# cheneeheng/2s-AGCN

Measured on AMD Instinct MI355X. Metric: skeleton-clips/sec fwd+bwd, NTU (N,3,300,25,2), higher is better.
Workload: dtype f32; 1 GPU; AGCN joint-stream NTU-xview shape, full training step (fwd, CE, bwd, grad all-reduce, clip 1.0, SGD nesterov); per_gpu_batch=64, global_batch=64, input=(N,3,300,25,2), parallelism=dp1, bn=per-replica

## Files before the change

### 2s-agcn_amd/csrc/agcn_common.h

```cpp
#pragma once
#include <hip/hip_runtime.h>
#include <stdint.h>
#include <stdlib.h>
#include <string.h>

typedef float f32x16 __attribute__((ext_vector_type(16)));
typedef float f32x4 __attribute__((ext_vector_type(4)));

#define AGCN_OK 0
#define AGCN_ERR_ARG (-1)
#define AGCN_ERR_WORKSPACE (-2)
#define AGCN_ERR_UNSUPPORTED (-3)

__device__ __forceinline__ f32x16 mfma32(float a, float b, f32x16 c) {
  return __builtin_amdgcn_mfma_f32_32x32x2f32(a, b, c, 0, 0, 0);
}
__device__ __forceinline__ int mfma_row(int j, int h) { return (j & 3) + 8 * (j >> 2) + 4 * h; }

__device__ __forceinline__ float mask_load(const float* m, long idx, int bits) {
  return bits ? m[idx >> 5] : m[idx];
}
__device__ __forceinline__ bool mask_pass(float raw, long idx, int bits) {
  return bits ? ((__builtin_bit_cast(unsigned, raw) >> (idx & 31)) & 1u) != 0u : raw > 0.f;
}

__device__ __forceinline__ float half_sum(float v) {
  v += __shfl_xor(v, 16);
  v += __shfl_xor(v, 8);
  v += __shfl_xor(v, 4);
  v += __shfl_xor(v, 2);
  v += __shfl_xor(v, 1);
  return v;
}

__device__ __forceinline__ int xcd_remap(int bid, int nwg) {
  const int q = nwg >> 3, r = nwg & 7, x = bid & 7, k = bid >> 3;
  const int base = (x < r) ? x * (q + 1) : r * (q + 1) + (x - r) * q;
  return base + k;
}

extern "C" size_t agcn_colsum_scratch_bytes(int W);
extern "C" int agcn_colsum(const float* X, int nslots, int W, void* scratch, float* out, void* stream);

int agcn_adj_finalize(const float* spart, const float* A, const float* PA, const float* alpha, float* P, float* adj,
                      int N, int Ci, int T, int V, hipStream_t s, int nused = -1);

bool agcn_adj_ws_supported(int N, int C, int Ci, int T, int V);
size_t agcn_adj_ws_workspace(int C, int Ci);
int agcn_adj_ws_scores(const float* x, const float* wab, const float* bab, float* tp_out, float* spart, int slots,
                       int* nslots_used, const float* x_absmax, void* ws, size_t ws_bytes, int N, int C, int Ci, int T, int V,
                       hipStream_t s);

size_t agcn_bf16_conv_workspace(int Cin, int Cout, int T, int V, int stride);
bool agcn_bf16_conv_wide(int taps, int M);
int agcn_bf16_conv9_fwd(const float* x, const float* w, const float* bias, float* y, float* stats_part, void* ws,
                        size_t ws_bytes, int N, int Cin, int Cout, int T, int V, int stride, int npl, hipStream_t s,
                        const float* add = nullptr, int relu = 0, const float* x_absmax = nullptr);
int agcn_bf16_conv9_bwd_data(const float* dy, const float* w, float* dx, int accumulate, const float* add1,
                             const float* mask1, const float* add2, const float* mask2, void* ws, size_t ws_bytes,
                             int N, int Cin, int Cout, int T, int V, int stride, int npl, hipStream_t s,
                             const float* dy_absmax = nullptr);

bool agcn_bf16_tconv_supported(int taps, int stride);
int agcn_bf16_tconv_tile_frames(int taps, int M, int V, int T_out, int npl);
int agcn_bf16_tconv_fwd(const float* x, const float* w, const float* bias, float* y, float* stats_part, void* ws,
                        size_t ws_bytes, int N, int Cin, int Cout, int T, int V, int taps, int pad, int npl,
                        hipStream_t s, const float* x_absmax);
int agcn_bf16_tconv_bwd_data(const float* dy, const float* w, float* dx, int accumulate, const float* add1,
                             const float* mask1, const float* add2, const float* mask2, void* ws, size_t ws_bytes,
                             int N, int Cin, int Cout, int T, int V, int taps, int pad, int npl, hipStream_t s,
                             const float* dy_absmax);

struct GateArgs;
bool agcn_bf16_tconv_infer_supported(int taps, int stride, int pad);
int agcn_bf16_tconv_infer(const float* x, const float* w, const float* bias, float* y, void* ws, size_t ws_bytes, int N,
                          int Cin, int Cout, int T, int V, int taps, int stride, int pad, int npl, hipStream_t s,
                          const float* add, int relu, const float* x_absmax, const GateArgs* gate);

size_t agcn_bf16_conv1_workspace(int Cin, int Cout, int T, int V, int stride);
int agcn_bf16_conv1_fwd(const float* x, const float* w, const float* bias, float* y, float* stats_part, void* ws,
                        size_t ws_bytes, int N, int Cin, int Cout, int T, int V, int stride, int npl, hipStream_t s,
                        const float* add = nullptr, int relu = 0);
int agcn_bf16_conv1_bwd_data(const float* dy, const float* w, float* dx, int accumulate, const float* add1,
                             const float* mask1, const float* add2, const float* mask2, void* ws, size_t ws_bytes,
                             int N, int Cin, int Cout, int T, int V, int npl, hipStream_t s);

bool agcn_gcn_chain_supported(int M, int K, int V);
int agcn_chain_f16x3();
int agcn_gcn_chain_tiles(int T);
int agcn_gcn_chain_stats_slots(int N, int M, int K, int T, int V);
size_t agcn_gcn_chain_workspace(int M, int K, int K2, int T, int V);
int agcn_gcn_chain(int mode, const float* in, const float* adj, const float* wcat, const float* bias, float* out,
                   float* stats_part, int accumulate, const float* add1, const float* mask1, const float* add2,
                   const float* mask2, int mask_bits, const float* in2, const float* w2, int K2, void* ws, size_t ws_bytes,
                   int N, int C, int Cout, int T, int V, hipStream_t stream, int relu = 0, int w2_rows_are_outputs = 0,
                   const float* in_absmax = nullptr, const float* in2_absmax = nullptr);

bool agcn_gcn_dadj_chain_supported(int C, int V);
int agcn_gcn_dadj_chain_slots(int C, int T);
size_t agcn_gcn_dadj_chain_workspace(int C, int Cout);
int agcn_gcn_dadj_chain(const float* dy, const float* wcat, const float* x, float* dadj_part, void* ws, size_t ws_bytes,
                        int N, int C, int Cout, int T, int V, hipStream_t stream, const float* dy_absmax = nullptr,
                        const float* x_absmax = nullptr);

bool agcn_wgrad_chain_supported(int M, int C, int V);
size_t agcn_wgrad_chain_workspace(int agg, int N, int M, int C, int V, int T_out);
int agcn_wgrad_chain(int agg, const float* dy, const float* x, const float* adj, void* ws, size_t ws_bytes, int* nslabs,
                     int N, int M, int C, int V, int T_src, int T_out, int stride, hipStream_t s,
                     const float* dy_absmax = nullptr, const float* x_absmax = nullptr);

bool agcn_wgrad9_bf16_supported(int M, int C, int V, int stride);
size_t agcn_wgrad9_bf16_workspace(int N, int M, int C, int V, int T, int stride);
int agcn_wgrad9_bf16(const float* dy, const float* x, void* ws, size_t ws_bytes, int* nslabs, int N, int M, int C, int V,
                     int T, int stride, hipStream_t s, const float* dy_absmax = nullptr, const float* x_absmax = nullptr);

bool agcn_wgrad_tconv_f16_supported(int M, int C, int V, int taps, int stride, int pad);
size_t agcn_wgrad_tconv_f16_workspace(int N, int M, int C, int V, int T, int taps, int pad);
int agcn_wgrad_tconv_f16(const float* dy, const float* x, void* ws, size_t ws_bytes, int* nslabs, int N, int M, int C,
                         int V, int T, int taps, int pad, hipStream_t s, const float* dy_absmax, const float* x_absmax);

static inline int agcn_gemm_precision() {
  static int mode = -1;
  if (mode < 0) {
    const char* e = getenv("AGCN_GEMM");
    mode = 3;
    if (e && !strcmp(e, "f32")) mode = 0;
    else if (e && !strcmp(e, "bf16x3")) mode = 2;
    else if (e && !strcmp(e, "bf16")) mode = 1;
  }
  return mode;
}
static inline bool agcn_chained() { const int m = agcn_gemm_precision(); return m == 3 || m == 1; }
static inline int agcn_npl() { return agcn_gemm_precision() == 1 ? 1 : 3; }

#define AGCN_MAX_DEVICES 64
static inline int agcn_allow_big_lds_rt(const void* kern, unsigned char* done) {
  int dev = 0;
  if (hipGetDevice(&dev) != hipSuccess || dev < 0 || dev >= AGCN_MAX_DEVICES) dev = -1;
  if (dev >= 0 && __atomic_load_n(&done[dev], __ATOMIC_ACQUIRE)) return AGCN_OK;
  hipError_t e = hipFuncSetAttribute(kern, hipFuncAttributeMaxDynamicSharedMemorySize, 160 * 1024);
  if (e != hipSuccess) return (int)e;
  if (dev >= 0) __atomic_store_n(&done[dev], (unsigned char)1, __ATOMIC_RELEASE);
  return AGCN_OK;
}

#include <stdio.h>
inline thread_local char agcn_last_kernel_buf[192] = "";
#define AGCN_NOTE_KERNEL(...) snprintf(agcn_last_kernel_buf, sizeof(agcn_last_kernel_buf), __VA_ARGS__)

static inline int agcn_check_launch() {
  hipError_t e = hipGetLastError();
  return e == hipSuccess ? AGCN_OK : (int)e;
}
```

### 2s-agcn_amd/csrc/bn.hip

```cpp
#include "agcn_common.h"

namespace {

constexpr int RG = 64;

__global__ void __launch_bounds__(256)
colsum_stage1_kernel(const float* __restrict__ X, int nslots, int W, int per_group, double* __restrict__ partial) {
  __shared__ double red[4][64];
  const int col = blockIdx.x * 64 + (threadIdx.x & 63), sub = threadIdx.x >> 6;
  const int g = blockIdx.y;
  const int s_end = min(nslots, (g + 1) * per_group);
  double acc = 0.0;
  if (col < W)
    for (int s = g * per_group + sub; s < s_end; s += 4) acc += (double)X[(long)s * W + col];
  red[sub][threadIdx.x & 63] = acc;
  __syncthreads();
  if (sub == 0 && col < W)
    partial[(long)g * W + col] = red[0][threadIdx.x] + red[1][threadIdx.x] + red[2][threadIdx.x] + red[3][threadIdx.x];
}

__global__ void colsum_stage2_kernel(const double* __restrict__ partial, int W, float* __restrict__ out) {
  const int col = blockIdx.x * blockDim.x + threadIdx.x;
  if (col >= W) return;
  double s = 0.0;
  for (int g = 0; g < RG; ++g) s += partial[(long)g * W + col];
  out[col] = (float)s;
}

__global__ void bn_stats_finalize_kernel(const double* __restrict__ partial, int C, double count,
                                         const float* __restrict__ gamma, const float* __restrict__ beta,
                                         float* __restrict__ rmean, float* __restrict__ rvar, float momentum,
                                         float eps, float* __restrict__ mean_out, float* __restrict__ invstd_out,
                                         float* __restrict__ scale_out, float* __restrict__ shift_out) {
  const int c = blockIdx.x * blockDim.x + threadIdx.x;
  if (c >= C) return;
  double s = 0.0, ss = 0.0;
  for (int g = 0; g < RG; ++g) {
    s += partial[((long)g * 2 + 0) * C + c];
    ss += partial[((long)g * 2 + 1) * C + c];
  }
  const double mean = s / count;
  double var = ss / count - mean * mean;
  if (var < 0.0) var = 0.0;
  const float invstd = (float)(1.0 / sqrt(var + (double)eps));
  mean_out[c] = (float)mean;
  invstd_out[c] = invstd;
  const float sc = gamma[c] * invstd;
  scale_out[c] = sc;
  shift_out[c] = beta[c] - (float)mean * sc;
  if (rmean) {
    const double unb = count > 1.0 ? var * count / (count - 1.0) : var;
    rmean[c] = (1.f - momentum) * rmean[c] + momentum * (float)mean;
    rvar[c] = (1.f - momentum) * rvar[c] + momentum * (float)unb;
  }
}

__global__ void bn_eval_coeff_kernel(const float* __restrict__ gamma, const float* __restrict__ beta,
                                     const float* __restrict__ rmean, const float* __restrict__ rvar, float eps, int C,
                                     float* __restrict__ scale_out, float* __restrict__ shift_out) {
  const int c = blockIdx.x * blockDim.x + threadIdx.x;
  if (c >= C) return;
  const float sc = gamma[c] / sqrtf(rvar[c] + eps);
  scale_out[c] = sc;
  shift_out[c] = beta[c] - rmean[c] * sc;
}

template <int RES, bool RELU>
__global__ void __launch_bounds__(256)
bn_act_fwd_kernel(const float4* __restrict__ y1, const float* __restrict__ scale1, const float* __restrict__ shift1,
                  const float4* __restrict__ r, const float* __restrict__ scale2, const float* __restrict__ shift2,
                  float4* __restrict__ out, unsigned* __restrict__ bits, unsigned total4, unsigned P, unsigned C,
                  unsigned* __restrict__ amax) {
  unsigned tmax = 0;
  for (unsigned i0 = blockIdx.x * blockDim.x; i0 < total4; i0 += gridDim.x * blockDim.x) {
    const unsigned i = i0 + threadIdx.x;
    const bool valid = i < total4;
    const unsigned ic = valid ? i : 0u;
    const unsigned e0 = ic * 4u;
    const unsigned row = e0 / P;
    const unsigned rem = e0 - row * P;
    const unsigned c0 = row % C;
    const unsigned c1 = (c0 + 1 == C) ? 0u : c0 + 1;
    const float4 a = y1[ic];
    float4 b = make_float4(0.f, 0.f, 0.f, 0.f);
    if (RES != 0) b = r[ic];
    float av[4] = {a.x, a.y, a.z, a.w};
    float bv[4] = {b.x, b.y, b.z, b.w};
    float ov[4];
#pragma unroll
    for (int k = 0; k < 4; ++k) {
      const unsigned c = (rem + k < P) ? c0 : c1;
      float v = scale1[c] * av[k] + shift1[c];
      if (RES == 1) v += bv[k];
      if (RES == 2) v += scale2[c] * bv[k] + shift2[c];
      ov[k] = RELU ? fmaxf(v, 0.f) : v;
    }
    if (valid) out[i] = make_float4(ov[0], ov[1], ov[2], ov[3]);
    if (amax && valid) {
#pragma unroll
      for (int k = 0; k < 4; ++k) tmax = max(tmax, __float_as_uint(ov[k]) & 0x7fffffffu);
    }
    if (bits) {
      unsigned nib = valid ? ((ov[0] > 0.f) | ((ov[1] > 0.f) << 1) | ((ov[2] > 0.f) << 2) | ((ov[3] > 0.f) << 3)) : 0u;
      unsigned w = nib << (4u * (threadIdx.x & 7u));
      w |= __shfl_xor(w, 1);
      w |= __shfl_xor(w, 2);
      w |= __shfl_xor(w, 4);
      if ((threadIdx.x & 7u) == 0u && valid) bits[e0 >> 5] = w;
    }
  }
  if (amax) {
#pragma unroll
    for (int k = 32; k >= 1; k >>= 1) tmax = max(tmax, (unsigned)__shfl_xor((int)tmax, k));
    __shared__ unsigned wmax[4];
    if ((threadIdx.x & 63u) == 0u) wmax[threadIdx.x >> 6] = tmax;
    __syncthreads();
    if (threadIdx.x == 0) {
      const unsigned m = max(max(wmax[0], wmax[1]), max(wmax[2], wmax[3]));
      if (m) atomicMax(amax, m);
    }
  }
}

template <bool HAS2>
__global__ void __launch_bounds__(256)
bn_bwd_reduce_kernel(const float* __restrict__ dout, const float* __restrict__ mask, int mask_bits,
                     const float* __restrict__ y1, const float* __restrict__ y2, float* __restrict__ part, int P) {
  __shared__ float red[3][4];
  const long row = blockIdx.x;
  const float* d = dout + row * P;
  const float* mk = (mask && !mask_bits) ? mask + row * P : nullptr;
  const unsigned* mb = (mask && mask_bits) ? reinterpret_cast<const unsigned*>(mask) : nullptr;
  const long e_row = row * P;
  const float* a = y1 + row * P;
  const float* b = HAS2 ? y2 + row * P : nullptr;
  float s0 = 0.f, s1 = 0.f, s2 = 0.f;
  typedef float4 float4_u __attribute__((aligned(4)));
  const int P4 = P >> 2;
  for (int q4 = threadIdx.x; q4 < P4; q4 += 256) {
    const float4 d4 = reinterpret_cast<const float4_u*>(d)[q4];
    const float4 a4 = reinterpret_cast<const float4_u*>(a)[q4];
    float dv[4] = {d4.x, d4.y, d4.z, d4.w};
    const float av[4] = {a4.x, a4.y, a4.z, a4.w};
    if (mk) {
      const float4 m4 = reinterpret_cast<const float4_u*>(mk)[q4];
      const float mv[4] = {m4.x, m4.y, m4.z, m4.w};
#pragma unroll
      for (int k = 0; k < 4; ++k) dv[k] = (mv[k] > 0.f) ? dv[k] : 0.f;
    }
    if (mb) {
      const long e = e_row + 4L * q4;
      const int sh = (int)(e & 31);
      unsigned nib = mb[e >> 5] >> sh;
      if (sh > 28) nib |= mb[(e >> 5) + 1] << (32 - sh);
#pragma unroll
      for (int k = 0; k < 4; ++k) dv[k] = ((nib >> k) & 1u) ? dv[k] : 0.f;
    }
    float bv[4] = {0.f, 0.f, 0.f, 0.f};
    if (HAS2) {
      const float4 b4 = reinterpret_cast<const float4_u*>(b)[q4];
      bv[0] = b4.x; bv[1] = b4.y; bv[2] = b4.z; bv[3] = b4.w;
    }
#pragma unroll
    for (int k = 0; k < 4; ++k) {
      s0 += dv[k];
      s1 += dv[k] * av[k];
      if (HAS2) s2 += dv[k] * bv[k];
    }
  }
  for (int q = 4 * P4 + threadIdx.x; q < P; q += 256) {
    float dz = d[q];
    if (mk) dz = (mk[q] > 0.f) ? dz : 0.f;
    if (mb) {
      const long e = e_row + q;
      dz = ((mb[e >> 5] >> (e & 31)) & 1u) ? dz : 0.f;
    }
    s0 += dz;
    s1 += dz * a[q];
    if (HAS2) s2 += dz * b[q];
  }
  s0 = half_sum(s0); s1 = half_sum(s1); s2 = half_sum(s2);
  s0 += __shfl_xor(s0, 32); s1 += __shfl_xor(s1, 32); s2 += __shfl_xor(s2, 32);
  const int wave = threadIdx.x >> 6;
  if ((threadIdx.x & 63) == 0) { red[0][wave] = s0; red[1][wave] = s1; red[2][wave] = s2; }
  __syncthreads();
  if (threadIdx.x < 3) {
    const int k = threadIdx.x;
    part[row * 3 + k] = red[k][0] + red[k][1] + red[k][2] + red[k][3];
  }
}

__global__ void bn_bwd_finalize_kernel(const float* __restrict__ part, int N, int C, double count, float pscale,
                                       const float* __restrict__ gamma1, const float* __restrict__ mean1,
                                       const float* __restrict__ invstd1, const float* __restrict__ gamma2,
                                       const float* __restrict__ mean2, const float* __restrict__ invstd2,
                                       float* __restrict__ coef, float* __restrict__ dgamma1,
                                       float* __restrict__ dbeta1, float* __restrict__ dgamma2,
                                       float* __restrict__ dbeta2) {
  const int c = blockIdx.x * blockDim.x + threadIdx.x;
  if (c >= C) return;
  double s0 = 0.0, s1 = 0.0, s2 = 0.0;
#pragma unroll 8
  for (int n = 0; n < N; ++n) {
    const float* p = part + ((long)n * C + c) * 3;
    s0 += (double)p[0]; s1 += (double)p[1]; s2 += (double)p[2];
  }
  {
    const double is = invstd1[c], mu = mean1[c], g = gamma1[c];
    const double sxh = is * (s1 - mu * s0);
    const double k = g * is;
    coef[0 * C + c] = (float)k;
    coef[1 * C + c] = (float)(-k * is * sxh / count);
    coef[2 * C + c] = (float)(-k * s0 / count + k * is * mu * sxh / count);
    dgamma1[c] = (float)sxh * pscale;
    dbeta1[c] = (float)s0 * pscale;
  }
  if (gamma2) {
    const double is = invstd2[c], mu = mean2[c], g = gamma2[c];
    const double sxh = is * (s2 - mu * s0);
    const double k = g * is;
    coef[3 * C + c] = (float)k;
    coef[4 * C + c] = (float)(-k * is * sxh / count);
    coef[5 * C + c] = (float)(-k * s0 / count + k * is * mu * sxh / count);
    dgamma2[c] = (float)sxh * pscale;
    dbeta2[c] = (float)s0 * pscale;
  }
}

template <bool HAS2>
__global__ void __launch_bounds__(256)
bn_bwd_apply_kernel(const float4* __restrict__ dout, const float4* __restrict__ mask, int mask_bits,
                    const float4* __restrict__ y1,
                    const float4* __restrict__ y2, const float* __restrict__ coef, float4* __restrict__ dy1,
                    float4* __restrict__ dy2, unsigned total4, unsigned P, unsigned C, unsigned* __restrict__ amax1) {
  unsigned tmax = 0;
  for (unsigned i = blockIdx.x * blockDim.x + threadIdx.x; i < total4; i += gridDim.x * blockDim.x) {
    const unsigned e0 = i * 4u;
    const unsigned row = e0 / P;
    const unsigned rem = e0 - row * P;
    const unsigned c0 = row % C;
    const unsigned c1 = (c0 + 1 == C) ? 0u : c0 + 1;
    const float4 d4 = dout[i];
    const float4 a4 = y1[i];
    float dv[4] = {d4.x, d4.y, d4.z, d4.w};
    float av[4] = {a4.x, a4.y, a4.z, a4.w};
    if (mask && !mask_bits) {
      const float4 m4 = mask[i];
      const float mv[4] = {m4.x, m4.y, m4.z, m4.w};
#pragma unroll
      for (int k = 0; k < 4; ++k) dv[k] = (mv[k] > 0.f) ? dv[k] : 0.f;
    } else if (mask) {
      const unsigned nib = reinterpret_cast<const unsigned*>(mask)[e0 >> 5] >> (e0 & 31u);
#pragma unroll
      for (int k = 0; k < 4; ++k) dv[k] = ((nib >> k) & 1u) ? dv[k] : 0.f;
    }
    float bv[4] = {0.f, 0.f, 0.f, 0.f};
    if (HAS2) {
      const float4 b4 = y2[i];
      bv[0] = b4.x; bv[1] = b4.y; bv[2] = b4.z; bv[3] = b4.w;
    }
    float o1[4], o2[4];
#pragma unroll
    for (int k = 0; k < 4; ++k) {
      const unsigned c = (rem + k < P) ? c0 : c1;
      o1[k] = coef[0 * C + c] * dv[k] + coef[1 * C + c] * av[k] + coef[2 * C + c];
      if (HAS2) o2[k] = coef[3 * C + c] * dv[k] + coef[4 * C + c] * bv[k] + coef[5 * C + c];
    }
    dy1[i] = make_float4(o1[0], o1[1], o1[2], o1[3]);
    if (HAS2) dy2[i] = make_float4(o2[0], o2[1], o2[2], o2[3]);
    if (amax1) {
#pragma unroll
      for (int k = 0; k < 4; ++k) tmax = max(tmax, __float_as_uint(o1[k]) & 0x7fffffffu);
    }
  }
  if (amax1) {
#pragma unroll
    for (int k = 32; k >= 1; k >>= 1) tmax = max(tmax, (unsigned)__shfl_xor((int)tmax, k));
    __shared__ unsigned wmax[4];
    if ((threadIdx.x & 63u) == 0u) wmax[threadIdx.x >> 6] = tmax;
    __syncthreads();
    if (threadIdx.x == 0) {
      const unsigned m = max(max(wmax[0], wmax[1]), max(wmax[2], wmax[3]));
      if (m) atomicMax(amax1, m);
    }
  }
}

inline unsigned ew_grid(unsigned total4) {
  unsigned g = (total4 + 255u) / 256u;
  return g > 4096u ? 4096u : (g ? g : 1u);
}

}

extern "C" {

size_t agcn_colsum_scratch_bytes(int W) { return sizeof(double) * (size_t)RG * (size_t)W; }

int agcn_colsum(const float* X, int nslots, int W, void* scratch, float* out, void* stream) {
  if (!X || !scratch || !out || nslots <= 0 || W <= 0) return AGCN_ERR_ARG;
  hipStream_t s = (hipStream_t)stream;
  const int per_group = (nslots + RG - 1) / RG;
  hipLaunchKernelGGL(colsum_stage1_kernel, dim3((W + 63) / 64, RG), dim3(256), 0, s, X, nslots, W, per_group,
                     (double*)scratch);
  int rc = agcn_check_launch();
  if (rc) return rc;
  hipLaunchKernelGGL(colsum_stage2_kernel, dim3((W + 255) / 256), dim3(256), 0, s, (const double*)scratch, W, out);
  return agcn_check_launch();
}

int agcn_bn_stats_finalize(const float* part, int nslots, int C, double count, const float* gamma, const float* beta,
                           float* running_mean, float* running_var, float momentum, float eps, void* scratch,
                           float* mean, float* invstd, float* scale, float* shift, void* stream) {
  if (!part || !gamma || !beta || !scratch || !mean || !invstd || !scale || !shift || C <= 0 || nslots <= 0)
    return AGCN_ERR_ARG;
  hipStream_t s = (hipStream_t)stream;
  const int W = 2 * C;
  const int per_group = (nslots + RG - 1) / RG;
  hipLaunchKernelGGL(colsum_stage1_kernel, dim3((W + 63) / 64, RG), dim3(256), 0, s, part, nslots, W, per_group,
                     (double*)scratch);
  int rc = agcn_check_launch();
  if (rc) return rc;
  hipLaunchKernelGGL(bn_stats_finalize_kernel, dim3((C + 63) / 64), dim3(64), 0, s, (const double*)scratch, C, count,
                     gamma, beta, running_mean, running_var, momentum, eps, mean, invstd, scale, shift);
  return agcn_check_launch();
}

int agcn_bn_eval_coeff(const float* gamma, const float* beta, const float* running_mean, const float* running_var,
                       float eps, int C, float* scale, float* shift, void* stream) {
  if (!gamma || !beta || !running_mean || !running_var || !scale || !shift || C <= 0) return AGCN_ERR_ARG;
  hipLaunchKernelGGL(bn_eval_coeff_kernel, dim3((C + 63) / 64), dim3(64), 0, (hipStream_t)stream, gamma, beta,
                     running_mean, running_var, eps, C, scale, shift);
  return agcn_check_launch();
}

int agcn_bn_act_fwd_ex(const float* y1, const float* scale1, const float* shift1, const float* r, const float* scale2,
                       const float* shift2, float* out, unsigned* sign_bits, float* absmax_out, int N, int C, int P,
                       int res_mode, int relu, void* stream);
int agcn_bn_act_fwd(const float* y1, const float* scale1, const float* shift1, const float* r, const float* scale2,
                    const float* shift2, float* out, unsigned* sign_bits, int N, int C, int P, int res_mode, int relu,
                    void* stream) {
  return agcn_bn_act_fwd_ex(y1, scale1, shift1, r, scale2, shift2, out, sign_bits, nullptr, N, C, P, res_mode, relu, stream);
}

int agcn_bn_act_fwd_ex(const float* y1, const float* scale1, const float* shift1, const float* r, const float* scale2,
                       const float* shift2, float* out, unsigned* sign_bits, float* absmax_out, int N, int C, int P,
                       int res_mode, int relu, void* stream) {
  if (!y1 || !scale1 || !shift1 || !out || N <= 0 || C <= 0 || P <= 0) return AGCN_ERR_ARG;
  if (absmax_out && hipMemsetAsync(absmax_out, 0, 4, (hipStream_t)stream) != hipSuccess) return AGCN_ERR_ARG;
  const long total = (long)N * C * P;
  if (total % 4 != 0 || total > 0xffffffffL) return AGCN_ERR_UNSUPPORTED;
  if (res_mode != 0 && !r) return AGCN_ERR_ARG;
  if (res_mode == 2 && (!scale2 || !shift2)) return AGCN_ERR_ARG;
  const unsigned t4 = (unsigned)(total / 4);
  hipStream_t s = (hipStream_t)stream;
  const dim3 g(ew_grid(t4)), b(256);
#define LAUNCH_ACT(R, A)                                                                                       \
  hipLaunchKernelGGL((bn_act_fwd_kernel<R, A>), g, b, 0, s, (const float4*)y1, scale1, shift1, (const float4*)r, \
                     scale2, shift2, (float4*)out, sign_bits, t4, (unsigned)P, (unsigned)C, (unsigned*)absmax_out)
  if (relu) {
    if (res_mode == 0) LAUNCH_ACT(0, true); else if (res_mode == 1) LAUNCH_ACT(1, true); else LAUNCH_ACT(2, true);
  } else {
    if (res_mode == 0) LAUNCH_ACT(0, false); else if (res_mode == 1) LAUNCH_ACT(1, false); else LAUNCH_ACT(2, false);
  }
#undef LAUNCH_ACT
  return agcn_check_launch();
}

int agcn_bn_bwd_reduce(const float* dout, const void* mask, int mask_bits, const float* y1, const float* y2, float* part,
                       int N, int C, int P, void* stream) {
  if (!dout || !y1 || !part || N <= 0 || C <= 0 || P <= 0) return AGCN_ERR_ARG;
  hipStream_t s = (hipStream_t)stream;
  if (y2) hipLaunchKernelGGL(bn_bwd_reduce_kernel<true>, dim3(N * C), dim3(256), 0, s, dout, (const float*)mask,
                             mask_bits, y1, y2, part, P);
  else hipLaunchKernelGGL(bn_bwd_reduce_kernel<false>, dim3(N * C), dim3(256), 0, s, dout, (const float*)mask,
                          mask_bits, y1, y2, part, P);
  return agcn_check_launch();
}

int agcn_bn_bwd_apply_ex(const float* part, int nrows, double count, float param_grad_scale, const float* dout,
                         const void* mask, int mask_bits, const float* y1, const float* gamma1, const float* mean1,
                         const float* invstd1, const float* y2, const float* gamma2, const float* mean2,
                         const float* invstd2, float* coef, float* dy1, float* dgamma1, float* dbeta1, float* dy2,
                         float* dgamma2, float* dbeta2, float* absmax1_out, int N, int C, int P, void* stream);
int agcn_bn_bwd_apply(const float* part, int nrows, double count, float param_grad_scale, const float* dout,
                      const void* mask, int mask_bits, const float* y1, const float* gamma1, const float* mean1, const float* invstd1,
                      const float* y2, const float* gamma2, const float* mean2, const float* invstd2, float* coef,
                      float* dy1, float* dgamma1, float* dbeta1, float* dy2, float* dgamma2, float* dbeta2, int N, int C,
                      int P, void* stream) {
  return agcn_bn_bwd_apply_ex(part, nrows, count, param_grad_scale, dout, mask, mask_bits, y1, gamma1, mean1, invstd1, y2,
                              gamma2, mean2, invstd2, coef, dy1, dgamma1, dbeta1, dy2, dgamma2, dbeta2, nullptr, N, C, P,
                              stream);
}

int agcn_bn_bwd_apply_ex(const float* part, int nrows, double count, float param_grad_scale, const float* dout,
                         const void* mask, int mask_bits, const float* y1, const float* gamma1, const float* mean1,
                         const float* invstd1, const float* y2, const float* gamma2, const float* mean2,
                         const float* invstd2, float* coef, float* dy1, float* dgamma1, float* dbeta1, float* dy2,
                         float* dgamma2, float* dbeta2, float* absmax1_out, int N, int C, int P, void* stream) {
  if (absmax1_out && hipMemsetAsync(absmax1_out, 0, 4, (hipStream_t)stream) != hipSuccess) return AGCN_ERR_ARG;
  if (!part || !dout || !y1 || !gamma1 || !mean1 || !invstd1 || !coef || !dy1 || !dgamma1 || !dbeta1 || nrows <= 0)
    return AGCN_ERR_ARG;
  if (y2 && (!gamma2 || !mean2 || !invstd2 || !dy2 || !dgamma2 || !dbeta2)) return AGCN_ERR_ARG;
  const long total = (long)N * C * P;
  if (total % 4 != 0 || total > 0xffffffffL) return AGCN_ERR_UNSUPPORTED;
  hipStream_t s = (hipStream_t)stream;
  hipLaunchKernelGGL(bn_bwd_finalize_kernel, dim3((C + 63) / 64), dim3(64), 0, s, part, nrows, C, count,
                     param_grad_scale, gamma1, mean1, invstd1, y2 ? gamma2 : nullptr, mean2, invstd2, coef, dgamma1,
                     dbeta1, dgamma2, dbeta2);
  int rc = agcn_check_launch();
  if (rc) return rc;
  const unsigned t4 = (unsigned)(total / 4);
  const dim3 g(ew_grid(t4)), b(256);
  if (y2)
    hipLaunchKernelGGL(bn_bwd_apply_kernel<true>, g, b, 0, s, (const float4*)dout, (const float4*)mask, mask_bits,
                       (const float4*)y1, (const float4*)y2, (const float*)coef, (float4*)dy1, (float4*)dy2, t4,
                       (unsigned)P, (unsigned)C, (unsigned*)absmax1_out);
  else
    hipLaunchKernelGGL(bn_bwd_apply_kernel<false>, g, b, 0, s, (const float4*)dout, (const float4*)mask, mask_bits,
                       (const float4*)y1, (const float4*)y2, (const float*)coef, (float4*)dy1, (float4*)dy2, t4,
                       (unsigned)P, (unsigned)C, (unsigned*)absmax1_out);
  return agcn_check_launch();
}

int agcn_bn_bwd(const float* dout, const void* mask, int mask_bits, const float* y1, const float* gamma1,
                const float* mean1, const float* invstd1, const float* y2, const float* gamma2, const float* mean2,
                const float* invstd2, float* part, float* coef, float* dy1, float* dgamma1, float* dbeta1, float* dy2,
                float* dgamma2, float* dbeta2, int N, int C, int P, void* stream) {
  int rc = agcn_bn_bwd_reduce(dout, mask, mask_bits, y1, y2, part, N, C, P, stream);
  if (rc) return rc;
  return agcn_bn_bwd_apply(part, N, (double)N * (double)P, 1.0f, dout, mask, mask_bits, y1, gamma1, mean1, invstd1, y2, gamma2,
                           mean2, invstd2, coef, dy1, dgamma1, dbeta1, dy2, dgamma2, dbeta2, N, C, P, stream);
}

const char* agcn_arch(void) { return "gfx950"; }
int agcn_version(void) { return 100; }

}
```

### 2s-agcn_amd/csrc/conv_wgrad.hip

```cpp
#include "agcn_common.h"

namespace {

struct WgradArgs {
  const float* dy;
  const float* in;
  const float* adj;
  float* part;
  int N, M, C, V, T_src, T_out, stride;
  int pad;
  int tt, ntiles, FW, WLP, DAP, GP;
  long so_m, so_t, so_c;
  long wsize;
  int nsplit, pairs_per_split;
  int off_bx, off_bg, off_adj, off_qoff;
};

template <int TAPS, int AGG, int MW, int CW, int TH, bool KSPLIT, int WBX>
__global__ void __launch_bounds__(512) conv_wgrad_kernel(const WgradArgs a) {
  constexpr int NW = 8, NT = 512;
  static_assert(MW * CW * TH == NW, "8 waves");
  constexpr int BM = MW * 32, CB = CW * 32;
  constexpr int NSUB = AGG ? 3 : 1;
  constexpr bool TSPLIT = (TH == 2) && !KSPLIT;
// ... 4 lines not shown
  float* Da = smem;
  float* Bx = smem + a.off_bx;
  float* Bg = smem + a.off_bg;
  float* adjp = smem + a.off_adj;
  int* qoff = reinterpret_cast<int*>(smem + a.off_qoff);

  const int tid = threadIdx.x, lane = tid & 63;
  const int wave = __builtin_amdgcn_readfirstlane(tid >> 6);
  const int lr = lane & 31, h = lane >> 5;
  const int th = wave / (MW * CW);
  const int wmc = wave - th * (MW * CW);
  const int mw = wmc % MW, cw = wmc / MW;
  const int ncb = (a.C + CB - 1) / CB;
  const int mb = blockIdx.x / ncb, cb = blockIdx.x - mb * ncb;
  const int m0 = mb * BM, c0 = cb * CB;
  const int V = a.V, tt = a.tt, ttv = tt * V;
  const int Psrc = a.T_src * V, Pout = a.T_out * V;
  const int WL = a.FW * V, WLP = a.WLP, DAP = a.DAP, GP = a.GP;
  const int KS = (ttv + 1) >> 1;
  const int tap0 = TSPLIT ? th * NTW : 0;
  const int ntaps = TSPLIT ? (th == 0 ? NTW : TAPS - NTW) : TAPS;
  const int s_begin = KSPLIT ? (th * ((KS + 1) >> 1)) : 0;
  const int s_end = KSPLIT ? min(KS, s_begin + ((KS + 1) >> 1)) : KS;

  for (int q = tid; q < 2 * KS + 2; q += NT) {
    int o = 0;
    if (q < ttv) {
      const int tl = q / V;
      o = AGG ? q : (tl * a.stride * V + (q - tl * V));
    }
    qoff[q] = o;
  }

  f32x16 acc[NACC];
#pragma unroll
  for (int z = 0; z < NACC; ++z)
#pragma unroll
    for (int j = 0; j < 16; ++j) acc[z][j] = 0.f;

  float rda[RD][2];
  float rbx[RB][WBX];

  auto pair_geom = [&](int p, int& n, int& t0, int& nvalid, int& g0) __attribute__((always_inline)) {
    n = p / a.ntiles;
    const int tile = p - n * a.ntiles;
    t0 = tile * tt;
    nvalid = min(tt, a.T_out - t0) * V;
    g0 = (AGG ? t0 : (t0 * a.stride - a.pad)) * V;
  };
  auto issue_loads = [&](int p) __attribute__((always_inline)) {
    int n, t0, nvalid, g0;
    pair_geom(p, n, t0, nvalid, g0);
#pragma unroll
    for (int j = 0; j < RD; ++j) {
      const int m = m0 + wave + j * NW;
      const bool okr = m < a.M;
      const float* src = a.dy + ((long)n * a.M + (okr ? m : 0)) * Pout + (long)t0 * V;
#pragma unroll
      for (int u = 0; u < 2; ++u) {
        const int q = lane + 64 * u;
        rda[j][u] = src[(okr && q < nvalid) ? q : 0];
      }
    }
#pragma unroll
    for (int j = 0; j < RB; ++j) {
      const int c = c0 + wave + j * NW;
      const bool okr = c < a.C;
      const float* src = a.in + ((long)n * a.C + (okr ? c : 0)) * Psrc;
#pragma unroll
      for (int u = 0; u < WBX; ++u) {
        const int r = lane + 64 * u;
        const int gp = g0 + r;
        rbx[j][u] = src[(okr && r < WL && gp >= 0 && gp < Psrc) ? gp : 0];
      }
    }
  };
  auto commit_lds = [&](int p) __attribute__((always_inline)) {
    int n, t0, nvalid, g0;
    pair_geom(p, n, t0, nvalid, g0);
#pragma unroll
    for (int j = 0; j < RD; ++j) {
      const int ml = wave + j * NW;
      const bool okr = (m0 + ml) < a.M;
#pragma unroll
      for (int u = 0; u < 2; ++u) {
        const int q = lane + 64 * u;
        if (q < DAP) Da[ml * DAP + q] = (okr && q < nvalid) ? rda[j][u] : 0.f;
      }
    }
#pragma unroll
    for (int j = 0; j < RB; ++j) {
      const int cl = wave + j * NW;
      const bool okr = (c0 + cl) < a.C;
#pragma unroll
      for (int u = 0; u < WBX; ++u) {
        const int r = lane + 64 * u;
        const int gp = g0 + r;
        if (r < WLP) Bx[cl * WLP + r] = (okr && r < WL && gp >= 0 && gp < Psrc) ? rbx[j][u] : 0.f;
      }
    }
  };

  const int total_pairs = a.N * a.ntiles;
  const int p_begin = blockIdx.y * a.pairs_per_split;
  const int p_end = min(total_pairs, p_begin + a.pairs_per_split);
  int last_n = -1;
  if (p_begin < p_end) issue_loads(p_begin);
  for (int p = p_begin; p < p_end; ++p) {
    __syncthreads();
    commit_lds(p);
    const int n = p / a.ntiles;
    if (AGG && n != last_n) {
      const int VP = 2 * ((V + 1) / 2);
      const float* adjn = a.adj + (long)n * 3 * V * V;
      for (int e = tid; e < 3 * VP * 32; e += NT) {
        const int i = e / (VP * 32), r = e - i * (VP * 32);
        const int u = r >> 5, col = r & 31;
        const bool ok = u < V && col < V;
        const float t = adjn[ok ? ((i * V + u) * V + col) : 0];
        adjp[e] = ok ? t : 0.f;
      }
      last_n = n;
    }
    if (p + 1 < p_end) issue_loads(p + 1);
    __syncthreads();
#pragma unroll
    for (int sub = 0; sub < NSUB; ++sub) {
      if (AGG) {
        if (sub > 0) __syncthreads();
        const int nrows = CB * tt;
        const int nrt = (nrows + 31) >> 5;
        const int VS = (V + 1) >> 1, VP = 2 * VS;
        for (int rt = wave; rt < nrt; rt += NW) {
          const int row = min(rt * 32 + lr, nrows - 1);
          f32x16 d;
#pragma unroll
          for (int j = 0; j < 16; ++j) d[j] = 0.f;
          for (int s = 0; s < VS; ++s) {
            const int u = 2 * s + h;
            float av = Bx[row * V + min(u, V - 1)];
            av = (u < V) ? av : 0.f;
            d = mfma32(av, adjp[(sub * VP + u) * 32 + lr], d);
          }
#pragma unroll
          for (int j = 0; j < 16; ++j) {
            const int r2 = rt * 32 + mfma_row(j, h);
            if (r2 < nrows && lr < V) {
              const int cl = r2 / tt, tl = r2 - cl * tt;
              Bg[cl * GP + tl * V + lr] = d[j];
            }
          }
        }
        __syncthreads();
      }
      const float* Bsrc = (AGG ? Bg : Bx) + (cw * 32 + lr) * (AGG ? GP : WLP) + tap0 * V;
      const float* Asrc = Da + (mw * 32 + lr) * DAP;
      const bool lin = AGG || a.stride == 1;
      auto load_ops = [&](int s, float& av, float (&bv)[NTW]) __attribute__((always_inline)) {
        const int q = 2 * s + h;
        const int qo = lin ? q : qoff[q];
        av = Asrc[q];
#pragma unroll
        for (int t = 0; t < NTW; ++t) bv[t] = Bsrc[qo + ((TSPLIT && t >= ntaps) ? 0 : t * V)];
      };
      if (s_begin < s_end) {
        float av, bv[NTW];
        load_ops(s_begin, av, bv);
        for (int s = s_begin; s < s_end; ++s) {
          float an, bn[NTW];
          load_ops(min(s + 1, s_end - 1), an, bn);
#pragma unroll
          for (int t = 0; t < NTW; ++t)
            if (!TSPLIT || t < ntaps) acc[sub * NTW + t] = mfma32(av, bv[t], acc[sub * NTW + t]);
          av = an;
#pragma unroll
          for (int t = 0; t < NTW; ++t) bv[t] = bn[t];
        }
      }
    }
  }
  const int slab = KSPLIT ? ((int)blockIdx.y * TH + th) : (int)blockIdx.y;
  float* dst = a.part + (long)slab * a.wsize;
#pragma unroll
  for (int z = 0; z < NACC; ++z) {
    const int sub = z / NTW, t = z - sub * NTW;
    if (TSPLIT && t >= ntaps) continue;
    const int zz = AGG ? sub : (tap0 + t);
#pragma unroll
    for (int j = 0; j < 16; ++j) {
      const int m = m0 + mw * 32 + mfma_row(j, h);
      const int c = c0 + cw * 32 + lr;
      if (m < a.M && c < a.C) dst[((long)zz * a.M + m) * a.C + c] = acc[z][j];
    }
  }
}

__global__ void wgrad_reduce_kernel(const float* __restrict__ part, float* __restrict__ dw, long wsize, int nsplit,
                                    int M, int C, long so_m, long so_t, long so_c) {
  const long i = (long)blockIdx.x * blockDim.x + threadIdx.x;
  if (i >= wsize) return;
  float s = 0.f;
  for (int k = 0; k < nsplit; ++k) s += part[(long)k * wsize + i];
  const int c = (int)(i % C);
  const long r = i / C;
  const int m = (int)(r % M);
  const int z = (int)(r / M);
  dw[(long)m * so_m + (long)z * so_t + (long)c * so_c] = s;
}

__global__ void __launch_bounds__(256)
wgrad_reduce_wide_kernel(const float* __restrict__ part, float* __restrict__ dw, long wsize, int nsplit, int M, int C,
                         long so_m, long so_t, long so_c) {
  __shared__ float red[8][32];
  const int el = threadIdx.x & 31, g = threadIdx.x >> 5;
  const long i = (long)blockIdx.x * 32 + el;
  float s = 0.f;
  if (i < wsize) {
#pragma unroll 8
    for (int k = g; k < nsplit; k += 8) s += part[(long)k * wsize + i];
  }
  red[g][el] = s;
  __syncthreads();
  if (g == 0 && i < wsize) {
    float t = red[0][el];
#pragma unroll
    for (int k = 1; k < 8; ++k) t += red[k][el];
    const int c = (int)(i % C);
    const long r = i / C;
    const int m = (int)(r % M);
    const int z = (int)(r / M);
    dw[(long)m * so_m + (long)z * so_t + (long)c * so_c] = t;
  }
}

inline int launch_reduce(const float* ws, float* dw, long wsize, int nslabs, int M, int C, long so_m, long so_t, long so_c,
                         hipStream_t stream) {
  if (nslabs >= 64) {
    hipLaunchKernelGGL(wgrad_reduce_wide_kernel, dim3((unsigned)((wsize + 31) / 32)), dim3(256), 0, stream, ws, dw,
                       wsize, nslabs, M, C, so_m, so_t, so_c);
  } else {
    const int threads = 256;
    hipLaunchKernelGGL(wgrad_reduce_kernel, dim3((unsigned)((wsize + threads - 1) / threads)), dim3(threads), 0,
                       stream, ws, dw, wsize, nslabs, M, C, so_m, so_t, so_c);
  }
  return agcn_check_launch();
}

struct WGeom {
  int tt, ntiles, FW, WLP, DAP, GP, nsplit, nslabs, pairs_per_split, grid_x;
  int off_bx, off_bg, off_adj, off_qoff;
  size_t smem_bytes;
};

template <int TAPS, int AGG, int MW, int CW, int TH, bool KSPLIT>
WGeom wgeom(int N, int M, int C, int V, int T_out, int stride, int tt_cap = 0) {
  constexpr int BM = MW * 32, CB = CW * 32;
  WGeom g;
  g.tt = 128 / V;
  if (g.tt > T_out) g.tt = T_out;
  if (tt_cap > 0 && g.tt > tt_cap) g.tt = tt_cap;
  const int ttv = g.tt * V;
  g.ntiles = (T_out + g.tt - 1) / g.tt;
  g.FW = AGG ? g.tt : ((g.tt - 1) * stride + TAPS);
  const int WL = g.FW * V;
  g.WLP = AGG ? WL : (WL | 1);
  if (!AGG && g.WLP == WL) g.WLP = WL + 2;
  g.DAP = (ttv + 2) | 1;
  g.GP = ttv | 1;
  const int da = BM * g.DAP;
  g.off_bx = (da + 3) & ~3;
  const int bx = CB * g.WLP + 64;
  g.off_bg = g.off_bx + ((bx + 3) & ~3);
  const int bg = AGG ? CB * g.GP + 64 : 0;
  g.off_adj = g.off_bg + ((bg + 3) & ~3);
  const int VP = 2 * ((V + 1) / 2);
  const int adjsz = AGG ? 3 * VP * 32 : 0;
  g.off_qoff = g.off_adj + ((adjsz + 3) & ~3);
  g.smem_bytes = 4 * ((size_t)g.off_qoff + ttv + 8);
  const int nmb = (M + BM - 1) / BM, ncb = (C + CB - 1) / CB;
  g.grid_x = nmb * ncb;
  const int pairs = N * g.ntiles;
  int want = 256 / g.grid_x;
  if (want < 1) want = 1;
  if (want > pairs) want = pairs;
  g.pairs_per_split = (pairs + want - 1) / want;
  g.nsplit = (pairs + g.pairs_per_split - 1) / g.pairs_per_split;
  g.nslabs = g.nsplit * (KSPLIT ? TH : 1);
  return g;
}

template <int TAPS, int AGG, int MW, int CW, int TH, bool KSPLIT, int WBX>
int launch_wgrad(WgradArgs a, float* dw, void* ws, size_t ws_bytes, hipStream_t stream, int tt_cap = 0) {
  const WGeom g = wgeom<TAPS, AGG, MW, CW, TH, KSPLIT>(a.N, a.M, a.C, a.V, a.T_out, a.stride, tt_cap);
  if (g.smem_bytes > 160 * 1024) return AGCN_ERR_UNSUPPORTED;
  if (g.WLP > WBX * 64 || g.tt * a.V > 128) return AGCN_ERR_UNSUPPORTED;
  if ((size_t)g.nslabs * a.wsize * 4 > ws_bytes) return AGCN_ERR_WORKSPACE;
  a.part = (float*)ws;
  a.tt = g.tt; a.ntiles = g.ntiles; a.FW = g.FW; a.WLP = g.WLP; a.DAP = g.DAP; a.GP = g.GP;
  a.nsplit = g.nsplit; a.pairs_per_split = g.pairs_per_split;
  a.off_bx = g.off_bx; a.off_bg = g.off_bg; a.off_adj = g.off_adj; a.off_qoff = g.off_qoff;
  auto kern = conv_wgrad_kernel<TAPS, AGG, MW, CW, TH, KSPLIT, WBX>;
  static unsigned char lds_ok[AGCN_MAX_DEVICES] = {};
  if (int e = agcn_allow_big_lds_rt(reinterpret_cast<const void*>(kern), lds_ok)) return e;
  hipLaunchKernelGGL(kern, dim3(g.grid_x, g.nsplit), dim3(512), g.smem_bytes, stream, a);
  int rc = agcn_check_launch();
  if (rc) return rc;
  return launch_reduce((const float*)ws, dw, a.wsize, g.nslabs, a.M, a.C, a.so_m, a.so_t, a.so_c, stream);
}

template <int TAPS, int AGG, int MW, int CW, int TH, bool KSPLIT>
size_t ws_wgrad(int N, int M, int C, int V, int T_out, int stride, long wsize, int tt_cap = 0) {
  const WGeom g = wgeom<TAPS, AGG, MW, CW, TH, KSPLIT>(N, M, C, V, T_out, stride, tt_cap);
  return (size_t)g.nslabs * wsize * 4;
}

int chain_wgrad_and_reduce(int agg, const WgradArgs& a, float* dw, void* ws, size_t ws_bytes, hipStream_t stream,
                           const float* dy_absmax = nullptr, const float* x_absmax = nullptr) {
  int nslabs = 0;
  int rc = agcn_wgrad_chain(agg, a.dy, a.in, a.adj, ws, ws_bytes, &nslabs, a.N, a.M, a.C, a.V, a.T_src, a.T_out,
                            a.stride, stream, dy_absmax, x_absmax);
  if (rc) return rc;
  return launch_reduce((const float*)ws, dw, a.wsize, nslabs, a.M, a.C, a.so_m, a.so_t, a.so_c, stream);
}

inline bool wgrad9_bf16_enabled() {
  static int v = -1;
  if (v < 0) {
    const char* e = getenv("AGCN_WGRAD9_BF16");
    v = (e && atoi(e) == 0) ? 0 : 1;
  }
  return v == 1;
}

constexpr int WBXT = 8;

inline int tconv_w_tt(int V, int T_out, int taps, int stride) {
  int tt = 128 / V;
  if (tt > T_out) tt = T_out;
  while (tt > 1 && ((tt - 1) * stride + taps) * V + 2 > WBXT * 64) --tt;
  return tt < 1 ? 1 : tt;
}

template <int TAPS>
int tconv_wgrad(WgradArgs a, float* dw, void* ws, size_t ws_bytes, hipStream_t s, size_t* ws_need) {
  const int cap = tconv_w_tt(a.V, a.T_out, TAPS, a.stride);
  if (!ws_need) AGCN_NOTE_KERNEL("conv_wgrad_kernel<%d, 0>", TAPS);
  if (TAPS == 1) {
    if (a.M % 128 == 0) {
      if (ws_need) { *ws_need = ws_wgrad<1, 0, 4, 2, 1, false>(a.N, a.M, a.C, a.V, a.T_out, a.stride, a.wsize, cap); return 0; }
      return launch_wgrad<1, 0, 4, 2, 1, false, WBXT>(a, dw, ws, ws_bytes, s, cap);
    }
    if (ws_need) { *ws_need = ws_wgrad<1, 0, 2, 2, 2, true>(a.N, a.M, a.C, a.V, a.T_out, a.stride, a.wsize, cap); return 0; }
    return launch_wgrad<1, 0, 2, 2, 2, true, WBXT>(a, dw, ws, ws_bytes, s, cap);
  }
  if (a.M % 128 == 0) {
    if (ws_need) { *ws_need = ws_wgrad<TAPS, 0, 4, 1, 2, false>(a.N, a.M, a.C, a.V, a.T_out, a.stride, a.wsize, cap); return 0; }
    return launch_wgrad<TAPS, 0, 4, 1, 2, false, WBXT>(a, dw, ws, ws_bytes, s, cap);
  }
  if (ws_need) { *ws_need = ws_wgrad<TAPS, 0, 2, 2, 2, false>(a.N, a.M, a.C, a.V, a.T_out, a.stride, a.wsize, cap); return 0; }
  return launch_wgrad<TAPS, 0, 2, 2, 2, false, WBXT>(a, dw, ws, ws_bytes, s, cap);
}

int tconv_wgrad_dispatch(int taps, const WgradArgs& a, float* dw, void* ws, size_t ws_bytes, hipStream_t s,
                         size_t* ws_need) {
  switch (taps) {
    case 1: return tconv_wgrad<1>(a, dw, ws, ws_bytes, s, ws_need);
    case 2: return tconv_wgrad<2>(a, dw, ws, ws_bytes, s, ws_need);
    case 3: return tconv_wgrad<3>(a, dw, ws, ws_bytes, s, ws_need);
    case 4: return tconv_wgrad<4>(a, dw, ws, ws_bytes, s, ws_need);
    case 5: return tconv_wgrad<5>(a, dw, ws, ws_bytes, s, ws_need);
    case 6: return tconv_wgrad<6>(a, dw, ws, ws_bytes, s, ws_need);
    case 7: return tconv_wgrad<7>(a, dw, ws, ws_bytes, s, ws_need);
    case 8: return tconv_wgrad<8>(a, dw, ws, ws_bytes, s, ws_need);
    case 9: return tconv_wgrad<9>(a, dw, ws, ws_bytes, s, ws_need);
    default: return AGCN_ERR_UNSUPPORTED;
  }
}

inline bool tconv_w_domain(int T, int taps, int stride, int pad) {
  return taps >= 1 && taps <= 9 && stride >= 1 && stride <= 9 && pad >= 0 && pad <= (taps - 1) / 2 && T + 2 * pad >= taps;
}

inline bool chain_wgrad_enabled() {
  static int v = -1;
  if (v < 0) {
    const char* e = getenv("AGCN_WGRAD_BF16");
    v = (e && atoi(e) == 0) ? 0 : 1;
  }
  return v == 1 && agcn_chained();
}

}

extern "C" {

size_t agcn_conv_bwd_weight_workspace(int N, int Cin, int Cout, int T, int V, int taps, int stride) {
  const int pad = (taps - 1) / 2;
  const int T_out = (T + 2 * pad - taps) / stride + 1;
  const long wsize = (long)Cout * Cin * taps;
  if (taps == 9) {
    size_t b9 = (Cout % 128 == 0) ? ws_wgrad<9, 0, 4, 1, 2, false>(N, Cout, Cin, V, T_out, stride, wsize)
                                  : ws_wgrad<9, 0, 2, 2, 2, false>(N, Cout, Cin, V, T_out, stride, wsize);
    if (agcn_wgrad9_bf16_supported(Cout, Cin, V, stride)) {
      const size_t t = agcn_wgrad9_bf16_workspace(N, Cout, Cin, V, T, stride);
      if (t > b9) b9 = t;
    }
    return b9;
  }
  size_t b = (Cout % 128 == 0) ? ws_wgrad<1, 0, 4, 2, 1, false>(N, Cout, Cin, V, T_out, stride, wsize)
                              : ws_wgrad<1, 0, 2, 2, 2, true>(N, Cout, Cin, V, T_out, stride, wsize);
  if (agcn_wgrad_chain_supported(Cout, Cin, V)) {
    const size_t t = agcn_wgrad_chain_workspace(0, N, Cout, Cin, V, T_out);
    if (t > b) b = t;
  }
  return b;
}

int agcn_conv_bwd_weight_ex(const float* dy, const float* x, float* dw, void* workspace, size_t workspace_bytes, int N,
                            int Cin, int Cout, int T, int V, int taps, int stride, const float* dy_absmax,
                            const float* x_absmax, void* stream);
int agcn_conv_bwd_weight(const float* dy, const float* x, float* dw, void* workspace, size_t workspace_bytes, int N,
                         int Cin, int Cout, int T, int V, int taps, int stride, void* stream) {
  return agcn_conv_bwd_weight_ex(dy, x, dw, workspace, workspace_bytes, N, Cin, Cout, T, V, taps, stride, nullptr, nullptr,
                                 stream);
}
int agcn_conv_bwd_weight_ex(const float* dy, const float* x, float* dw, void* workspace, size_t workspace_bytes, int N,
                            int Cin, int Cout, int T, int V, int taps, int stride, const float* dy_absmax,
                            const float* x_absmax, void* stream) {
  if (!dy || !x || !dw || !workspace || N <= 0 || Cin <= 0 || Cout <= 0 || T <= 0 || V <= 0 || V > 32)
    return AGCN_ERR_ARG;
  if ((taps != 1 && taps != 9) || (stride != 1 && stride != 2)) return AGCN_ERR_UNSUPPORTED;
  const int pad = (taps - 1) / 2;
  WgradArgs a = {};
  a.dy = dy; a.in = x; a.N = N; a.M = Cout; a.C = Cin; a.V = V; a.T_src = T;
  a.T_out = (T + 2 * pad - taps) / stride + 1; a.stride = stride; a.pad = pad;
  a.so_m = (long)Cin * taps; a.so_t = 1; a.so_c = taps; a.wsize = (long)Cout * Cin * taps;
  hipStream_t s = (hipStream_t)stream;
  if (taps == 9) {
    if (wgrad9_bf16_enabled() && agcn_wgrad9_bf16_supported(Cout, Cin, V, stride)) {
      int nslabs = 0;
      int rc = agcn_wgrad9_bf16(dy, x, workspace, workspace_bytes, &nslabs, N, Cout, Cin, V, T, stride, s, dy_absmax, x_absmax);
      if (rc) return rc;
      return launch_reduce((const float*)workspace, dw, a.wsize, nslabs, a.M, a.C, a.so_m, a.so_t, a.so_c, s);
    }
    if (stride == 1) {
      if (Cout % 128 == 0) return launch_wgrad<9, 0, 4, 1, 2, false, 6>(a, dw, workspace, workspace_bytes, s);
      return launch_wgrad<9, 0, 2, 2, 2, false, 6>(a, dw, workspace, workspace_bytes, s);
    }
    if (Cout % 128 == 0) return launch_wgrad<9, 0, 4, 1, 2, false, 7>(a, dw, workspace, workspace_bytes, s);
    return launch_wgrad<9, 0, 2, 2, 2, false, 7>(a, dw, workspace, workspace_bytes, s);
  }
  if (chain_wgrad_enabled() && agcn_wgrad_chain_supported(Cout, Cin, V))
    return chain_wgrad_and_reduce(0, a, dw, workspace, workspace_bytes, s, dy_absmax, x_absmax);
  if (Cout % 128 == 0) return launch_wgrad<1, 0, 4, 2, 1, false, 4>(a, dw, workspace, workspace_bytes, s);
  return launch_wgrad<1, 0, 2, 2, 2, true, 4>(a, dw, workspace, workspace_bytes, s);
}

size_t agcn_gcn_project_bwd_weight_workspace(int N, int C, int Cout, int T, int V) {
  const long wsize = 3L * Cout * C;
  size_t b = (Cout % 128 == 0) ? ws_wgrad<1, 1, 4, 2, 1, false>(N, Cout, C, V, T, 1, wsize)
                              : ws_wgrad<1, 1, 2, 2, 2, true>(N, Cout, C, V, T, 1, wsize);
  if (agcn_wgrad_chain_supported(Cout, C, V)) {
    const size_t t = agcn_wgrad_chain_workspace(1, N, Cout, C, V, T);
    if (t > b) b = t;
  }
  return b;
}

int agcn_gcn_project_bwd_weight_ex(const float* dy, const float* x, const float* adj, float* dwcat, void* workspace,
                                   size_t workspace_bytes, int N, int C, int Cout, int T, int V, const float* dy_absmax,
                                   const float* x_absmax, void* stream);
int agcn_gcn_project_bwd_weight(const float* dy, const float* x, const float* adj, float* dwcat, void* workspace,
                                size_t workspace_bytes, int N, int C, int Cout, int T, int V, void* stream) {
  return agcn_gcn_project_bwd_weight_ex(dy, x, adj, dwcat, workspace, workspace_bytes, N, C, Cout, T, V, nullptr, nullptr,
                                        stream);
}
int agcn_gcn_project_bwd_weight_ex(const float* dy, const float* x, const float* adj, float* dwcat, void* workspace,
                                   size_t workspace_bytes, int N, int C, int Cout, int T, int V, const float* dy_absmax,
                                   const float* x_absmax, void* stream) {
  if (!dy || !x || !adj || !dwcat || !workspace || N <= 0 || C <= 0 || Cout <= 0 || T <= 0 || V <= 0 || V > 32)
    return AGCN_ERR_ARG;
  WgradArgs a = {};
  a.dy = dy; a.in = x; a.adj = adj; a.N = N; a.M = Cout; a.C = C; a.V = V; a.T_src = T; a.T_out = T; a.stride = 1;
  a.so_m = 3L * C; a.so_t = C; a.so_c = 1; a.wsize = 3L * Cout * C;
  hipStream_t s = (hipStream_t)stream;
  if (chain_wgrad_enabled() && agcn_wgrad_chain_supported(Cout, C, V))
    return chain_wgrad_and_reduce(1, a, dwcat, workspace, workspace_bytes, s, dy_absmax, x_absmax);
  if (Cout % 128 == 0) return launch_wgrad<1, 1, 4, 2, 1, false, 2>(a, dwcat, workspace, workspace_bytes, s);
  return launch_wgrad<1, 1, 2, 2, 2, true, 2>(a, dwcat, workspace, workspace_bytes, s);
}


size_t agcn_tconv_bwd_weight_workspace(int N, int Cin, int Cout, int T, int V, int taps, int stride, int pad) {
  if (N <= 0 || Cin <= 0 || Cout <= 0 || T <= 0 || V <= 0 || !tconv_w_domain(T, taps, stride, pad)) return 0;
  if (pad == (taps - 1) / 2 && (taps == 1 || taps == 9) && (stride == 1 || stride == 2))
    return agcn_conv_bwd_weight_workspace(N, Cin, Cout, T, V, taps, stride);
  WgradArgs a = {};
  a.N = N; a.M = Cout; a.C = Cin; a.V = V; a.T_src = T; a.T_out = (T + 2 * pad - taps) / stride + 1; a.stride = stride;
  a.pad = pad; a.wsize = (long)Cout * Cin * taps;
  size_t need = 0;
  tconv_wgrad_dispatch(taps, a, nullptr, nullptr, 0, nullptr, &need);
  if (agcn_wgrad_tconv_f16_supported(Cout, Cin, V, taps, stride, pad)) {
    const size_t t = agcn_wgrad_tconv_f16_workspace(N, Cout, Cin, V, T, taps, pad);
    if (t > need) need = t;
  }
  return need;
}

int agcn_tconv_bwd_weight(const float* dy, const float* x, float* dw, void* workspace, size_t workspace_bytes, int N,
                          int Cin, int Cout, int T, int V, int taps, int stride, int pad, const float* dy_absmax,
                          const float* x_absmax, void* stream) {
  if (!dy || !x || !dw || !workspace || N <= 0 || Cin <= 0 || Cout <= 0 || T <= 0 || V <= 0 || V > 32)
    return AGCN_ERR_ARG;
  if (!tconv_w_domain(T, taps, stride, pad)) return AGCN_ERR_UNSUPPORTED;
  if (pad == (taps - 1) / 2 && (taps == 1 || taps == 9) && (stride == 1 || stride == 2))
    return agcn_conv_bwd_weight_ex(dy, x, dw, workspace, workspace_bytes, N, Cin, Cout, T, V, taps, stride, dy_absmax,
                                   x_absmax, stream);
  WgradArgs a = {};
  a.dy = dy; a.in = x; a.N = N; a.M = Cout; a.C = Cin; a.V = V; a.T_src = T;
  a.T_out = (T + 2 * pad - taps) / stride + 1; a.stride = stride; a.pad = pad;
  a.so_m = (long)Cin * taps; a.so_t = 1; a.so_c = taps; a.wsize = (long)Cout * Cin * taps;
  hipStream_t s = (hipStream_t)stream;
  if (agcn_wgrad_tconv_f16_supported(Cout, Cin, V, taps, stride, pad)) {
    int nslabs = 0;
    const int rc = agcn_wgrad_tconv_f16(dy, x, workspace, workspace_bytes, &nslabs, N, Cout, Cin, V, T, taps, pad, s,
                                        dy_absmax, x_absmax);
    if (rc) return rc;
    return launch_reduce((const float*)workspace, dw, a.wsize, nslabs, a.M, a.C, a.so_m, a.so_t, a.so_c, s);
  }
  return tconv_wgrad_dispatch(taps, a, dw, workspace, workspace_bytes, s, nullptr);
}

}
```

### 2s-agcn_amd/csrc/wgrad_chain.hip

```cpp
#include "agcn_common.h"
#include "split_f16.h"

namespace {

typedef __bf16 bf16x8 __attribute__((ext_vector_type(8)));
typedef __bf16 bf16x2 __attribute__((ext_vector_type(2)));
typedef float f32x2 __attribute__((ext_vector_type(2)));
typedef unsigned u32x4 __attribute__((ext_vector_type(4)));
typedef f32x4 f32x4_u __attribute__((aligned(4)));

struct WcArgs {
  const float* dy;
  const float* in;
  const float* adj;
  float* part;
  int N, M, C, V, T_src, T_out, stride;
  int ntiles, pairs_per_split, ncg;
  int XP;
  long wsize;
  int npl;
  int dbg;
  int pad;
  const float* dy_absmax;
  const float* in_absmax;
// ... 314 lines not shown
            for (int e = 0; e < 4; ++e) rdy[k][4 * run + e] = q[e];
          }
        } else {
#pragma unroll
          for (int e = 0; e < 8; ++e) {
            const float* q = src + (e & 3) + 8 * (e >> 2);
            rdy[k][e] = (q < dy_end) ? *q : 0.f;
          }
        }
      }
      const int piece = ptid & (LPR - 1), rsub = (ptid & 63) / LPR;
      const float* xb = a.in + (long)n * a.C * Psrc + (long)t0 * V + 4 * piece;
#pragma unroll
      for (int u = 0; u < XV; ++u) {
        const int row = (wave - NWC) * (CG / NWP) + u * (64 / LPR) + rsub;
        const float* src = xb + (long)min(c0 + row, a.C - 1) * Psrc;
        if (src + 4 <= x_end) {
          rx[u] = *reinterpret_cast<const f32x4_u*>(src);
        } else {
#pragma unroll
          for (int e = 0; e < 4; ++e) rx[u][e] = (src + e < x_end) ? src[e] : 0.f;
        }
      }
    };
    auto commit = [&](int p, unsigned char* buf) __attribute__((always_inline)) {
      int n, t0;
      pair_geom(p, n, t0);
      int ptid = threadIdx.x - NWC * 64;
      asm volatile("" : "+v"(ptid));
      unsigned char* dyi = buf;
      float* xs = reinterpret_cast<float*>(buf + DY_BYTES);
#pragma unroll
      for (int k = 0; k < DI; ++k) {
        const int item = ptid + k * NTP;
        const int o = item / (FT * 4), r = item - o * (FT * 4);
        u32x4 ph, pm, pl;
#pragma unroll
        for (int e2 = 0; e2 < 4; ++e2) {
          unsigned q0, q1, q2 = 0;
          if constexpr (F16) split_pair_f16(rdy[k][2 * e2] * s_dy, rdy[k][2 * e2 + 1] * s_dy, q0, q1);
          else wc_split_pair(rdy[k][2 * e2], rdy[k][2 * e2 + 1], q0, q1, q2);
          ph[e2] = q0; pm[e2] = q1; pl[e2] = q2;
        }
        const int slot = r * BMP + o;
        *reinterpret_cast<u32x4*>(dyi + ((0 * FT * 4) * BMP + slot) * 16) = ph;
        *reinterpret_cast<u32x4*>(dyi + ((1 * FT * 4) * BMP + slot) * 16) = pm;
        if constexpr (!F16) *reinterpret_cast<u32x4*>(dyi + ((2 * FT * 4) * BMP + slot) * 16) = pl;
      }
      const int piece = ptid & (LPR - 1), rsub = (ptid & 63) / LPR;
#pragma unroll
      for (int u = 0; u < XV; ++u) {
        const int row = (wave - NWC) * (CG / NWP) + u * (64 / LPR) + rsub;
#pragma unroll
        for (int e = 0; e < 4; ++e) {
          const int q = 4 * piece + e;
          if (q < FTV) xs[row * XP + q] = rx[u][e];
        }
      }
      if (AGG && n != adj_n[p & 1]) {
        adj_n[p & 1] = n;
        const float* adjn = a.adj + (long)n * 3 * V * V;
        if constexpr (!BCH) {
          float* adjp = reinterpret_cast<float*>(buf + BUF_BYTES - ADJ_BYTES);
          for (int e = ptid; e < 3 * 32 * 32; e += NTP) {
            const int sub = e >> 10, u = (e >> 5) & 31, v = e & 31;
            const bool ok = u < V && v < V;
            const float tv = adjn[ok ? ((sub * V + u) * V + v) : 0];
            adjp[e] = ok ? tv : 0.f;
          }
        } else {
          unsigned char* adjq = buf + BUF_BYTES - ADJ_BYTES;
          for (int e = ptid; e < 3 * 2 * 2 * 32 * 4; e += NTP) {
            const int e2 = e & 3, col = (e >> 2) & 31, hh = (e >> 7) & 1, ks = (e >> 8) & 1, sub = e >> 9;
            float vv[2];
#pragma unroll
            for (int q = 0; q < 2; ++q) {
              const int u = 16 * ks + 8 * hh + 2 * e2 + q;
              const bool ok = u < V && col < V;
              const float tv = adjn[ok ? ((sub * V + u) * V + col) : 0];
              vv[q] = ok ? tv : 0.f;
            }
            unsigned q0, q1, q2 = 0;
            if constexpr (F16) split_pair_f16(vv[0], vv[1], q0, q1);
            else wc_split_pair(vv[0], vv[1], q0, q1, q2);
            const int o = (((ks * 2 + hh) * 32) + col) * 16 + e2 * 4;
            *reinterpret_cast<unsigned*>(adjq + (sub * PLA + 0) * 2048 + o) = q0;
            *reinterpret_cast<unsigned*>(adjq + (sub * PLA + 1) * 2048 + o) = q1;
            if constexpr (!F16) *reinterpret_cast<unsigned*>(adjq + (sub * PLA + 2) * 2048 + o) = q2;
          }
        }
      }
    };
    if (XP > FTV)
      for (int e = threadIdx.x - NWC * 64; e < 2 * CG; e += NTP)
        reinterpret_cast<float*>(smem + (e / CG) * BUF_BYTES + DY_BYTES)[(e % CG) * XP + FTV] = 0.f;
    {
      const int gap = (((CG * XP * 4 + 15) & ~15) - CG * XP * 4 + XSLACK) / 4;
      const int e = threadIdx.x - NWC * 64;
      if (e < 2 * gap) reinterpret_cast<float*>(smem + (e / max(gap, 1)) * BUF_BYTES + DY_BYTES)[CG * XP + e % max(gap, 1)] = 0.f;
    }
    if (p_begin < p_end) {
      issue(p_begin);
      commit(p_begin, smem + (p_begin & 1) * BUF_BYTES);
      if (p_begin + 1 < p_end) issue(p_begin + 1);
    }
    stage_barrier();
    for (int p = p_begin; p < p_end; ++p) {
      if (p + 1 < p_end && !(a.dbg & 2)) {
        commit(p + 1, smem + ((p + 1) & 1) * BUF_BYTES);
        if (p + 2 < p_end) issue(p + 2);
      }
      stage_barrier();
    }
    return;
  }

  const int lane = threadIdx.x & 63;
  const int lr = lane & 31, h = lane >> 5;
  const int cbw = wave % NCB, fg = (wave / NCB) % NFG, rb = wave / (NCB * NFG);
  f32x16 acc[NS][TM];
#pragma unroll
  for (int sub = 0; sub < NS; ++sub)
#pragma unroll
    for (int tm = 0; tm < TM; ++tm)
#pragma unroll
      for (int j = 0; j < 16; ++j) acc[sub][tm][j] = 0.f;
  stage_barrier();
  for (int p = p_begin; p < p_end; ++p) {
    int n, t0;
    pair_geom(p, n, t0);
    const unsigned char* dyi = smem + (p & 1) * BUF_BYTES;
    const float* xs = reinterpret_cast<const float*>(dyi + DY_BYTES);
    const int f = fg;
    if (t0 + f < a.T_out && !(a.dbg & 1)) {
      const float* xr = xs + (cbw * 32 + lr) * XP + f * V;
      const unsigned char* ab = dyi + (((f * 4 + h) * BMP) + rb * (TM * 32) + lr) * 16;
#pragma unroll
      for (int sub = 0; sub < NS; ++sub) {
        f32x16 d;
        if (AGG) {
#pragma unroll
          for (int j = 0; j < 16; ++j) d[j] = 0.f;
          const float* xrs = xr;
          asm volatile("" : "+v"(xrs));
          if constexpr (!BCH) {
            const float* adjp = reinterpret_cast<const float*>(dyi + BUF_BYTES - ADJ_BYTES) + sub * 1024;
            float ao[BCH ? 1 : VS], xo[BCH ? 1 : VS];
#pragma unroll
            for (int s = 0; s < VS; ++s) {
              ao[s] = adjp[(2 * s + h) * 32 + lr];
              xo[s] = xrs[2 * s + h];
            }
#pragma unroll
            for (int s = 0; s < VS; ++s) d = mfma32(ao[s], xo[s], d);
          } else {
            const unsigned char* aq = dyi + BUF_BYTES - ADJ_BYTES + sub * PLA * 2048 + (h * 32 + lr) * 16;
#pragma unroll
            for (int ks = 0; ks < 2; ++ks) {
              u32x4 qh, qm, ql;
#pragma unroll
              for (int e2 = 0; e2 < 4; ++e2) {
                unsigned q0, q1, q2 = 0;
                const float xa = xrs[16 * ks + 8 * h + 2 * e2], xb2 = xrs[16 * ks + 8 * h + 2 * e2 + 1];
                if constexpr (F16) split_pair_f16_mix(xa * s_x, xb2 * s_x, q0, q1);
                else wc_split_pair(xa, xb2, q0, q1, q2);
                qh[e2] = q0; qm[e2] = q1; ql[e2] = q2;
              }
              if constexpr (F16) {
                const f16x8 x0 = __builtin_bit_cast(f16x8, qh), x1 = __builtin_bit_cast(f16x8, qm);
                const f16x8 a0 = *reinterpret_cast<const f16x8*>(aq + 0 * 2048 + ks * 1024);
                const f16x8 a1 = *reinterpret_cast<const f16x8*>(aq + 1 * 2048 + ks * 1024);
                d = __builtin_amdgcn_mfma_f32_32x32x16_f16(a1, x0, d, 0, 0, 0);
                d = __builtin_amdgcn_mfma_f32_32x32x16_f16(a0, x1, d, 0, 0, 0);
                d = __builtin_amdgcn_mfma_f32_32x32x16_f16(a0, x0, d, 0, 0, 0);
              } else {
                const bf16x8 x0 = __builtin_bit_cast(bf16x8, qh), x1 = __builtin_bit_cast(bf16x8, qm),
                             x2 = __builtin_bit_cast(bf16x8, ql);
                const bf16x8 a0 = *reinterpret_cast<const bf16x8*>(aq + 0 * 2048 + ks * 1024);
                const bf16x8 a1 = *reinterpret_cast<const bf16x8*>(aq + 1 * 2048 + ks * 1024);
                const bf16x8 a2 = *reinterpret_cast<const bf16x8*>(aq + 2 * 2048 + ks * 1024);
                d = __builtin_amdgcn_mfma_f32_32x32x16_bf16(a2, x0, d, 0, 0, 0);
                d = __builtin_amdgcn_mfma_f32_32x32x16_bf16(a0, x2, d, 0, 0, 0);
                d = __builtin_amdgcn_mfma_f32_32x32x16_bf16(a1, x1, d, 0, 0, 0);
                d = __builtin_amdgcn_mfma_f32_32x32x16_bf16(a1, x0, d, 0, 0, 0);
                d = __builtin_amdgcn_mfma_f32_32x32x16_bf16(a0, x1, d, 0, 0, 0);
                d = __builtin_amdgcn_mfma_f32_32x32x16_bf16(a0, x0, d, 0, 0, 0);
              }
            }
          }
        } else {
#pragma unroll
          for (int j = 0; j < 16; ++j) {
            const int v = (j & 3) + 8 * (j >> 2) + 4 * h;
            const float t = xr[v];
            d[j] = (v < V) ? t : 0.f;
          }
        }
        bf16x8 gb[2][3];
#pragma unroll
        for (int ks = 0; ks < 2; ++ks) {
          u32x4 gh, gm, gl;
#pragma unroll
          for (int e2 = 0; e2 < 4; ++e2) {
            unsigned q0, q1, q2 = 0;
            if constexpr (F16 && BCH) split_pair_f16_mix(d[8 * ks + 2 * e2], d[8 * ks + 2 * e2 + 1], q0, q1);
            else if constexpr (F16) split_pair_f16(d[8 * ks + 2 * e2] * s_x, d[8 * ks + 2 * e2 + 1] * s_x, q0, q1);
            else wc_split_pair(d[8 * ks + 2 * e2], d[8 * ks + 2 * e2 + 1], q0, q1, q2);
            gh[e2] = q0; gm[e2] = q1; gl[e2] = q2;
          }
          gb[ks][0] = __builtin_bit_cast(bf16x8, gh);
          gb[ks][1] = __builtin_bit_cast(bf16x8, gm);
          gb[ks][2] = __builtin_bit_cast(bf16x8, gl);
        }
        auto load_a = [&](bf16x8 (&af)[3], int step) __attribute__((always_inline)) {
          const int ks = step / TM, tm = step - ks * TM;
#pragma unroll
          for (int pl = 0; pl < PL; ++pl)
            af[pl] = *reinterpret_cast<const bf16x8*>(ab + ((pl * FT * 4 + ks * 2) * BMP + tm * 32) * 16);
        };
        bf16x8 afc[3];
        load_a(afc, 0);
        __builtin_amdgcn_sched_group_barrier(0x100, PL, 0);
#pragma unroll
        for (int step = 0; step < 2 * TM; ++step) {
          const int ks = step / TM, tm = step - ks * TM;
          bf16x8 afn[3];
          if (step + 1 < 2 * TM) load_a(afn, step + 1);
          if constexpr (F16) {
            acc[sub][tm] = __builtin_amdgcn_mfma_f32_32x32x16_f16(__builtin_bit_cast(f16x8, afc[1]), __builtin_bit_cast(f16x8, gb[ks][0]), acc[sub][tm], 0, 0, 0);
            acc[sub][tm] = __builtin_amdgcn_mfma_f32_32x32x16_f16(__builtin_bit_cast(f16x8, afc[0]), __builtin_bit_cast(f16x8, gb[ks][1]), acc[sub][tm], 0, 0, 0);
            acc[sub][tm] = __builtin_amdgcn_mfma_f32_32x32x16_f16(__builtin_bit_cast(f16x8, afc[0]), __builtin_bit_cast(f16x8, gb[ks][0]), acc[sub][tm], 0, 0, 0);
          } else {
          if (a.npl == 3) {
            acc[sub][tm] = __builtin_amdgcn_mfma_f32_32x32x16_bf16(afc[2], gb[ks][0], acc[sub][tm], 0, 0, 0);
            acc[sub][tm] = __builtin_amdgcn_mfma_f32_32x32x16_bf16(afc[0], gb[ks][2], acc[sub][tm], 0, 0, 0);
            acc[sub][tm] = __builtin_amdgcn_mfma_f32_32x32x16_bf16(afc[1], gb[ks][1], acc[sub][tm], 0, 0, 0);
            acc[sub][tm] = __builtin_amdgcn_mfma_f32_32x32x16_bf16(afc[1], gb[ks][0], acc[sub][tm], 0, 0, 0);
            acc[sub][tm] = __builtin_amdgcn_mfma_f32_32x32x16_bf16(afc[0], gb[ks][1], acc[sub][tm], 0, 0, 0);
          }
          acc[sub][tm] = __builtin_amdgcn_mfma_f32_32x32x16_bf16(afc[0], gb[ks][0], acc[sub][tm], 0, 0, 0);
          }
          if (step + 1 < 2 * TM) {
            __builtin_amdgcn_sched_group_barrier(0x100, PL, 0);
#pragma unroll
            for (int pl = 0; pl < PL; ++pl) afc[pl] = afn[pl];
          }
          __builtin_amdgcn_sched_group_barrier(0x008, NPROD, 0);
        }
        __builtin_amdgcn_sched_barrier(0);
      }
    }
    stage_barrier();
  }
  const int slab = (int)blockIdx.y * NFG + fg;
#pragma unroll
  for (int sub = 0; sub < NS; ++sub) {
    float* dst = a.part + (long)slab * a.wsize + (long)sub * a.M * a.C;
#pragma unroll
    for (int tm = 0; tm < TM; ++tm)
#pragma unroll
      for (int j = 0; j < 16; ++j) {
        const int m = m0 + (rb * TM + tm) * 32 + mfma_row(j, h);
        const int c = c0 + cbw * 32 + lr;
        if (m < a.M && c < a.C) dst[(long)m * a.C + c] = F16 ? acc[sub][tm][j] * (inv_dy * inv_x) : acc[sub][tm][j];
      }
  }
}

struct WcGeom {
  int ntiles, ncg, nmb, nsplit, nslabs, pairs_per_split, grid_x, XP;
  size_t smem_bytes;
};

template <int AGG, int TM, int NCB, int NW = 8>
WcGeom wc_geom(int N, int M, int C, int V, int T_out) {
  constexpr int BM = TM * 32, NFG = NW / NCB, FPW = (NCB <= 2) ? 1 : 2, FT = NFG * FPW, CG = NCB * 32;
  WcGeom g;
  g.ntiles = (T_out + FT - 1) / FT;
  g.ncg = (C + CG - 1) / CG;
  g.nmb = (M + BM - 1) / BM;
  g.XP = (FT * V) | 1;
  g.smem_bytes = (size_t)3 * FT * 4 * (BM + 1) * 16 + (size_t)CG * g.XP * 4 + (AGG ? 32 * 32 * 4 : 0);
  g.grid_x = g.nmb * g.ncg * (AGG ? 3 : 1);
  const int pairs = N * g.ntiles;
  int want = (256 * 8 / NW) / g.grid_x;
  if (want < 1) want = 1;
  if (want > pairs) want = pairs;
  g.pairs_per_split = (pairs + want - 1) / want;
  g.nsplit = (pairs + g.pairs_per_split - 1) / g.pairs_per_split;
  g.nslabs = g.nsplit * NFG;
  return g;
}

template <int AGG, int TM, int NCB, int VS, int NW = 8>
int wc_launch(WcArgs a, void* ws, size_t ws_bytes, int* nslabs_out, hipStream_t stream) {
  const WcGeom g = wc_geom<AGG, TM, NCB, NW>(a.N, a.M, a.C, a.V, a.T_out);
  if (g.smem_bytes > 160 * 1024) return AGCN_ERR_UNSUPPORTED;
  if ((size_t)g.nslabs * a.wsize * 4 > ws_bytes) return AGCN_ERR_WORKSPACE;
  a.part = (float*)ws;
  a.ntiles = g.ntiles; a.pairs_per_split = g.pairs_per_split; a.ncg = g.ncg; a.XP = g.XP;
  auto kern = wgrad_chain_kernel<AGG, TM, NCB, VS, NW>;
  static unsigned char lds_ok[AGCN_MAX_DEVICES] = {};
  if (int e = agcn_allow_big_lds_rt(reinterpret_cast<const void*>(kern), lds_ok)) return e;
  hipLaunchKernelGGL(kern, dim3(g.grid_x, g.nsplit), dim3(NW * 64), g.smem_bytes, stream, a);
  *nslabs_out = g.nslabs;
  return agcn_check_launch();
}

template <int AGG, int TM, int NCB>
int wc_dispatch_vs(const WcArgs& a, void* ws, size_t ws_bytes, int* nslabs, hipStream_t s) {
  const int vs = (a.V + 1) / 2;
  if constexpr (!AGG) {
    return wc_launch<AGG, TM, NCB, 1>(a, ws, ws_bytes, nslabs, s);
  } else {
    if (vs == 13) return wc_launch<AGG, TM, NCB, 13>(a, ws, ws_bytes, nslabs, s);
    if (vs == 9) return wc_launch<AGG, TM, NCB, 9>(a, ws, ws_bytes, nslabs, s);
    return wc_launch<AGG, TM, NCB, 16>(a, ws, ws_bytes, nslabs, s);
  }
}

static inline bool wc_four_waves() {
  static int v = -1;
  if (v < 0) {
    const char* e = getenv("AGCN_WGRAD_NW");
    v = (e && atoi(e) == 8) ? 0 : 1;
  }
  return v == 1;
}

template <int AGG, int TM, int NCB, int NW>
int wc_dispatch_vs4(const WcArgs& a, void* ws, size_t ws_bytes, int* nslabs, hipStream_t s) {
  const int vs = (a.V + 1) / 2;
  if constexpr (!AGG) {
    return wc_launch<AGG, TM, NCB, 1, NW>(a, ws, ws_bytes, nslabs, s);
  } else {
    if (vs == 13) return wc_launch<AGG, TM, NCB, 13, NW>(a, ws, ws_bytes, nslabs, s);
    if (vs == 9) return wc_launch<AGG, TM, NCB, 9, NW>(a, ws, ws_bytes, nslabs, s);
    return wc_launch<AGG, TM, NCB, 16, NW>(a, ws, ws_bytes, nslabs, s);
  }
}

template <int AGG, int TM>
int wc_dispatch_ncb(const WcArgs& a, void* ws, size_t ws_bytes, int* nslabs, hipStream_t s) {
  if (wc_four_waves() && !AGG && a.C % 128 == 0) return wc_dispatch_vs4<AGG, TM, 4, 4>(a, ws, ws_bytes, nslabs, s);
  if (wc_four_waves() && a.C % 64 == 0 && !(AGG && a.C % 128 == 0)) return wc_dispatch_vs4<AGG, TM, 2, 4>(a, ws, ws_bytes, nslabs, s);
  if (a.C % 256 == 0) return wc_dispatch_vs<AGG, TM, 8>(a, ws, ws_bytes, nslabs, s);
  if (a.C % 128 == 0) return wc_dispatch_vs<AGG, TM, 4>(a, ws, ws_bytes, nslabs, s);
  if (a.C % 64 == 0) return wc_dispatch_vs<AGG, TM, 2>(a, ws, ws_bytes, nslabs, s);
  return wc_dispatch_vs<AGG, TM, 1>(a, ws, ws_bytes, nslabs, s);
}

template <int AGG>
size_t wc_slabs(int N, int M, int C, int V, int T_out) {
  const bool tm4 = M > 64 && C % 64 == 0;
  int n;
  if (wc_four_waves() && !AGG && C % 128 == 0) n = tm4 ? wc_geom<AGG, 4, 4, 4>(N, M, C, V, T_out).nslabs : wc_geom<AGG, 2, 4, 4>(N, M, C, V, T_out).nslabs;
  else if (wc_four_waves() && C % 64 == 0 && !(AGG && C % 128 == 0)) n = tm4 ? wc_geom<AGG, 4, 2, 4>(N, M, C, V, T_out).nslabs : wc_geom<AGG, 2, 2, 4>(N, M, C, V, T_out).nslabs;
  else if (C % 256 == 0) n = tm4 ? wc_geom<AGG, 4, 8>(N, M, C, V, T_out).nslabs : wc_geom<AGG, 2, 8>(N, M, C, V, T_out).nslabs;
  else if (C % 128 == 0) n = tm4 ? wc_geom<AGG, 4, 4>(N, M, C, V, T_out).nslabs : wc_geom<AGG, 2, 4>(N, M, C, V, T_out).nslabs;
  else if (C % 64 == 0) n = tm4 ? wc_geom<AGG, 4, 2>(N, M, C, V, T_out).nslabs : wc_geom<AGG, 2, 2>(N, M, C, V, T_out).nslabs;
  else n = tm4 ? wc_geom<AGG, 4, 1>(N, M, C, V, T_out).nslabs : wc_geom<AGG, 2, 1>(N, M, C, V, T_out).nslabs;
  return (size_t)n;
}


template <int AGG, int TM, int NCB, int NRB>
WcGeom wc_geom_pc(int N, int M, int C, int V, int T_out, bool bch = false, int planes = 3) {
  constexpr int BM = TM * 32 * NRB, NFG = 8 / (NCB * NRB), FT = NFG, CG = NCB * 32;
  WcGeom g;
  g.ntiles = (T_out + FT - 1) / FT;
  g.ncg = (C + CG - 1) / CG;
  g.nmb = (M + BM - 1) / BM;
  g.XP = (FT * V) | 1;
  g.smem_bytes = 2 * ((size_t)planes * FT * 4 * (BM + 1) * 16 + (((size_t)CG * g.XP * 4 + 15) & ~(size_t)15) +
                      (AGG ? (bch ? (size_t)3 * planes * 2 * 2 * 32 * 16 + 128 : (size_t)3 * 32 * 32 * 4) : 0)) + 32;
  g.grid_x = g.nmb * g.ncg;
  const int pairs = N * g.ntiles;
  int want = 256 / g.grid_x;
  if (want < 1) want = 1;
  if (want > pairs) want = pairs;
  g.pairs_per_split = (pairs + want - 1) / want;
  g.nsplit = (pairs + g.pairs_per_split - 1) / g.pairs_per_split;
  g.nslabs = g.nsplit * NFG;
  return g;
}

static inline bool wc_f16x3() {
  static const int on = getenv("AGCN_WGRAD_F16X3") ? atoi(getenv("AGCN_WGRAD_F16X3")) : 1;
  return on != 0;
}

template <int AGG, int TM, int NCB, int NRB, int VS, int NWP = 4>
int wc_launch_pc(WcArgs a, void* ws, size_t ws_bytes, int* nslabs_out, hipStream_t stream) {
  {
    if (a.dy_absmax && a.in_absmax && a.npl == 3 && wc_f16x3()) {
      const WcGeom g = wc_geom_pc<AGG, TM, NCB, NRB>(a.N, a.M, a.C, a.V, a.T_out, AGG && VS == 0, 2);
      if (g.smem_bytes > 160 * 1024) return AGCN_ERR_UNSUPPORTED;
      if ((size_t)g.nslabs * a.wsize * 4 > ws_bytes) return AGCN_ERR_WORKSPACE;
      a.part = (float*)ws;
      a.ntiles = g.ntiles; a.pairs_per_split = g.pairs_per_split; a.ncg = g.ncg; a.XP = g.XP;
      auto kern = wgrad_pc_kernel<AGG, TM, NCB, VS, NRB, 8, NWP, true>;
      static unsigned char lds_ok[AGCN_MAX_DEVICES] = {};
      if (int e = agcn_allow_big_lds_rt(reinterpret_cast<const void*>(kern), lds_ok)) return e;
      AGCN_NOTE_KERNEL("wgrad_pc_kernel<%d, %d, %d, %d, %d, 8, %d, true>", AGG, TM, NCB, VS, NRB, NWP);
      hipLaunchKernelGGL(kern, dim3(g.grid_x, g.nsplit), dim3((8 + NWP) * 64), g.smem_bytes, stream, a);
      *nslabs_out = g.nslabs;
      return agcn_check_launch();
    }
  }
  const WcGeom g = wc_geom_pc<AGG, TM, NCB, NRB>(a.N, a.M, a.C, a.V, a.T_out, AGG && VS == 0);
  if (g.smem_bytes > 160 * 1024) return AGCN_ERR_UNSUPPORTED;
  if ((size_t)g.nslabs * a.wsize * 4 > ws_bytes) return AGCN_ERR_WORKSPACE;
  a.part = (float*)ws;
  a.ntiles = g.ntiles; a.pairs_per_split = g.pairs_per_split; a.ncg = g.ncg; a.XP = g.XP;
  auto kern = wgrad_pc_kernel<AGG, TM, NCB, VS, NRB, 8, NWP>;
  static unsigned char lds_ok[AGCN_MAX_DEVICES] = {};
  if (int e = agcn_allow_big_lds_rt(reinterpret_cast<const void*>(kern), lds_ok)) return e;
  AGCN_NOTE_KERNEL("wgrad_pc_kernel<%d, %d, %d, %d, %d, 8, %d>", AGG, TM, NCB, VS, NRB, NWP);
  hipLaunchKernelGGL(kern, dim3(g.grid_x, g.nsplit), dim3((8 + NWP) * 64), g.smem_bytes, stream, a);
  *nslabs_out = g.nslabs;
  return agcn_check_launch();
}

template <int AGG, int TM, int NCB, int NRB>
int wc_dispatch_pc_vs(const WcArgs& a, void* ws, size_t ws_bytes, int* nslabs, hipStream_t s) {
  const int vs = (a.V + 1) / 2;
  if constexpr (!AGG) {
    return wc_launch_pc<AGG, TM, NCB, NRB, 1>(a, ws, ws_bytes, nslabs, s);
  } else {
    static const int bch = getenv("AGCN_WC_BCH") ? atoi(getenv("AGCN_WC_BCH")) : 0;
    if (bch && a.npl == 3) return wc_launch_pc<AGG, TM, NCB, NRB, 0>(a, ws, ws_bytes, nslabs, s);
    static const int agg16 = getenv("AGCN_WC_AGG16") ? atoi(getenv("AGCN_WC_AGG16")) : 1;
    if (agg16 && a.dy_absmax && a.in_absmax && a.npl == 3 && wc_f16x3())
      return wc_launch_pc<AGG, TM, NCB, NRB, 0>(a, ws, ws_bytes, nslabs, s);
    if (vs == 13) return wc_launch_pc<AGG, TM, NCB, NRB, 13>(a, ws, ws_bytes, nslabs, s);
    if (vs == 9) return wc_launch_pc<AGG, TM, NCB, NRB, 9>(a, ws, ws_bytes, nslabs, s);
    return wc_launch_pc<AGG, TM, NCB, NRB, 16>(a, ws, ws_bytes, nslabs, s);
  }
}

static inline bool wc_pc_enabled() {
  static int v = -1;
  if (v < 0) {
    const char* e = getenv("AGCN_WC_PC");
    v = (e && atoi(e) == 0) ? 0 : 1;
  }
  return v == 1;
}
static inline bool wc_pc_applies(int C) { return wc_pc_enabled() && C % 64 == 0; }

template <int AGG>
int wc_dispatch_pc(const WcArgs& a, void* ws, size_t ws_bytes, int* nslabs, hipStream_t s) {
  if constexpr (AGG) {
    if (a.C % 128 == 0) return wc_dispatch_pc_vs<1, 2, 4, 1>(a, ws, ws_bytes, nslabs, s);
    return wc_dispatch_pc_vs<1, 2, 2, 2>(a, ws, ws_bytes, nslabs, s);
  } else {
    static const int nwp8 = getenv("AGCN_WC_NWP8") ? atoi(getenv("AGCN_WC_NWP8")) : -1;
    if (a.C % 128 == 0 && (nwp8 == 1 || (nwp8 < 0 && a.M > 64 && a.M <= 192)))
      return wc_launch_pc<0, 2, 4, 1, 1, 8>(a, ws, ws_bytes, nslabs, s);
    if (a.C % 128 == 0) {
      if (a.M > 64) return wc_dispatch_pc_vs<0, 4, 4, 1>(a, ws, ws_bytes, nslabs, s);
      return wc_dispatch_pc_vs<0, 2, 4, 1>(a, ws, ws_bytes, nslabs, s);
    }
    return wc_dispatch_pc_vs<0, 2, 2, 2>(a, ws, ws_bytes, nslabs, s);
  }
}

template <int AGG>
size_t wc_slabs_pc(int N, int M, int C, int V, int T_out) {
  if constexpr (AGG) {
    if (C % 128 == 0) return (size_t)wc_geom_pc<1, 2, 4, 1>(N, M, C, V, T_out).nslabs;
    return (size_t)wc_geom_pc<1, 2, 2, 2>(N, M, C, V, T_out).nslabs;
  } else {
    if (C % 128 == 0) {
      const size_t n4 = (size_t)wc_geom_pc<0, 4, 4, 1>(N, M, C, V, T_out).nslabs;
      const size_t n2 = (size_t)wc_geom_pc<0, 2, 4, 1>(N, M, C, V, T_out).nslabs;
      return n4 > n2 ? n4 : n2;
    }
    return (size_t)wc_geom_pc<0, 2, 2, 2>(N, M, C, V, T_out).nslabs;
  }
}

}

bool agcn_wgrad_chain_supported(int M, int C, int V) { return M >= 64 && (C % 64 == 0 || C <= 32) && C >= 1 && V <= 32; }

size_t agcn_wgrad_chain_workspace(int agg, int N, int M, int C, int V, int T_out) {
  const long wsize = (long)(agg ? 3 : 1) * M * C;
  size_t n = agg ? wc_slabs<1>(N, M, C, V, T_out) : wc_slabs<0>(N, M, C, V, T_out);
  if (C % 64 == 0) {
    const size_t m = agg ? wc_slabs_pc<1>(N, M, C, V, T_out) : wc_slabs_pc<0>(N, M, C, V, T_out);
    if (m > n) n = m;
  }
  return n * (size_t)wsize * 4;
}

int agcn_wgrad_chain(int agg, const float* dy, const float* x, const float* adj, void* ws, size_t ws_bytes, int* nslabs,
                     int N, int M, int C, int V, int T_src, int T_out, int stride, hipStream_t s, const float* dy_absmax,
                     const float* x_absmax) {
  WcArgs a = {};
  a.dy_absmax = dy_absmax; a.in_absmax = x_absmax;
  a.npl = agcn_npl();
  { const char* e = getenv("AGCN_WC_PAD"); a.pad = (e && atoi(e) == 0) ? 0 : 1; }
  { const char* e = getenv("AGCN_WC_DBG"); a.dbg = e ? atoi(e) : 0; }
  a.dy = dy; a.in = x; a.adj = adj; a.N = N; a.M = M; a.C = C; a.V = V; a.T_src = T_src; a.T_out = T_out;
  a.stride = stride; a.wsize = (long)(agg ? 3 : 1) * M * C;
  if (wc_pc_applies(C) && stride == 1 && !(agg && C % 128 != 0 && M <= 64)) return agg ? wc_dispatch_pc<1>(a, ws, ws_bytes, nslabs, s) : wc_dispatch_pc<0>(a, ws, ws_bytes, nslabs, s);
  const bool tm4 = M > 64 && C % 64 == 0;
  if (agg) return tm4 ? wc_dispatch_ncb<1, 4>(a, ws, ws_bytes, nslabs, s) : wc_dispatch_ncb<1, 2>(a, ws, ws_bytes, nslabs, s);
  return tm4 ? wc_dispatch_ncb<0, 4>(a, ws, ws_bytes, nslabs, s) : wc_dispatch_ncb<0, 2>(a, ws, ws_bytes, nslabs, s);
}
```

### 2s-agcn_amd/lib.py

```python
import ctypes
import os

import torch

_HERE = os.path.dirname(os.path.abspath(__file__))
LIB_PATH = os.path.join(_HERE, "libagcn_hip.so")

_P = ctypes.c_void_p
_I = ctypes.c_int
_F = ctypes.c_float
_D = ctypes.c_double
_Z = ctypes.c_size_t

SIGNATURES = {
    "agcn_version": (_I, []),
    "agcn_arch": (ctypes.c_char_p, []),
    "agcn_last_kernel": (ctypes.c_char_p, []),
    "agcn_gemm_mode": (ctypes.c_char_p, []),
    "agcn_chain_mode": (ctypes.c_char_p, []),
    "agcn_conv_tile_frames": (_I, [_I, _I]),
    "agcn_conv_num_tiles": (_I, [_I, _I]),
    "agcn_conv_stats_tiles": (_I, [_I, _I, _I, _I, _I, _I]),
    "agcn_dadj_num_slots": (_I, [_I, _I, _I]),
    "agcn_scores_num_tiles": (_I, [_I, _I]),
    "agcn_conv_workspace": (_Z, [_I, _I, _I, _I, _I, _I]),
    "agcn_gcn_workspace": (_Z, [_I, _I, _I, _I]),
    "agcn_gcn_stats_tiles": (_I, [_I, _I, _I, _I]),
    "agcn_gcn_stats_slots": (_I, [_I, _I, _I, _I, _I]),
    "agcn_conv_fwd": (_I, [_P, _P, _P, _P, _P, _P, _Z, _I, _I, _I, _I, _I, _I, _I, _P]),
    "agcn_conv_bwd_data": (_I, [_P, _P, _P, _I, _P, _P, _P, _P, _P, _Z, _I, _I, _I, _I, _I, _I, _I, _P]),
    "agcn_conv_bwd_weight_workspace": (_Z, [_I, _I, _I, _I, _I, _I, _I]),
    "agcn_conv_bwd_weight": (_I, [_P, _P, _P, _P, _Z, _I, _I, _I, _I, _I, _I, _I, _P]),
    "agcn_gcn_aggregate_project_fwd": (_I, [_P, _P, _P, _P, _P, _P, _P, _Z, _I, _I, _I, _I, _I, _P]),
    "agcn_gcn_aggregate_project_fwd_ex": (_I, [_P, _P, _P, _P, _P, _P, _P, _Z, _I, _I, _I, _I, _I, _P, _P]),
    "agcn_gcn_aggregate_project_bwd_data_ex": (_I, [_P, _P, _P, _P, _P, _I, _P, _I, _P, _P, _P, _P, _I, _P, _Z, _I, _I, _I, _I, _I, _P, _P, _P]),
    "agcn_gcn_dadj_ex": (_I, [_P, _P, _P, _P, _P, _Z, _I, _I, _I, _I, _I, _P, _P, _P]),
    "agcn_adjacency_bwd_scores_ex": (_I, [_P, _P, _P, _P, _P, _P, _P, _I, _I, _I, _I, _P]),
    "agcn_conv_bwd_weight_ex": (_I, [_P, _P, _P, _P, _Z, _I, _I, _I, _I, _I, _I, _I, _P, _P, _P]),
    "agcn_gcn_project_bwd_weight_ex": (_I, [_P, _P, _P, _P, _P, _Z, _I, _I, _I, _I, _I, _P, _P, _P]),
    "agcn_absmax": (_I, [_P, ctypes.c_long, _P, _P]),
    "agcn_tconv_workspace": (_Z, [_I] * 7),
    "agcn_tconv_stats_tiles": (_I, [_I] * 7),
    "agcn_tconv_fwd": (_I, [_P] * 6 + [_Z] + [_I] * 8 + [_P, _P]),
    "agcn_tconv_bwd_data": (_I, [_P, _P, _P, _I, _P, _P, _P, _P, _P, _Z] + [_I] * 8 + [_P, _P]),
    "agcn_tconv_bwd_weight_workspace": (_Z, [_I] * 8),
    "agcn_tconv_bwd_weight": (_I, [_P] * 4 + [_Z] + [_I] * 8 + [_P] * 3),
    "agcn_bn_act_fwd_ex": (_I, [_P, _P, _P, _P, _P, _P, _P, _P, _P, _I, _I, _I, _I, _I, _P]),
    "agcn_bn_bwd_apply_ex": (_I, [_P, _I, _D, _F, _P, _P, _I] + [_P] * 16 + [_I, _I, _I, _P]),
    "agcn_conv_fwd_ex": (_I, [_P, _P, _P, _P, _P, _P, _Z, _I, _I, _I, _I, _I, _I, _I, _P, _P]),
    "agcn_conv_bwd_data_ex": (_I, [_P, _P, _P, _I, _P, _P, _P, _P, _P, _Z, _I, _I, _I, _I, _I, _I, _I, _P, _P]),
    "agcn_gcn_first_supported": (_I, [_I, _I, _I]),
    "agcn_gcn_first_tiles": (_I, [_I, _I]),
    "agcn_gcn_first_fwd": (_I, [_P, _P, _P, _P, _P, _P, _P, _P, _P, _P, _I, _I, _I, _I, _I, _P]),
    "agcn_gcn_unit_infer_workspace": (_Z, [_I, _I, _I, _I, _I]),
    "agcn_gcn_unit_infer": (_I, [_P, _P, _P, _P, _P, _P, _P, _I, _I, _P, _P, _Z, _I, _I, _I, _I, _I, _P]),
    "agcn_conv9_infer": (_I, [_P, _P, _P, _P, _I, _P, _P, _Z, _I, _I, _I, _I, _I, _I, _P]),
    "agcn_tconv_infer": (_I, [_P] * 7 + [_I, _P, _P, _Z] + [_I] * 8 + [_P, _P]),
    "agcn_gcn_aggregate_project_bwd_data": (_I, [_P, _P, _P, _P, _I, _P, _P, _P, _P, _I, _P, _Z, _I, _I, _I, _I, _I, _P]),
    "agcn_gcn_bwd_data_fused_supported": (_I, [_I, _I, _I]),
    "agcn_gcn_aggregate_project_bwd_data_fused": (_I, [_P, _P, _P, _P, _P, _I, _P, _I, _P, _P, _P, _P, _I, _P, _Z, _I, _I, _I, _I, _I, _P]),
    "agcn_gcn_dadj": (_I, [_P, _P, _P, _P, _P, _Z, _I, _I, _I, _I, _I, _P]),
    "agcn_gcn_project_bwd_weight_workspace": (_Z, [_I, _I, _I, _I, _I]),
    "agcn_gcn_project_bwd_weight": (_I, [_P, _P, _P, _P, _P, _Z, _I, _I, _I, _I, _I, _P]),
    "agcn_adjacency_fwd": (_I, [_P, _P, _P, _P, _P, _P, _P, _I, _I, _I, _I, _P]),
    "agcn_adjacency_fused_supported": (_I, [_I, _I, _I, _I]),
    "agcn_adjacency_fused_workspace": (_Z, [_I, _I]),
    "agcn_adjacency_fused_fwd": (_I, [_P, _P, _P, _P, _P, _P, _P, _P, _P, _P, _P, _Z, _I, _I, _I, _I, _I, _P]),
    "agcn_adjacency_fused_fwd_ex": (_I, [_P, _P, _P, _P, _P, _P, _P, _P, _P, _P, _P, _P, _P, _Z, _I, _I, _I, _I, _I, _P]),
    "agcn_adjacency_fused_bwd_scores": (_I, [_P, _P, _P, _P, _P, _P, _P, _P, _P, _Z, _I, _I, _I, _I, _I, _P]),
    "agcn_adjacency_bwd_softmax": (_I, [_P, _P, _P, _P, _P, _P, _P, _I, _I, _I, _I, _I, _P]),
    "agcn_adjacency_bwd_scores": (_I, [_P, _P, _P, _P, _P, _P, _I, _I, _I, _I, _P]),
    "agcn_colsum_scratch_bytes": (_Z, [_I]),
    "agcn_colsum": (_I, [_P, _I, _I, _P, _P, _P]),
    "agcn_bn_stats_finalize": (_I, [_P, _I, _I, _D, _P, _P, _P, _P, _F, _F, _P, _P, _P, _P, _P, _P]),
    "agcn_bn_eval_coeff": (_I, [_P, _P, _P, _P, _F, _I, _P, _P, _P]),
    "agcn_bn_act_fwd": (_I, [_P, _P, _P, _P, _P, _P, _P, _P, _I, _I, _I, _I, _I, _P]),
    "agcn_bn_bwd": (_I, [_P, _P, _I] + [_P] * 16 + [_I, _I, _I, _P]),
    "agcn_bn_bwd_reduce": (_I, [_P, _P, _I, _P, _P, _P, _I, _I, _I, _P]),
    "agcn_bn_bwd_apply": (_I, [_P, _I, _D, _F, _P, _P, _I] + [_P] * 15 + [_I, _I, _I, _P]),
    "agcn_bn_eval_coeff_ex": (_I, [_P, _P, _P, _P, _F, _I, _P, _P, _P, _P, _P]),
    "agcn_bn_bwd_eval": (_I, [_P, _P, _I, _P, _P, _P, _P, _I, _P, _P, _P, _P, _I, _I, _I, _P]),
    "agcn_bn_bwd_eval_finalize": (_I, [_P, _I, _I] + [_P] * 13),
    "agcn_stc_row_reduce": (_I, [_P, _P, _P, _P, _I, _P, _P, _F, _F, _I, _I, _I, _I, _P]),
    "agcn_stc_apply": (_I, [_P, _P, _P, _P, _P, _I, _I, _I, _I, _P]),
    "agcn_stc_apply_ex": (_I, [_P, _P, _P, _P, _P, _P, _I, _I, _I, _I, _P]),
    "agcn_stc_bwd_apply": (_I, [_P, _P, _P, _P, _P, _P, _P, _I, _I, _I, _I, _P]),
    "agcn_data_bn_stats": (_I, [_P, _P, _I, _I, _I, _I, _I, _P]),
    "agcn_data_bn_apply": (_I, [_P, _P, _P, _P, _I, _I, _I, _I, _I, _P]),
    "agcn_data_bn_bwd_reduce": (_I, [_P, _P, _P, _P, _P, _I, _I, _I, _I, _I, _P]),
    "agcn_data_bn_bwd_apply": (_I, [_P, _P, _P, _P, _P, _P, _D, _P, _I, _I, _I, _I, _I, _P]),
    "agcn_pool_fwd": (_I, [_P, _P, _P, _I, _I, _I, _I, _P]),
    "agcn_pool_bwd": (_I, [_P, _P, _I, _I, _I, _I, _P]),
    "agcn_linear_fwd": (_I, [_P, _P, _P, _P, _I, _I, _I, _I, _P]),
    "agcn_linear_bwd": (_I, [_P, _P, _P, _P, _P, _P, _P, _P, _I, _I, _I, _I, _P]),
    "agcn_gate_conv_fwd": (_I, [_P, _P, _P, _P, _I, _I, _I, _I, _P]),
    "agcn_gate_conv_bwd": (_I, [_P, _P, _P, _P, _P, _P, _P, _P, _I, _I, _I, _I, _P]),
    "agcn_sgd_step_workspace": (_Z, [ctypes.c_long]),
    "agcn_sgd_step": (_I, [_P, _P, _P, ctypes.c_long, _F, _F, _F, _I, _F, _F, _I, _P, _Z, _P, _P]),
}

_lib = None


def load():
    global _lib
    if _lib is not None:
        return _lib
    if not os.path.exists(LIB_PATH):
        raise RuntimeError(
            f"agcn_amd: HIP extension {LIB_PATH} not found -- run `python -c 'import __graft_entry__ as g; "
            f"g.build()'` (hipcc --offload-arch=gfx950).  There is no CPU fallback for the hot path.")
    lib = ctypes.CDLL(LIB_PATH)
    for name, (res, args) in SIGNATURES.items():
        fn = getattr(lib, name)
        fn.restype = res
        fn.argtypes = args
    _lib = lib
    return lib


def ptr_bits(t):
    if t is None:
        return None
    if not (t.is_cuda and t.is_contiguous() and t.dtype == torch.int32):
        raise RuntimeError(f"agcn_amd: expected a contiguous int32 GPU tensor, got {t.dtype} on {t.device}")
    return t.data_ptr()


def ptr(t):
    if t is None:
        return None
    if not (t.is_cuda and t.is_contiguous() and t.dtype == torch.float32):
        raise RuntimeError(f"agcn_amd: expected a contiguous fp32 GPU tensor, got {t.dtype} "
                           f"{tuple(t.shape)} on {t.device} contiguous={t.is_contiguous()}")
    return t.data_ptr()


def stream():
    return torch.cuda.current_stream().cuda_stream


def check(rc, what):
    if rc != 0:
        raise RuntimeError(f"agcn_amd: {what} failed with code {rc}")
```

### 2s-agcn_amd/ops.py

```python
import os
import weakref

import torch

from . import lib as _lib

BN_EPS = 1e-5
BN_MOMENTUM = 0.1


def _L():
    return _lib.load()


def _empty(shape, like):
    return torch.empty(shape, dtype=torch.float32, device=like.device)


def _ws(nbytes, like):
    return torch.empty((int(nbytes) + 3) // 4, dtype=torch.float32, device=like.device)


def _conv_ws(Cin, Cout, T, V, taps, stride, like, pad=None):
    pad = (taps - 1) // 2 if pad is None else pad
# ... 314 lines not shown
                                       _lib.stream()), "agcn_gate_conv_fwd")
    return a


def gate_conv_bwd(da, a, x, w):
    N, C, L = x.shape
    Ks = w.shape[-1]
    dpre = _empty((N, L), x)
    dx, dw, db = _empty((N, C, L), x), _empty((1, C, Ks), x), _empty((1,), x)
    _lib.check(_L().agcn_gate_conv_bwd(_lib.ptr(da), _lib.ptr(a), _lib.ptr(x), _lib.ptr(w.reshape(C, Ks)),
                                       _lib.ptr(dpre), _lib.ptr(dx), _lib.ptr(dw), _lib.ptr(db), N, C, L, Ks,
                                       _lib.stream()), "agcn_gate_conv_bwd")
    return dx, dw, db


class DataBNFunction(torch.autograd.Function):

    @staticmethod
    def forward(ctx, x, w, b, rm, rv, training, sync=None):
        x = x.contiguous()
        N, C, T, V, M = x.shape
        CH = C * V * M
        L = _L()
        if training:
            part = _empty((N, 2, CH), x)
            _lib.check(L.agcn_data_bn_stats(_lib.ptr(x), _lib.ptr(part), N, C, T, V, M, _lib.stream()),
                       "agcn_data_bn_stats")
            (st,), gcount = _bn_coeffs(True, [part], N * T, [(w, b, rm, rv)], sync, N)
        else:
            (st,), gcount = _bn_coeffs(False, [None], N * T, [(w, b, rm, rv)], None, N)
        out = _empty((N * M, C, T, V), x)
        _lib.check(L.agcn_data_bn_apply(_lib.ptr(x), _lib.ptr(st.scale), _lib.ptr(st.shift), _lib.ptr(out), N, C, T, V, M,
                                        _lib.stream()), "agcn_data_bn_apply")
        ctx.st, ctx.sync, ctx.gcount, ctx.training = st, sync, gcount, training
        ctx.save_for_backward(x, w)
        return out

    @staticmethod
    def backward(ctx, dy):
        x, w = ctx.saved_tensors
        st, sync = ctx.st, ctx.sync
        dy = dy.contiguous()
        N, C, T, V, M = x.shape
        CH = C * V * M
        L = _L()
        if not ctx.training:
            dx = dgamma = dbeta = None
            if ctx.needs_input_grad[0]:
                dx = torch.empty_like(x)
                zero = torch.zeros(2 * CH, dtype=torch.float32, device=x.device)
                _lib.check(L.agcn_data_bn_bwd_apply(_lib.ptr(dy), _lib.ptr(x), _lib.ptr(w), _lib.ptr(st.mean),
                                                    _lib.ptr(st.invstd), _lib.ptr(zero), float(ctx.gcount), _lib.ptr(dx),
                                                    N, C, T, V, M, _lib.stream()), "agcn_data_bn_bwd_apply")
            if ctx.needs_input_grad[1] or ctx.needs_input_grad[2]:
                part = _empty((N, 2, CH), x)
                _lib.check(L.agcn_data_bn_bwd_reduce(_lib.ptr(dy), _lib.ptr(x), _lib.ptr(st.mean), _lib.ptr(st.invstd),
                                                     _lib.ptr(part), N, C, T, V, M, _lib.stream()),
                           "agcn_data_bn_bwd_reduce")
                sums = _colsum(part, N, 2 * CH)
                dbeta, dgamma = sums[:CH], sums[CH:]
            return dx, dgamma, dbeta, None, None, None, None
        part = _empty((N, 2, CH), x)
        _lib.check(L.agcn_data_bn_bwd_reduce(_lib.ptr(dy), _lib.ptr(x), _lib.ptr(st.mean), _lib.ptr(st.invstd),
                                             _lib.ptr(part), N, C, T, V, M, _lib.stream()), "agcn_data_bn_bwd_reduce")
        sums = _colsum(part, N, 2 * CH)
        scale = 1.0
        if sync is not None:
            sums = _allreduce_sum(sums, sync)
            scale = 1.0 / sync.world
        dx = None
        if ctx.needs_input_grad[0]:
            dx = torch.empty_like(x)
            _lib.check(L.agcn_data_bn_bwd_apply(_lib.ptr(dy), _lib.ptr(x), _lib.ptr(w), _lib.ptr(st.mean),
                                                _lib.ptr(st.invstd), _lib.ptr(sums), float(ctx.gcount), _lib.ptr(dx), N, C,
                                                T, V, M, _lib.stream()), "agcn_data_bn_bwd_apply")
        dbeta, dgamma = sums[:CH], sums[CH:]
        if scale != 1.0:
            dbeta, dgamma = dbeta * scale, dgamma * scale
        return dx, dgamma, dbeta, None, None, None, None


def data_bn_supported(bn):
    return type(bn) in (torch.nn.BatchNorm1d, torch.nn.SyncBatchNorm)


class PoolFCFunction(torch.autograd.Function):

    @staticmethod
    def forward(ctx, x, w, b, M):
        x = x.contiguous()
        NM, C, T, V = x.shape
        N = NM // M
        rowmean, pooled = _empty((NM, C), x), _empty((N, C), x)
        _lib.check(_L().agcn_pool_fwd(_lib.ptr(x), _lib.ptr(rowmean), _lib.ptr(pooled), N, M, C, T * V, _lib.stream()),
                   "agcn_pool_fwd")
        logits = linear_fwd(pooled, w, b, 0)
        ctx.save_for_backward(pooled, logits, w)
        ctx.shape, ctx.M = (NM, C, T, V), M
        return logits

    @staticmethod
    def backward(ctx, dlogits):
        pooled, logits, w = ctx.saved_tensors
        NM, C, T, V = ctx.shape
        M = ctx.M
        dpooled, dw, db = linear_bwd(dlogits.contiguous(), logits, pooled, w, 0, need_din=True)
        dx = None
        if ctx.needs_input_grad[0]:
            dx = _empty((NM, C, T, V), pooled)
            _lib.check(_L().agcn_pool_bwd(_lib.ptr(dpooled), _lib.ptr(dx), NM // M, M, C, T * V, _lib.stream()),
                       "agcn_pool_bwd")
        return dx, dw, db, None


class STCAttentionFunction(torch.autograd.Function):

    @staticmethod
    def _gates(m_s, mv1, sa_w, sa_b, ta_w, ta_b, f1w, f1b, f2w, f2b, a_s=None):
        if a_s is None:
            a_s = gate_conv_fwd(m_s, sa_w, sa_b)
        if mv1 is None:
            return a_s, None, None, None, None
        a_t = gate_conv_fwd(mv1, ta_w, ta_b)
        m_c = (mv1 * a_t.unsqueeze(1)).mean(-1)
        h = linear_fwd(m_c, f1w, f1b, 1)
        a_c = linear_fwd(h, f2w, f2b, 2)
        return a_s, a_t, a_c, m_c, h

    @staticmethod
    def forward(ctx, y, sa_w, sa_b, ta_w, ta_b, f1w, f1b, f2w, f2b):
        y = y.contiguous()
        N, C, T, V = y.shape
        par = (sa_w, sa_b, ta_w, ta_b, f1w, f1b, f2w, f2b)
        _, m_s = stc_row_reduce(y, want_v=True, scale_v=1.0 / T)
        a_s = STCAttentionFunction._gates(m_s, None, *par)[0]
        mv1, _ = stc_row_reduce(y, wv=a_s, want_t=True, scale_t=1.0 / V)
        _, a_t, a_c, m_c, h = STCAttentionFunction._gates(m_s, mv1, *par, a_s=a_s)
        out = torch.empty_like(y)
        o_amax = _empty((1,), y) if fused_amax_enabled() else None
        INFER_STATS['stc_apply'] += 1
        _lib.check(_L().agcn_stc_apply_ex(_lib.ptr(y), _lib.ptr(a_s), _lib.ptr(a_t), _lib.ptr(a_c), _lib.ptr(out),
                                          _lib.ptr(o_amax), N, C, T, V, _lib.stream()), "agcn_stc_apply")
        _note_out_amax(out, o_amax)
        ctx.save_for_backward(y, m_s, mv1, a_s, a_t, a_c, m_c, h, *par)
        return out

    @staticmethod
    def backward(ctx, dout):
        y, m_s, mv1, a_s, a_t, a_c, m_c, h, *par = ctx.saved_tensors
        sa_w, sa_b, ta_w, ta_b, f1w, f1b, f2w, f2b = par
        dout = dout.contiguous()
        N, C, T, V = y.shape
        P1, P2 = stc_row_reduce(y, g=dout, wv=a_s, wt=a_t, want_t=True, want_v=True)
        da_c = (P1 * a_t.unsqueeze(1)).sum(-1).contiguous()
        da_t = (P1 * a_c.unsqueeze(-1)).sum(1)
        da_s = (P2 * a_c.unsqueeze(-1)).sum(1)
        dh, df2w, df2b = linear_bwd(da_c, a_c, h, f2w, 2)
        dm_c, df1w, df1b = linear_bwd(dh, h, m_c, f1w, 1)
        da_t = (da_t + (dm_c.unsqueeze(-1) * mv1).sum(1) / T).contiguous()
        dmv1 = dm_c.unsqueeze(-1) * a_t.unsqueeze(1) / T
        dmv1_t, dta_w, dta_b = gate_conv_bwd(da_t, a_t, mv1, ta_w)
        dmv1 = ((dmv1 + dmv1_t) / V).contiguous()
        _, R = stc_row_reduce(y, wt=dmv1, want_v=True)
        da_s = (da_s + R.sum(1)).contiguous()
        dm_s, dsa_w, dsa_b = gate_conv_bwd(da_s, a_s, m_s, sa_w)
        dms = (dm_s / T).contiguous()
        dy = torch.empty_like(y)
        _lib.check(_L().agcn_stc_bwd_apply(_lib.ptr(dout), _lib.ptr(a_s), _lib.ptr(a_t), _lib.ptr(a_c), _lib.ptr(dmv1),
                                           _lib.ptr(dms), _lib.ptr(dy), N, C, T, V, _lib.stream()),
                   "agcn_stc_bwd_apply")
        return dy, dsa_w, dsa_b, dta_w, dta_b, df1w, df1b, df2w, df2b


class BNState:
    __slots__ = ("mean", "invstd", "scale", "shift", "S", "eval")

    def __init__(self):
        self.S = 1
        self.eval = False


class SyncBN:
    __slots__ = ("world", "group")

    def __init__(self, world, group=None):
        self.world, self.group = int(world), group


def sync_of(bn_module):
    import torch.distributed as dist
    if isinstance(bn_module, torch.nn.SyncBatchNorm) and dist.is_available() and dist.is_initialized():
        world = dist.get_world_size(bn_module.process_group)
        if world > 1:
            return SyncBN(world, bn_module.process_group)
    return None


def _colsum(slab, nslots, width):
    out = _empty((width,), slab)
    scratch = _scratch(width, slab)
    _lib.check(_L().agcn_colsum(_lib.ptr(slab), int(nslots), int(width), scratch.data_ptr(), _lib.ptr(out),
                                _lib.stream()), "agcn_colsum")
    return out


COLLECTIVES = {'bn': 0, 'grad': 0}


def _allreduce_sum(t, sync):
    import torch.distributed as dist
    COLLECTIVES['bn'] += 1
    dist.all_reduce(t, op=dist.ReduceOp.SUM, group=sync.group)
    return t


def sync_stats(stats_parts, count, sync):
    sums = [_colsum(sp, sp.shape[0], sp.shape[1] * sp.shape[2]) for sp in stats_parts]
    buf = torch.cat(sums) if len(sums) > 1 else sums[0]
    _allreduce_sum(buf, sync)
    out, o = [], 0
    for sp in stats_parts:
        w = sp.shape[1] * sp.shape[2]
        out.append(buf[o:o + w].view(1, 2, sp.shape[2]))
        o += w
    return out


def bn_train_coeffs(stats_part, count, gamma, beta, running_mean, running_var, momentum=BN_MOMENTUM, eps=BN_EPS):
    C = gamma.numel()
    st = BNState()
    st.mean, st.invstd = _empty((C,), gamma), _empty((C,), gamma)
    st.scale, st.shift = _empty((C,), gamma), _empty((C,), gamma)
    nslots = stats_part.shape[0]
    scratch = _scratch(2 * C, gamma)
    _lib.check(_L().agcn_bn_stats_finalize(_lib.ptr(stats_part), nslots, C, float(count), _lib.ptr(gamma),
                                           _lib.ptr(beta), _lib.ptr(running_mean), _lib.ptr(running_var),
                                           float(momentum), float(eps), scratch.data_ptr(), _lib.ptr(st.mean),
                                           _lib.ptr(st.invstd),
                                           _lib.ptr(st.scale), _lib.ptr(st.shift), _lib.stream()),
               "agcn_bn_stats_finalize")
    return st


def bn_eval_coeffs(gamma, beta, running_mean, running_var, eps=BN_EPS):
    C = gamma.numel()
    st = BNState()
    st.eval = True
    st.scale, st.shift = _empty((C,), gamma), _empty((C,), gamma)
    st.mean, st.invstd = _empty((C,), gamma), _empty((C,), gamma)
    _lib.check(_L().agcn_bn_eval_coeff_ex(_lib.ptr(gamma), _lib.ptr(beta), _lib.ptr(running_mean),
                                          _lib.ptr(running_var), float(eps), C, _lib.ptr(st.scale), _lib.ptr(st.shift),
                                          _lib.ptr(st.mean), _lib.ptr(st.invstd), _lib.stream()),
               "agcn_bn_eval_coeff_ex")
    return st


def bn_act_fwd(y1, st1, r=None, st2=None, relu=True, want_bits=False, amax_out=None):
    N, C, T, V = y1.shape
    if st1.S > 1:
        N, C = N // st1.S, C * st1.S
    out = torch.empty_like(y1)
    bits = torch.empty((y1.numel() + 31) // 32, dtype=torch.int32, device=y1.device) if want_bits else None
    mode = 0 if r is None else (1 if st2 is None else 2)
    _lib.check(_L().agcn_bn_act_fwd_ex(_lib.ptr(y1), _lib.ptr(st1.scale), _lib.ptr(st1.shift), _lib.ptr(r),
                                       _lib.ptr(st2.scale) if st2 else None, _lib.ptr(st2.shift) if st2 else None,
                                       _lib.ptr(out), _lib.ptr_bits(bits), _lib.ptr(amax_out), N, C, T * V, mode,
                                       int(relu), _lib.stream()),
               "agcn_bn_act_fwd")
    return (out, bits) if want_bits else out


EVAL_BWD_STATS = {'sums': 0, 'nosums': 0}


def bn_bwd_eval(dout, mask, y1, st1, y2=None, st2=None, want_sums=True, amax_out=None):
    N, C, T, V = dout.shape
    two = st2 is not None
    dy1 = torch.empty_like(dout)
    dy2 = torch.empty_like(dout) if two else None
    part = _empty((N * C * 3,), dout) if want_sums else None
    mbits = int(mask is not None and mask.dtype == torch.int32)
    mptr = _lib.ptr_bits(mask) if mbits else _lib.ptr(mask)
    EVAL_BWD_STATS['sums' if want_sums else 'nosums'] += 1
    _lib.check(_L().agcn_bn_bwd_eval(_lib.ptr(dout), mptr, mbits, _lib.ptr(y1) if want_sums else None,
                                     _lib.ptr(st1.scale), _lib.ptr(y2) if (want_sums and two) else None,
                                     _lib.ptr(st2.scale) if two else None, int(want_sums), _lib.ptr(part),
                                     _lib.ptr(dy1), _lib.ptr(dy2), _lib.ptr(amax_out), N, C, T * V, _lib.stream()),
               "agcn_bn_bwd_eval")
    if not want_sums:
        return dy1, None, None, None, dy2, None, None, None
    dg1, db1, dc1 = _empty((C,), dout), _empty((C,), dout), _empty((C,), dout)
    dg2 = db2 = dc2 = None
    if two:
        dg2, db2, dc2 = _empty((C,), dout), _empty((C,), dout), _empty((C,), dout)
    _lib.check(_L().agcn_bn_bwd_eval_finalize(
        _lib.ptr(part), N, C, _lib.ptr(st1.scale), _lib.ptr(st1.mean), _lib.ptr(st1.invstd),
        _lib.ptr(st2.scale) if two else None, _lib.ptr(st2.mean) if two else None,
        _lib.ptr(st2.invstd) if two else None, _lib.ptr(dg1), _lib.ptr(db1), _lib.ptr(dc1), _lib.ptr(dg2),
        _lib.ptr(db2), _lib.ptr(dc2), _lib.stream()), "agcn_bn_bwd_eval_finalize")
    return dy1, dg1, db1, dc1, dy2, dg2, db2, dc2


def bn_bwd(dout, mask, y1, gamma1, st1, y2=None, gamma2=None, st2=None, sync=None, gcount=None, amax_out=None,
           want_sums=True, bias_out=None):
    if st1.eval:
        dy1, dg1, db1, dc1, dy2, dg2, db2, dc2 = bn_bwd_eval(dout, mask, y1, st1, y2, st2 if y2 is not None else None,
                                                             want_sums, amax_out)
        if bias_out is not None:
            bias_out[:] = [dc1, dc2]
        return dy1, dg1, db1, dy2, dg2, db2
    N, C, T, V = y1.shape
    S = st1.S
    if S > 1:
        N, C = N // S, C * S
        gamma1 = gamma1.repeat(S)
        gamma2 = gamma2.repeat(S) if gamma2 is not None else None
    part = _empty((N * C * 3,), y1)
    coef = _empty((6 * C,), y1)
    dy1 = torch.empty_like(y1)
    dg1, db1 = _empty((C,), y1), _empty((C,), y1)
    dy2 = dg2 = db2 = None
    if y2 is not None:
        dy2 = torch.empty_like(y2)
        dg2, db2 = _empty((C,), y1), _empty((C,), y1)
    mbits = int(mask is not None and mask.dtype == torch.int32)
    mptr = _lib.ptr_bits(mask) if mbits else _lib.ptr(mask)
    if sync is None and amax_out is not None:
        _lib.check(_L().agcn_bn_bwd_reduce(_lib.ptr(dout), mptr, mbits, _lib.ptr(y1), _lib.ptr(y2),
                                           _lib.ptr(part), N, C, T * V, _lib.stream()), "agcn_bn_bwd_reduce")
        _lib.check(_L().agcn_bn_bwd_apply_ex(
            _lib.ptr(part), N, float(N) * float(T * V), 1.0, _lib.ptr(dout), mptr, mbits, _lib.ptr(y1),
            _lib.ptr(gamma1), _lib.ptr(st1.mean), _lib.ptr(st1.invstd), _lib.ptr(y2), _lib.ptr(gamma2),
            _lib.ptr(st2.mean) if st2 else None, _lib.ptr(st2.invstd) if st2 else None, _lib.ptr(coef), _lib.ptr(dy1),
            _lib.ptr(dg1), _lib.ptr(db1), _lib.ptr(dy2), _lib.ptr(dg2), _lib.ptr(db2), _lib.ptr(amax_out), N, C, T * V,
            _lib.stream()), "agcn_bn_bwd_apply")
    elif sync is None:
        _lib.check(_L().agcn_bn_bwd(
            _lib.ptr(dout), mptr, mbits, _lib.ptr(y1), _lib.ptr(gamma1), _lib.ptr(st1.mean), _lib.ptr(st1.invstd),
            _lib.ptr(y2), _lib.ptr(gamma2), _lib.ptr(st2.mean) if st2 else None, _lib.ptr(st2.invstd) if st2 else None,
            _lib.ptr(part), _lib.ptr(coef), _lib.ptr(dy1), _lib.ptr(dg1), _lib.ptr(db1), _lib.ptr(dy2), _lib.ptr(dg2),
            _lib.ptr(db2), N, C, T * V, _lib.stream()), "agcn_bn_bwd")
    else:
        _lib.check(_L().agcn_bn_bwd_reduce(_lib.ptr(dout), mptr, mbits, _lib.ptr(y1), _lib.ptr(y2),
                                           _lib.ptr(part), N, C, T * V, _lib.stream()), "agcn_bn_bwd_reduce")
        sums = _allreduce_sum(_colsum(part, N, 3 * C), sync)
        total = float(gcount) if gcount is not None else float(N * T * V * sync.world)
        _lib.check(_L().agcn_bn_bwd_apply_ex(
            _lib.ptr(sums), 1, total, 1.0 / sync.world, _lib.ptr(dout), mptr, mbits, _lib.ptr(y1),
            _lib.ptr(gamma1), _lib.ptr(st1.mean), _lib.ptr(st1.invstd), _lib.ptr(y2), _lib.ptr(gamma2),
            _lib.ptr(st2.mean) if st2 else None, _lib.ptr(st2.invstd) if st2 else None, _lib.ptr(coef), _lib.ptr(dy1),
            _lib.ptr(dg1), _lib.ptr(db1), _lib.ptr(dy2), _lib.ptr(dg2), _lib.ptr(db2), _lib.ptr(amax_out), N, C, T * V,
            _lib.stream()), "agcn_bn_bwd_apply")
    if S > 1:
        dg1, db1 = dg1.view(S, -1).sum(0), db1.view(S, -1).sum(0)
        if dg2 is not None:
            dg2, db2 = dg2.view(S, -1).sum(0), db2.view(S, -1).sum(0)
    return dy1, dg1, db1, dy2, dg2, db2



class _Ctx:
    pass


def _bn_coeffs(training, stats, count, bns, sync=None, nsamples=None):
    S = bns[0][2].numel() // bns[0][0].numel()
    if not training:
        out = []
        for w, b, rm, rv in bns:
            C = w.numel()
            out.append(bn_eval_coeffs(w, b, rm[:C].contiguous(), rv[:C].contiguous()))
        return out, count
    if S > 1:
        if nsamples is None or nsamples % S:
            raise RuntimeError(f"agcn_amd: GhostBatchNorm with {S} splits needs a batch (x persons) divisible by {S}")
        stats = [_ghost_regroup(sp, S, nsamples) for sp in stats]
        bns = [(w.repeat(S), b.repeat(S), rm, rv) for w, b, rm, rv in bns]
        count = count // S
    if sync is not None:
        stats = sync_stats(stats, count, sync)
        count = count * sync.world
    note_params_changed()
    res = [bn_train_coeffs(sp, count, *bn) for sp, bn in zip(stats, bns)]
    for st in res:
        st.S = S
    return res, count


def _ghost_regroup(stats_part, S, nsamples):
    slots, two, C = stats_part.shape
    nt = slots // nsamples
    return stats_part.view(nsamples // S, S, nt, two, C).permute(0, 2, 3, 1, 4).reshape(nsamples // S * nt, two, S * C)


def gcn_forward(c, x, A, PA, wab, bab, wd, bd, bn, down, training, alpha=None, adaptive=True, sync=None,
                need_bwd=True):
    N, C, T, V = x.shape
    count = N * T * V
    first = down is not None and first_layer_enabled() and bool(_L().agcn_gcn_first_supported(C, wd.shape[0], V))
    x_amax = None if first else _take_out_amax(x)
    if adaptive and adjacency_fused_supported(C, wab.shape[0] // 6, T, V):
        keep = need_bwd and not adjacency_recompute()
        amax_here = None
        if x_amax is None and not first and fused_amax_enabled():
            amax_here = _empty((1,), x)
        if keep:
            P, adj, tp = adjacency_fused_fwd(x, wab, bab, A, PA, alpha, keep_tp=True, x_amax_out=amax_here, x_amax=x_amax)
        else:
            tp = None
            P, adj = adjacency_fused_fwd(x, wab, bab, A, PA, alpha, x_amax_out=amax_here, x_amax=x_amax)
        if amax_here is not None:
            x_amax = amax_here
    elif adaptive:
        tp, _ = conv_fwd(x, wab, bab)
        P, adj = adjacency_fwd(tp, A, PA, alpha)
    else:
        tp = P = None
        adj = A.unsqueeze(0).expand(N, 3, V, V).contiguous()
    if first:
        ypre, st, dpre, st2 = gcn_first_fwd(x, adj, wd, bd, down[0], down[1], want_stats=training)
    else:
        c.g_x_amax = x_amax
        ypre, st = aggregate_project_fwd(x, adj, wd, bd, want_stats=training, x_amax=c.g_x_amax)
    bn2 = None
    if not first:
        dpre = None
    if down is not None:
        if not first:
            dpre, st2 = conv_fwd(x, down[0], down[1], want_stats=training)
        (bn1, bn2), gcount = _bn_coeffs(training, [st, st2], count, [bn, down[2:]], sync, N)
        c.g_amax = _empty((1,), x) if fused_amax_enabled() else None
        out, bits = bn_act_fwd(ypre, bn1, dpre, bn2, relu=True, want_bits=True, amax_out=c.g_amax)
    else:
        (bn1,), gcount = _bn_coeffs(training, [st], count, [bn], sync, N)
        c.g_amax = _empty((1,), x) if fused_amax_enabled() else None
        out, bits = bn_act_fwd(ypre, bn1, x, None, relu=True, want_bits=True, amax_out=c.g_amax)
    c.g_sync, c.g_count = sync, gcount
    c.g_bits = bits
    c.g_x, c.g_tp, c.g_P, c.g_adj, c.g_ypre, c.g_dpre, c.g_out = x, tp, P, adj, ypre, dpre, out
    c.g_bn1, c.g_bn2 = bn1, bn2
    c.g_params = (wab, wd, bn[0], down[0] if down is not None else None, down[2] if down is not None else None)
    c.g_bab = bab
    c.g_alpha, c.g_adaptive = alpha, adaptive
    return out


def gcn_backward(c, dout, extra_add=None, extra_mask=None):
    x, tp, P, adj, ypre, dpre, out = c.g_x, c.g_tp, c.g_P, c.g_adj, c.g_ypre, c.g_dpre, c.g_out
    wab, wd, gamma1, wdown, gamma2 = c.g_params
    Cout = wd.shape[0]
    dy_amax = _empty((1,), dout) if fused_amax_enabled() else None
    c.g_dbias = []
    dypre, dg1, db1, ddpre, dg2, db2 = bn_bwd(dout, c.g_bits, ypre, gamma1, c.g_bn1, dpre, gamma2, c.g_bn2,
                                              sync=c.g_sync, gcount=c.g_count, amax_out=dy_amax,
                                              want_sums=getattr(c, 'g_want_sums', True), bias_out=c.g_dbias)
    x_amax = getattr(c, 'g_x_amax', None)
    dwd = _side_run(lambda: project_bwd_weight(dypre, x, adj, Cout, dy_amax, x_amax), (dypre, x, adj, dy_amax, x_amax))
    dPA = dwab = dbab = dalpha = dtp = dtp_amax = None
    if c.g_adaptive:
        dPA, dtp, dbab, dalpha, _, dtp_amax = adjacency_bwd(dypre, wd, x, tp, P, c.g_alpha, wab, c.g_bab,
                                                            dy_amax=dy_amax, x_amax=x_amax)
        dwab = _side_run(lambda: conv_bwd_weight(dtp, x, wab.shape, 1, dtp_amax, x_amax), (dtp, x, dtp_amax, x_amax))
    fuse = dtp is not None and fused_bwd_data_supported(x.shape[1], Cout, x.shape[3])
    ftp = dict(dtp=dtp, wab=wab) if fuse else {}
    ftp['dy_amax'] = dy_amax
    if fuse:
        ftp['dtp_amax'] = dtp_amax
    if dpre is None:
        dx = aggregate_project_bwd_data(dypre, adj, wd, x.shape, add1=dout, mask1=c.g_bits, add2=extra_add,
                                        mask2=extra_mask, **ftp)
    else:
        dx = aggregate_project_bwd_data(dypre, adj, wd, x.shape, add1=extra_add, mask1=extra_mask, **ftp)
    if dtp is not None and not fuse:
        conv_bwd_data(dtp, wab, x.shape, out=dx, accumulate=True)
    c.g_dalpha = dalpha
    dwdown = None
    if dpre is not None:
        dwdown = _side_run(lambda: conv_bwd_weight(ddpre, x, wdown.shape), (ddpre, x))
        conv_bwd_data(ddpre, wdown, x.shape, out=dx, accumulate=True)
    _side_join()
    return dx, dPA, dwab, dbab, dwd, dg1, db1, dwdown, dg2, db2


def tcn_forward(c, g, w, b, bn, stride, res_x, res, relu, training, sync=None, pad=None):
    N, C, T, V = g.shape
    if res is not None:
        To = conv_out_frames(T, w.shape[2], stride, pad)
        Tr = res_x.shape[2] if isinstance(res, str) else conv_out_frames(res_x.shape[2], 1, stride, 0)
        if Tr != To:
            raise RuntimeError(f"agcn_amd: the residual has {Tr} frames but the temporal convolution ({w.shape[2]} taps, "
                               f"stride {stride}, padding {(w.shape[2] - 1) // 2 if pad is None else pad}) gives {To} "
                               f"for {T} input frames; they must agree (the reference fails here too)")
    g_amax = getattr(c, 'g_amax', None) if getattr(c, 'g_out', None) is g else None
    if g_amax is None and getattr(c, 'g_out', None) is None:
        g_amax = _take_out_amax(g)
    zpre, st = conv_fwd(g, w, b, stride, want_stats=training, x_amax=g_amax, pad=pad)
    To = zpre.shape[2]
    count = N * To * V
    rpre = bn2 = None
    if res is None or isinstance(res, str):
        (bn1,), gcount = _bn_coeffs(training, [st], count, [bn], sync, N)
        o_amax = _empty((1,), g) if fused_amax_enabled() else None
        out, bits = bn_act_fwd(zpre, bn1, None if res is None else res_x, None, relu=relu, want_bits=True,
                               amax_out=o_amax)
    else:
        rpre, st2 = conv_fwd(res_x, res[0], res[1], stride, want_stats=training)
        (bn1, bn2), gcount = _bn_coeffs(training, [st, st2], count, [bn, res[2:]], sync, N)
        o_amax = _empty((1,), g) if fused_amax_enabled() else None
        out, bits = bn_act_fwd(zpre, bn1, rpre, bn2, relu=relu, want_bits=True, amax_out=o_amax)
    _note_out_amax(out, o_amax)
    c.t_sync, c.t_count = sync, gcount
    c.t_bits = bits
    c.t_g, c.t_zpre, c.t_rpre, c.t_out, c.t_bn1, c.t_bn2 = g, zpre, rpre, out, bn1, bn2
    c.t_g_amax = g_amax
    c.t_resx, c.t_res_identity = res_x, isinstance(res, str)
    c.t_params = (w, bn[0], res[0] if isinstance(res, tuple) else None, res[2] if isinstance(res, tuple) else None)
    c.t_stride, c.t_relu, c.t_pad = stride, relu, pad
    return out


def tcn_backward(c, dout, join=True):
    w, gamma1, wres, gamma2 = c.t_params
    mask = c.t_bits if c.t_relu else None
    dz_amax = _empty((1,), dout) if fused_amax_enabled() else None
    c.t_dbias = []
    dzpre, dg1, db1, drpre, dg2, db2 = bn_bwd(dout, mask, c.t_zpre, gamma1, c.t_bn1, c.t_rpre, gamma2, c.t_bn2,
                                              sync=c.t_sync, gcount=c.t_count, amax_out=dz_amax,
                                              want_sums=getattr(c, 't_want_sums', True), bias_out=c.t_dbias)
    t_g, t_stride, t_pad = c.t_g, c.t_stride, getattr(c, 't_pad', None)
    t_g_amax = getattr(c, 't_g_amax', None)
    dw = _side_run(lambda: conv_bwd_weight(dzpre, t_g, w.shape, t_stride, dz_amax, t_g_amax, pad=t_pad),
                   (dzpre, t_g, dz_amax, t_g_amax))
    dg = conv_bwd_data(dzpre, w, c.t_g.shape, c.t_stride, dy_amax=dz_amax, pad=t_pad)
    dwres = None
    if drpre is not None:
        t_resx = c.t_resx
        dwres = _side_run(lambda: conv_bwd_weight(drpre, t_resx, wres.shape, t_stride), (drpre, t_resx))
    if join:
        _side_join()
    return dg, dw, dg1, db1, drpre, dwres, dg2, db2


ERR_UNSUPPORTED = -3

_PARAM_EPOCH = [0]


def note_params_changed():
    _PARAM_EPOCH[0] += 1


def infer_fold_enabled():
    return os.environ.get('AGCN_INFER_FOLD', '1') != '0'


INFER_STATS = {'aagcn_unit_fused': 0, 'tconv_infer': 0, 'stc_apply': 0}


def _fold(bn):
    w, b, rm, rv = bn
    C = w.numel()
    s = w / torch.sqrt(rv[:C] + BN_EPS)
    return s, b - rm[:C] * s


def _fold_conv(w, b, bn):
    s, sh = _fold(bn)
    return (w * s[:, None, None, None]).contiguous(), (b * s + sh).contiguous()


def gcn_unit_infer(x, adj, wcat, bias, res=None, x2=None, w2=None, relu=True):
    N, C, T, V = x.shape
    Cout = wcat.shape[0]
    K2 = 0 if x2 is None else x2.shape[1]
    nbytes = _L().agcn_gcn_unit_infer_workspace(C, Cout, K2, T, V)
    ws = _ws(nbytes, x)
    y = _empty((N, Cout, T, V), x)
    rc = _L().agcn_gcn_unit_infer(_lib.ptr(x), _lib.ptr(adj), _lib.ptr(wcat), _lib.ptr(bias), _lib.ptr(res),
                                  _lib.ptr(x2), _lib.ptr(w2), K2, 1 if relu else 0, _lib.ptr(y), ws.data_ptr(), nbytes,
                                  N, C, Cout, T, V, _lib.stream())
    if rc == ERR_UNSUPPORTED:
        return None
    _lib.check(rc, "agcn_gcn_unit_infer")
    return y


def conv9_infer(x, w, b, res=None, relu=True, stride=1):
    N, Cin, T, V = x.shape
    Cout = w.shape[0]
    To = conv_out_frames(T, 9, stride)
    ws, nbytes = _conv_ws(Cin, Cout, T, V, 9, stride, x)
    y = _empty((N, Cout, To, V), x)
    rc = _L().agcn_conv9_infer(_lib.ptr(x), _lib.ptr(w), _lib.ptr(b), _lib.ptr(res), 1 if relu else 0, _lib.ptr(y),
                               ws.data_ptr(), nbytes, N, Cin, Cout, T, V, stride, _lib.stream())
    if rc == ERR_UNSUPPORTED:
        return None
    _lib.check(rc, "agcn_conv9_infer")
    return y


def tconv_infer(x, w, b, a_s=None, a_t=None, a_c=None, res=None, relu=True, stride=1, pad=None, x_amax=None):
    N, Cin, T, V = x.shape
    Cout, Cin2, taps, one = w.shape
    assert Cin2 == Cin and one == 1
    pad = (taps - 1) // 2 if pad is None else pad
    To = conv_out_frames(T, taps, stride, pad)
    if To < 1:
        raise ValueError(f"agcn_amd: a {taps}-frame kernel with padding {pad} does not fit {T} frames")
    ws, nbytes = _conv_ws(Cin, Cout, T, V, taps, stride, x, pad)
    y = _empty((N, Cout, To, V), x)
    rc = _L().agcn_tconv_infer(_lib.ptr(x), _lib.ptr(w), _lib.ptr(b), _lib.ptr(a_s), _lib.ptr(a_t), _lib.ptr(a_c),
                               _lib.ptr(res), 1 if relu else 0, _lib.ptr(y), ws.data_ptr(), nbytes, N, Cin, Cout, T, V,
                               taps, stride, pad, _lib.ptr(x_amax), _lib.stream())
    if rc == ERR_UNSUPPORTED:
        return None
    _lib.check(rc, "agcn_tconv_infer")
    INFER_STATS['tconv_infer'] += 1
    return y


def _cache_key(srcs):
    return (_PARAM_EPOCH[0],) + tuple((t.data_ptr(), t._version) for t in srcs if t is not None)


def tcn_infer(x, w, b, bn, stride, pad, cache=None):
    key = _cache_key([w, b, *bn])
    f = cache.get('folded') if cache is not None else None
    if f is None or f[0] != key:
        f = (key,) + _fold_conv(w, b, bn)
        if cache is not None:
            cache['folded'] = f
    return tconv_infer(x.contiguous(), f[1], f[2], relu=False, stride=stride, pad=pad)


def aagcn_unit_infer(x, p, cache=None):
    x = x.contiguous()
    N, C, T, V = x.shape
    if C < 32 or _L().agcn_gemm_mode() not in (b'bf16x6', b'bf16'):
        return None
    srcs = [t for wb in p['conv_d'] for t in wb] + [t for q in (p['ab'] or []) for t in q]
    srcs += [*p['gbn'], p['tw'], p['tb'], *p['tbn']] + list(p['down'] or []) + list(p['res'] or [])
    key = _cache_key(srcs)
    f = cache.get('folded') if cache is not None else None
    if f is None or f[0] != key:
        Cout = p['conv_d'][0][0].shape[0]
        wd = torch.cat([w.view(Cout, C) for w, _ in p['conv_d']], dim=1)
        bd = p['conv_d'][0][1] + p['conv_d'][1][1] + p['conv_d'][2][1]
        s1, sh1 = _fold(p['gbn'])
        wdf = (wd * s1[:, None]).contiguous()
        bias = bd * s1 + sh1
        w2 = None
        if p['down'] is not None:
            dw, db = _fold_conv(p['down'][0], p['down'][1], p['down'][2:])
            w2 = dw.reshape(Cout, C)
            bias = bias + db
        twf, tbf = _fold_conv(p['tw'], p['tb'], p['tbn'])
        rwf = rbf = None
        if p['res'] is not None:
            rwf, rbf = _fold_conv(p['res'][0], p['res'][1], p['res'][2:])
        wab = bab = None
        if p['ab'] is not None:
            wab = torch.cat([t for wa, _, wb_, _ in p['ab'] for t in (wa, wb_)], 0).contiguous()
            bab = torch.cat([t for _, ba, _, bb in p['ab'] for t in (ba, bb)], 0).contiguous()
        f = (key, wdf, bias.contiguous(), w2, twf, tbf, rwf, rbf, wab, bab)
        if cache is not None:
            cache['folded'] = f
    _, wdf, bias, w2, twf, tbf, rwf, rbf, wab, bab = f
    if wab is not None and adjacency_fused_supported(C, wab.shape[0] // 6, T, V):
        _, adj = adjacency_fused_fwd(x, wab, bab, None, p['PA'], p['alpha'])
    elif wab is not None:
        tp, _ = conv_fwd(x, wab, bab)
        _, adj = adjacency_fwd(tp, None, p['PA'], p['alpha'])
    else:
        adj = p['A'].unsqueeze(0).expand(N, 3, V, V).contiguous()
    if w2 is None:
        g = gcn_unit_infer(x, adj, wdf, bias, res=x)
    else:
        g = gcn_unit_infer(x, adj, wdf, bias, x2=x, w2=w2)
    if g is None:
        return None
    a_s = a_t = a_c = None
    if p['attn'] is not None:
        _, m_s = stc_row_reduce(g, want_v=True, scale_v=1.0 / T)
        a_s = STCAttentionFunction._gates(m_s, None, *p['attn'])[0]
        mv1, _ = stc_row_reduce(g, wv=a_s, want_t=True, scale_t=1.0 / V)
        _, a_t, a_c, _, _ = STCAttentionFunction._gates(m_s, mv1, *p['attn'], a_s=a_s)
    if p['res_mode'] == 0:
        r = None
    elif p['res_mode'] == 1:
        r = x
    else:
        r, _ = conv_fwd(x, rwf, rbf, p['stride'])
    y = tconv_infer(g, twf, tbf, a_s, a_t, a_c, res=r, relu=True, stride=p['stride'], pad=p['pad'])
    if y is not None:
        INFER_STATS['aagcn_unit_fused'] += 1
    return y


def unit_infer(x, A, PA, wab, bab, wd, bd, gbn, down, tw, tb, tbn, res_mode, res, stride, alpha=None, adaptive=True,
               cache=None):
    x = x.contiguous()
    N, C, T, V = x.shape
    Cout = wd.shape[0]
    if C < 32:
        return None
    srcs = [wd, bd, *gbn, tw, tb, *tbn] + (list(down) if down is not None else []) + \
           (list(res) if isinstance(res, tuple) else [])
    key = (_PARAM_EPOCH[0],) + tuple((t.data_ptr(), t._version) for t in srcs)
    f = cache.get('folded') if cache is not None else None
    if f is None or f[0] != key:
        s1, sh1 = _fold(gbn)
        wdf = (wd * s1[:, None]).contiguous()
        bias = bd * s1 + sh1
        w2 = None
        if down is not None:
            s2, sh2 = _fold(down[2:])
            w2 = (down[0].reshape(Cout, C) * s2[:, None]).contiguous()
            bias = bias + down[1] * s2 + sh2
        s3, sh3 = _fold(tbn)
        twf = (tw * s3[:, None, None, None]).contiguous()
        tbf = tb * s3 + sh3
        rwf = rbf = None
        if isinstance(res, tuple):
            s4, sh4 = _fold(res[2:])
            rwf = (res[0] * s4[:, None, None, None]).contiguous()
            rbf = res[1] * s4 + sh4
        f = (key, wdf, bias.contiguous(), w2, twf, tbf.contiguous(), rwf, rbf)
        if cache is not None:
            cache['folded'] = f
    _, wdf, bias, w2, twf, tbf, rwf, rbf = f
    if adaptive and adjacency_fused_supported(C, wab.shape[0] // 6, T, V):
        _, adj = adjacency_fused_fwd(x, wab, bab, A, PA, alpha)
    elif adaptive:
        tp, _ = conv_fwd(x, wab, bab)
        _, adj = adjacency_fwd(tp, A, PA, alpha)
    else:
        adj = A.unsqueeze(0).expand(N, 3, V, V).contiguous()
    if down is None:
        g = gcn_unit_infer(x, adj, wdf, bias, res=x)
    else:
        g = gcn_unit_infer(x, adj, wdf, bias, x2=x, w2=w2)
    if g is None:
        return None
    if res_mode == 0:
        r = None
    elif res_mode == 1:
        r = x
    else:
        r, _ = conv_fwd(x, rwf, rbf, stride)
    if tw.shape[2] == 9:
        return conv9_infer(g, twf, tbf, r, relu=True, stride=stride)
    return tconv_infer(g, twf, tbf, res=r, relu=True, stride=stride)


def _bias_grad(slot, k, n, like, needed=True):
    if slot and slot[k] is not None:
        return slot[k]
    if slot:
        return None
    return torch.zeros(n, dtype=torch.float32, device=like.device) if needed else None


class UnitGCNFunction(torch.autograd.Function):

    @staticmethod
    def forward(ctx, x, A, PA, wab, bab, wd, bd, bn_w, bn_b, bn_rm, bn_rv, down_w, down_b, dbn_w, dbn_b, dbn_rm,
                dbn_rv, training, alpha=None, adaptive=True, sync=None):
        c = _Ctx()
        down = None if down_w is None else (down_w, down_b, dbn_w, dbn_b, dbn_rm, dbn_rv)
        out = gcn_forward(c, x.contiguous(), A, PA, wab, bab, wd, bd, (bn_w, bn_b, bn_rm, bn_rv), down, training,
                          alpha, adaptive, sync, need_bwd=any(ctx.needs_input_grad))
        ctx.c, ctx.training = c, training
        ctx.has_down = down is not None
        _note_out_amax(out, getattr(c, 'g_amax', None))
        return out

    @staticmethod
    def backward(ctx, dout):
        ng = ctx.needs_input_grad
        ctx.c.g_want_sums = any(ng[i] for i in (6, 7, 8, 12, 13, 14))
        dx, dPA, dwab, dbab, dwd, dg1, db1, dwdown, dg2, db2 = gcn_backward(ctx.c, dout.contiguous())
        dbd = _bias_grad(ctx.c.g_dbias, 0, dwd.shape[0], dout)
        dbdown = _bias_grad(ctx.c.g_dbias, 1, dwd.shape[0], dout, ctx.has_down)
        dalpha = ctx.c.g_dalpha
        if dalpha is not None:
            dalpha = dalpha.reshape(1)
        ctx.c = None
        return (dx, None, dPA, dwab, dbab, dwd, dbd, dg1, db1, None, None, dwdown, dbdown, dg2, db2, None, None, None,
                dalpha, None, None)


class UnitTCNFunction(torch.autograd.Function):

    @staticmethod
    def forward(ctx, x, w, b, bn_w, bn_b, bn_rm, bn_rv, stride, training, sync=None, pad=None):
        c = _Ctx()
        out = tcn_forward(c, x.contiguous(), w, b, (bn_w, bn_b, bn_rm, bn_rv), stride, None, None, False, training,
                          sync, pad)
        ctx.c, ctx.training = c, training
        return out

    @staticmethod
    def backward(ctx, dout):
        ctx.c.t_want_sums = any(ctx.needs_input_grad[i] for i in (2, 3, 4))
        dg, dw, dg1, db1, _, _, _, _ = tcn_backward(ctx.c, dout.contiguous())
        dbias = _bias_grad(ctx.c.t_dbias, 0, dw.shape[0], dout)
        ctx.c = None
        return dg, dw, dbias, dg1, db1, None, None, None, None, None, None


class TCNResidualFunction(torch.autograd.Function):

    @staticmethod
    def forward(ctx, g, x, w, b, bn_w, bn_b, bn_rm, bn_rv, res_mode, rw, rb, rbn_w, rbn_b, rbn_rm, rbn_rv, stride,
                training, sync=None, pad=None):
        c = _Ctx()
        res = None if res_mode == 0 else ('identity' if res_mode == 1 else (rw, rb, rbn_w, rbn_b, rbn_rm, rbn_rv))
        x = x.contiguous() if x is not None else None
        out = tcn_forward(c, g.contiguous(), w, b, (bn_w, bn_b, bn_rm, bn_rv), stride, x, res, True, training, sync,
                          pad)
        ctx.c, ctx.training, ctx.res_mode, ctx.stride = c, training, res_mode, stride
        ctx.x_shape = tuple(x.shape) if x is not None else None
        return out

    @staticmethod
    def backward(ctx, dout):
        c = ctx.c
        dout = dout.contiguous()
        c.t_want_sums = any(ctx.needs_input_grad[i] for i in (3, 4, 5, 10, 11, 12))
        dg, dw, dg1, db1, drpre, dwres, dg2, db2 = tcn_backward(c, dout)
        dtb = _bias_grad(c.t_dbias, 0, dw.shape[0], dout)
        drb = _bias_grad(c.t_dbias, 1, dw.shape[0], dout, ctx.res_mode == 2)
        dx = None
        if ctx.res_mode == 1:
            dx = torch.where(c.t_out > 0, dout, torch.zeros_like(dout))
        elif ctx.res_mode == 2:
            dx = conv_bwd_data(drpre, c.t_params[2], ctx.x_shape, ctx.stride)
        ctx.c = None
        return (dg, dx, dw, dtb, dg1, db1, None, None, None,
                dwres, drb, dg2, db2, None, None, None, None, None, None)
# ... 48 lines not shown
```

### include/agcn_hip.h

```cpp
#ifndef AGCN_HIP_H
#define AGCN_HIP_H

#include <stddef.h>

#ifdef __cplusplus
extern "C" {
#endif

#define AGCN_OK 0
#define AGCN_ERR_ARG (-1)
#define AGCN_ERR_WORKSPACE (-2)
#define AGCN_ERR_UNSUPPORTED (-3)

int agcn_version(void);
const char* agcn_arch(void);

const char* agcn_last_kernel(void);
const char* agcn_gemm_mode(void);
const char* agcn_chain_mode(void);

int agcn_conv_tile_frames(int V, int T_out);
int agcn_conv_num_tiles(int V, int T_out);
int agcn_conv_stats_tiles(int Cin, int Cout, int T_out, int V, int taps, int stride);
int agcn_scores_num_tiles(int V, int T);
int agcn_dadj_num_slots(int C, int V, int T);

size_t agcn_conv_workspace(int Cin, int Cout, int T, int V, int taps, int stride);
int agcn_conv_fwd(const float* x, const float* w, const float* bias, float* y, float* stats_part, void* workspace,
                  size_t workspace_bytes, int N, int Cin, int Cout, int T, int V, int taps, int stride, void* stream);
int agcn_conv_bwd_data(const float* dy, const float* w, float* dx, int accumulate, const float* add1,
                       const float* mask1, const float* add2, const float* mask2, void* workspace,
                       size_t workspace_bytes, int N, int Cin, int Cout, int T, int V, int taps, int stride,
                       void* stream);
size_t agcn_conv_bwd_weight_workspace(int N, int Cin, int Cout, int T, int V, int taps, int stride);
int agcn_conv_bwd_weight(const float* dy, const float* x, float* dw, void* workspace, size_t workspace_bytes, int N,
                         int Cin, int Cout, int T, int V, int taps, int stride, void* stream);

size_t agcn_gcn_workspace(int C, int Cout, int T, int V);
int agcn_gcn_stats_tiles(int C, int Cout, int T, int V);
int agcn_gcn_stats_slots(int N, int C, int Cout, int T, int V);
int agcn_gcn_aggregate_project_fwd(const float* x, const float* adj, const float* wcat, const float* bias, float* y,
                                   float* stats_part, void* workspace, size_t workspace_bytes, int N, int C, int Cout,
                                   int T, int V, void* stream);
int agcn_bn_act_fwd_ex(const float* y1, const float* scale1, const float* shift1, const float* r, const float* scale2,
                       const float* shift2, float* out, unsigned* sign_bits, float* absmax_out, int N, int C, int P,
                       int res_mode, int relu, void* stream);
int agcn_bn_bwd_apply_ex(const float* part, int nrows, double count, float param_grad_scale, const float* dout,
                         const void* mask, int mask_bits, const float* y1, const float* gamma1, const float* mean1,
                         const float* invstd1, const float* y2, const float* gamma2, const float* mean2,
                         const float* invstd2, float* coef, float* dy1, float* dgamma1, float* dbeta1, float* dy2,
                         float* dgamma2, float* dbeta2, float* absmax1_out, int N, int C, int P, void* stream);
int agcn_gcn_aggregate_project_fwd_ex(const float* x, const float* adj, const float* wcat, const float* bias, float* y,
                                      float* stats_part, void* workspace, size_t workspace_bytes, int N, int C, int Cout,
                                      int T, int V, const float* x_absmax, void* stream);
int agcn_gcn_aggregate_project_bwd_data_ex(const float* dy, const float* adj, const float* wcat, const float* dtp,
                                           const float* w2, int K2, float* dx, int accumulate, const float* add1,
                                           const float* mask1, const float* add2, const float* mask2, int mask_bits,
                                           void* workspace, size_t workspace_bytes, int N, int C, int Cout, int T, int V,
                                           const float* dy_absmax, const float* dtp_absmax, void* stream);
int agcn_gcn_dadj_ex(const float* dy, const float* wcat, const float* x, float* dadj_part, void* workspace,
                     size_t workspace_bytes, int N, int C, int Cout, int T, int V, const float* dy_absmax,
                     const float* x_absmax, void* stream);
int agcn_adjacency_bwd_scores_ex(const float* tp, const float* dS, float* dtp, float* dbpart, void* scratch, float* db,
                                 float* dtp_absmax_out, int N, int Ci, int T, int V, void* stream);
int agcn_conv_bwd_weight_ex(const float* dy, const float* x, float* dw, void* workspace, size_t workspace_bytes, int N,
                            int Cin, int Cout, int T, int V, int taps, int stride, const float* dy_absmax,
                            const float* x_absmax, void* stream);
int agcn_gcn_project_bwd_weight_ex(const float* dy, const float* x, const float* adj, float* dwcat, void* workspace,
                                   size_t workspace_bytes, int N, int C, int Cout, int T, int V, const float* dy_absmax,
                                   const float* x_absmax, void* stream);
int agcn_absmax(const float* x, long n, float* out, void* stream);
int agcn_conv_fwd_ex(const float* x, const float* w, const float* bias, float* y, float* stats_part, void* workspace,
                     size_t workspace_bytes, int N, int Cin, int Cout, int T, int V, int taps, int stride,
                     const float* x_absmax, void* stream);
int agcn_conv_bwd_data_ex(const float* dy, const float* w, float* dx, int accumulate, const float* add1,
                          const float* mask1, const float* add2, const float* mask2, void* workspace,
                          size_t workspace_bytes, int N, int Cin, int Cout, int T, int V, int taps, int stride,
                          const float* dy_absmax, void* stream);

size_t agcn_tconv_workspace(int Cin, int Cout, int T, int V, int taps, int stride, int pad);
int agcn_tconv_stats_tiles(int Cin, int Cout, int T_out, int V, int taps, int stride, int pad);
int agcn_tconv_fwd(const float* x, const float* w, const float* bias, float* y, float* stats_part, void* workspace,
                   size_t workspace_bytes, int N, int Cin, int Cout, int T, int V, int taps, int stride, int pad,
                   const float* x_absmax, void* stream);
int agcn_tconv_bwd_data(const float* dy, const float* w, float* dx, int accumulate, const float* add1,
                        const float* mask1, const float* add2, const float* mask2, void* workspace,
                        size_t workspace_bytes, int N, int Cin, int Cout, int T, int V, int taps, int stride, int pad,
                        const float* dy_absmax, void* stream);
size_t agcn_tconv_bwd_weight_workspace(int N, int Cin, int Cout, int T, int V, int taps, int stride, int pad);
int agcn_tconv_bwd_weight(const float* dy, const float* x, float* dw, void* workspace, size_t workspace_bytes, int N,
                          int Cin, int Cout, int T, int V, int taps, int stride, int pad, const float* dy_absmax,
                          const float* x_absmax, void* stream);

int agcn_gcn_first_supported(int C, int Cout, int V);
int agcn_gcn_first_tiles(int T, int V);
int agcn_gcn_first_fwd(const float* x, const float* adj, const float* wcat, const float* bias, const float* wdown,
                       const float* bdown, float* ypre, float* ystats, float* dpre, float* dstats, int N, int C, int Cout,
                       int T, int V, void* stream);

size_t agcn_gcn_unit_infer_workspace(int C, int Cout, int K2, int T, int V);
int agcn_gcn_unit_infer(const float* x, const float* adj, const float* wcat, const float* bias, const float* res,
                        const float* x2, const float* w2, int K2, int relu, float* y, void* workspace,
                        size_t workspace_bytes, int N, int C, int Cout, int T, int V, void* stream);
int agcn_conv9_infer(const float* x, const float* w, const float* bias, const float* res, int relu, float* y,
                     void* workspace, size_t workspace_bytes, int N, int Cin, int Cout, int T, int V, int stride,
                     void* stream);

int agcn_tconv_infer(const float* x, const float* w, const float* bias, const float* a_s, const float* a_t,
                     const float* a_c, const float* res, int relu, float* y, void* workspace, size_t workspace_bytes,
                     int N, int Cin, int Cout, int T, int V, int taps, int stride, int pad, const float* x_absmax,
                     void* stream);

int agcn_gcn_aggregate_project_bwd_data(const float* dy, const float* adj, const float* wcat, float* dx,
                                        int accumulate, const float* add1, const float* mask1, const float* add2,
                                        const float* mask2, int mask_bits, void* workspace, size_t workspace_bytes, int N, int C,
                                        int Cout, int T, int V, void* stream);
int agcn_gcn_bwd_data_fused_supported(int C, int Cout, int V);
int agcn_gcn_aggregate_project_bwd_data_fused(const float* dy, const float* adj, const float* wcat, const float* dtp,
                                              const float* w2, int K2, float* dx, int accumulate, const float* add1,
                                              const float* mask1, const float* add2, const float* mask2, int mask_bits,
                                              void* workspace, size_t workspace_bytes, int N, int C, int Cout, int T,
                                              int V, void* stream);
size_t agcn_gcn_project_bwd_weight_workspace(int N, int C, int Cout, int T, int V);
int agcn_gcn_project_bwd_weight(const float* dy, const float* x, const float* adj, float* dwcat, void* workspace,
                                size_t workspace_bytes, int N, int C, int Cout, int T, int V, void* stream);
int agcn_gcn_dadj(const float* dy, const float* wcat, const float* x, float* dadj_part, void* workspace,
                  size_t workspace_bytes, int N, int C, int Cout, int T, int V, void* stream);

int agcn_adjacency_fwd(const float* tp, const float* A, const float* PA, const float* alpha, float* spart, float* P,
                       float* adj, int N, int Ci, int T, int V, void* stream);
int agcn_adjacency_fused_supported(int C, int Ci, int T, int V);
size_t agcn_adjacency_fused_workspace(int C, int Ci);
int agcn_adjacency_fused_fwd(const float* x, const float* wab, const float* bab, const float* A, const float* PA,
                             const float* alpha, float* tp_out, float* spart, float* P, float* adj, void* workspace,
                             size_t workspace_bytes, int N, int C, int Ci, int T, int V, void* stream);
int agcn_adjacency_fused_fwd_ex(const float* x, const float* wab, const float* bab, const float* A, const float* PA,
                                const float* alpha, float* tp_out, float* spart, float* P, float* adj, float* x_absmax_out,
                                const float* x_absmax_in, void* workspace, size_t workspace_bytes, int N, int C, int Ci, int T,
                                int V, void* stream);
int agcn_adjacency_fused_bwd_scores(const float* x, const float* wab, const float* bab, const float* dS, float* dtp,
                                    float* dbpart, void* scratch, float* db, void* workspace, size_t workspace_bytes,
                                    int N, int C, int Ci, int T, int V, void* stream);
int agcn_adjacency_bwd_softmax(const float* dadj_part, const float* P, const float* alpha, float* dadj, float* dS,
                               float* dPA, float* dalpha_part, int N, int Ci, int T, int V, int nslots, void* stream);
int agcn_adjacency_bwd_scores(const float* tp, const float* dS, float* dtp, float* dbpart, void* scratch, float* db,
                              int N, int Ci, int T, int V, void* stream);

size_t agcn_colsum_scratch_bytes(int W);
int agcn_colsum(const float* X, int nslots, int W, void* scratch, float* out, void* stream);
int agcn_bn_stats_finalize(const float* stats_part, int nslots, int C, double count, const float* gamma,
                           const float* beta, float* running_mean, float* running_var, float momentum, float eps,
                           void* scratch , float* mean, float* invstd,
                           float* scale, float* shift, void* stream);
int agcn_bn_eval_coeff(const float* gamma, const float* beta, const float* running_mean, const float* running_var,
                       float eps, int C, float* scale, float* shift, void* stream);
int agcn_bn_act_fwd(const float* y1, const float* scale1, const float* shift1, const float* r, const float* scale2,
                    const float* shift2, float* out, unsigned* sign_bits, int N, int C, int P, int res_mode, int relu,
                    void* stream);
int agcn_bn_bwd_reduce(const float* dout, const void* mask, int mask_bits, const float* y1, const float* y2, float* part,
                       int N, int C, int P, void* stream);
int agcn_bn_bwd_apply(const float* part, int nrows, double count, float param_grad_scale, const float* dout,
                      const void* mask, int mask_bits, const float* y1, const float* gamma1, const float* mean1,
                      const float* invstd1, const float* y2, const float* gamma2, const float* mean2, const float* invstd2, float* coef,
                      float* dy1, float* dgamma1, float* dbeta1, float* dy2, float* dgamma2, float* dbeta2, int N, int C,
                      int P, void* stream);
int agcn_bn_bwd(const float* dout, const void* mask, int mask_bits, const float* y1, const float* gamma1,
                const float* mean1, const float* invstd1, const float* y2, const float* gamma2, const float* mean2, const float* invstd2,
                float* part, float* coef, float* dy1, float* dgamma1, float* dbeta1, float* dy2, float* dgamma2,
                float* dbeta2, int N, int C, int P, void* stream);
int agcn_bn_eval_coeff_ex(const float* gamma, const float* beta, const float* running_mean, const float* running_var,
                          float eps, int C, float* scale, float* shift, float* mean, float* invstd, void* stream);
int agcn_bn_bwd_eval(const float* dout, const void* mask, int mask_bits, const float* y1, const float* scale1,
                     const float* y2, const float* scale2, int want_sums, float* part , float* dy1,
                     float* dy2, float* absmax1_out, int N, int C, int P, void* stream);
int agcn_bn_bwd_eval_finalize(const float* part, int nrows, int C, const float* scale1, const float* mean1,
                              const float* invstd1, const float* scale2, const float* mean2, const float* invstd2,
                              float* dgamma1, float* dbeta1, float* dbias1, float* dgamma2, float* dbeta2,
                              float* dbias2, void* stream);

int agcn_stc_row_reduce(const float* y, const float* g, const float* wv, const float* wt, int wt_per_row, float* out_t,
                        float* out_v, float scale_t, float scale_v, int N, int C, int T, int V, void* stream);
int agcn_stc_apply(const float* y, const float* a_s, const float* a_t, const float* a_c, float* out, int N, int C, int T,
                   int V, void* stream);
int agcn_stc_apply_ex(const float* y, const float* a_s, const float* a_t, const float* a_c, float* out, float* absmax_out,
                      int N, int C, int T, int V, void* stream);
int agcn_stc_bwd_apply(const float* dout, const float* a_s, const float* a_t, const float* a_c, const float* dmv,
                       const float* dms, float* dy, int N, int C, int T, int V, void* stream);

int agcn_data_bn_stats(const float* x, float* part, int N, int C, int T, int V, int M, void* stream);
int agcn_data_bn_apply(const float* x, const float* scale, const float* shift, float* out, int N, int C, int T, int V,
                       int M, void* stream);
int agcn_data_bn_bwd_reduce(const float* dy, const float* x, const float* mean, const float* invstd, float* part, int N,
                            int C, int T, int V, int M, void* stream);
int agcn_data_bn_bwd_apply(const float* dy, const float* x, const float* gamma, const float* mean, const float* invstd,
                           const float* sums, double count, float* dx, int N, int C, int T, int V, int M, void* stream);
int agcn_pool_fwd(const float* x, float* rowmean, float* pooled, int N, int M, int C, int P, void* stream);
int agcn_pool_bwd(const float* dpooled, float* dx, int N, int M, int C, int P, void* stream);
int agcn_linear_fwd(const float* in, const float* w, const float* b, float* out, int N, int K, int O, int act,
                    void* stream);
int agcn_linear_bwd(const float* dout, const float* out, const float* in, const float* w, float* dpre, float* din,
                    float* dw, float* db, int N, int K, int O, int act, void* stream);
int agcn_gate_conv_fwd(const float* in, const float* w, const float* b, float* a, int N, int C, int L, int Ks,
                       void* stream);
int agcn_gate_conv_bwd(const float* da, const float* a, const float* in, const float* w, float* dpre, float* din,
                       float* dw, float* db, int N, int C, int L, int Ks, void* stream);

size_t agcn_sgd_step_workspace(long n);
int agcn_sgd_step(float* param, const float* grad, float* momentum_buf, long n, float lr, float momentum,
                  float weight_decay, int nesterov, float max_norm, float grad_scale, int first_step, void* workspace,
                  size_t workspace_bytes, float* norm_out, void* stream);

#ifdef __cplusplus
}
#endif
#endif
```

Measured before the change: 1045 clips/s.

## Add streaming f16x3 MFMA wgrad kernel for 1x1 residual/down convs with fused absmax

Adds a new weight-gradient kernel for stride-1 pointwise convolutions that streams dy and x over the flattened N*T*V axis. It splits operands into hi/lo f16 pairs and accumulates with three 32x32x16 f16 MFMAs, reducing across K-waves in LDS and writing per-split partial slabs. The BN backward kernel now also computes the absmax of the second (residual/down) gradient, so these 1x1 wgrads get the range scales the f16 path needs. The kernel is only enabled for a few listed M/C configurations, and the split-f16 emulation may slightly change numerics relative to the previous path.

After: 1048 clips/s, median of 6. About the same (+0.3%).

```diff
diff --git a/2s-agcn_amd/csrc/agcn_common.h b/2s-agcn_amd/csrc/agcn_common.h
--- a/2s-agcn_amd/csrc/agcn_common.h
+++ b/2s-agcn_amd/csrc/agcn_common.h
@@ -109,6 +109,11 @@
                      int N, int M, int C, int V, int T_src, int T_out, int stride, hipStream_t s,
                      const float* dy_absmax = nullptr, const float* x_absmax = nullptr);
 
+bool agcn_wgrad_stream_supported(int N, int M, int C, int P, int stride, const float* dy_absmax, const float* x_absmax);
+size_t agcn_wgrad_stream_workspace(int N, int M, int C, int P);
+int agcn_wgrad_stream(const float* dy, const float* x, void* ws, size_t ws_bytes, int* nslabs, int N, int M, int C, int P,
+                      hipStream_t s, const float* dy_absmax, const float* x_absmax);
+
 bool agcn_wgrad9_bf16_supported(int M, int C, int V, int stride);
 size_t agcn_wgrad9_bf16_workspace(int N, int M, int C, int V, int T, int stride);
 int agcn_wgrad9_bf16(const float* dy, const float* x, void* ws, size_t ws_bytes, int* nslabs, int N, int M, int C, int V,
diff --git a/2s-agcn_amd/csrc/bn.hip b/2s-agcn_amd/csrc/bn.hip
--- a/2s-agcn_amd/csrc/bn.hip
+++ b/2s-agcn_amd/csrc/bn.hip
@@ -232,8 +232,9 @@
 bn_bwd_apply_kernel(const float4* __restrict__ dout, const float4* __restrict__ mask, int mask_bits,
                     const float4* __restrict__ y1,
                     const float4* __restrict__ y2, const float* __restrict__ coef, float4* __restrict__ dy1,
-                    float4* __restrict__ dy2, unsigned total4, unsigned P, unsigned C, unsigned* __restrict__ amax1) {
-  unsigned tmax = 0;
+                    float4* __restrict__ dy2, unsigned total4, unsigned P, unsigned C, unsigned* __restrict__ amax1,
+                    unsigned* __restrict__ amax2) {
+  unsigned tmax = 0, tmax2 = 0;
   for (unsigned i = blockIdx.x * blockDim.x + threadIdx.x; i < total4; i += gridDim.x * blockDim.x) {
     const unsigned e0 = i * 4u;
     const unsigned row = e0 / P;
@@ -272,6 +273,10 @@
 #pragma unroll
       for (int k = 0; k < 4; ++k) tmax = max(tmax, __float_as_uint(o1[k]) & 0x7fffffffu);
     }
+    if (HAS2 && amax2) {
+#pragma unroll
+      for (int k = 0; k < 4; ++k) tmax2 = max(tmax2, __float_as_uint(o2[k]) & 0x7fffffffu);
+    }
   }
   if (amax1) {
 #pragma unroll
@@ -282,6 +287,17 @@
     if (threadIdx.x == 0) {
       const unsigned m = max(max(wmax[0], wmax[1]), max(wmax[2], wmax[3]));
       if (m) atomicMax(amax1, m);
+    }
+  }
+  if (HAS2 && amax2) {
+#pragma unroll
+    for (int k = 32; k >= 1; k >>= 1) tmax2 = max(tmax2, (unsigned)__shfl_xor((int)tmax2, k));
+    __shared__ unsigned wmax2[4];
+    if ((threadIdx.x & 63u) == 0u) wmax2[threadIdx.x >> 6] = tmax2;
+    __syncthreads();
+    if (threadIdx.x == 0) {
+      const unsigned m = max(max(wmax2[0], wmax2[1]), max(wmax2[2], wmax2[3]));
+      if (m) atomicMax(amax2, m);
     }
   }
 }
@@ -382,23 +398,26 @@
                          const void* mask, int mask_bits, const float* y1, const float* gamma1, const float* mean1,
                          const float* invstd1, const float* y2, const float* gamma2, const float* mean2,
                          const float* invstd2, float* coef, float* dy1, float* dgamma1, float* dbeta1, float* dy2,
-                         float* dgamma2, float* dbeta2, float* absmax1_out, int N, int C, int P, void* stream);
+                         float* dgamma2, float* dbeta2, float* absmax1_out, float* absmax2_out, int N, int C, int P,
+                         void* stream);
 int agcn_bn_bwd_apply(const float* part, int nrows, double count, float param_grad_scale, const float* dout,
                       const void* mask, int mask_bits, const float* y1, const float* gamma1, const float* mean1, const float* invstd1,
                       const float* y2, const float* gamma2, const float* mean2, const float* invstd2, float* coef,
                       float* dy1, float* dgamma1, float* dbeta1, float* dy2, float* dgamma2, float* dbeta2, int N, int C,
                       int P, void* stream) {
   return agcn_bn_bwd_apply_ex(part, nrows, count, param_grad_scale, dout, mask, mask_bits, y1, gamma1, mean1, invstd1, y2,
-                              gamma2, mean2, invstd2, coef, dy1, dgamma1, dbeta1, dy2, dgamma2, dbeta2, nullptr, N, C, P,
-                              stream);
+                              gamma2, mean2, invstd2, coef, dy1, dgamma1, dbeta1, dy2, dgamma2, dbeta2, nullptr, nullptr, N, C,
+                              P, stream);
 }
 
 int agcn_bn_bwd_apply_ex(const float* part, int nrows, double count, float param_grad_scale, const float* dout,
                          const void* mask, int mask_bits, const float* y1, const float* gamma1, const float* mean1,
                          const float* invstd1, const float* y2, const float* gamma2, const float* mean2,
                          const float* invstd2, float* coef, float* dy1, float* dgamma1, float* dbeta1, float* dy2,
-                         float* dgamma2, float* dbeta2, float* absmax1_out, int N, int C, int P, void* stream) {
+                         float* dgamma2, float* dbeta2, float* absmax1_out, float* absmax2_out, int N, int C, int P,
+                         void* stream) {
   if (absmax1_out && hipMemsetAsync(absmax1_out, 0, 4, (hipStream_t)stream) != hipSuccess) return AGCN_ERR_ARG;
+  if (absmax2_out && hipMemsetAsync(absmax2_out, 0, 4, (hipStream_t)stream) != hipSuccess) return AGCN_ERR_ARG;
   if (!part || !dout || !y1 || !gamma1 || !mean1 || !invstd1 || !coef || !dy1 || !dgamma1 || !dbeta1 || nrows <= 0)
     return AGCN_ERR_ARG;
   if (y2 && (!gamma2 || !mean2 || !invstd2 || !dy2 || !dgamma2 || !dbeta2)) return AGCN_ERR_ARG;
@@ -415,11 +434,11 @@
   if (y2)
     hipLaunchKernelGGL(bn_bwd_apply_kernel<true>, g, b, 0, s, (const float4*)dout, (const float4*)mask, mask_bits,
                        (const float4*)y1, (const float4*)y2, (const float*)coef, (float4*)dy1, (float4*)dy2, t4,
-                       (unsigned)P, (unsigned)C, (unsigned*)absmax1_out);
+                       (unsigned)P, (unsigned)C, (unsigned*)absmax1_out, (unsigned*)absmax2_out);
   else
     hipLaunchKernelGGL(bn_bwd_apply_kernel<false>, g, b, 0, s, (const float4*)dout, (const float4*)mask, mask_bits,
                        (const float4*)y1, (const float4*)y2, (const float*)coef, (float4*)dy1, (float4*)dy2, t4,
-                       (unsigned)P, (unsigned)C, (unsigned*)absmax1_out);
+                       (unsigned)P, (unsigned)C, (unsigned*)absmax1_out, (unsigned*)absmax2_out);
   return agcn_check_launch();
 }
 
diff --git a/2s-agcn_amd/csrc/conv_wgrad.hip b/2s-agcn_amd/csrc/conv_wgrad.hip
--- a/2s-agcn_amd/csrc/conv_wgrad.hip
+++ b/2s-agcn_amd/csrc/conv_wgrad.hip
@@ -330,6 +330,7 @@
   auto kern = conv_wgrad_kernel<TAPS, AGG, MW, CW, TH, KSPLIT, WBX>;
   static unsigned char lds_ok[AGCN_MAX_DEVICES] = {};
   if (int e = agcn_allow_big_lds_rt(reinterpret_cast<const void*>(kern), lds_ok)) return e;
+  AGCN_NOTE_KERNEL("conv_wgrad_kernel<%d, %d, %d, %d, %d, %d, %d>", TAPS, AGG, MW, CW, TH, (int)KSPLIT, WBX);
   hipLaunchKernelGGL(kern, dim3(g.grid_x, g.nsplit), dim3(512), g.smem_bytes, stream, a);
   int rc = agcn_check_launch();
   if (rc) return rc;
@@ -439,6 +440,10 @@
                               : ws_wgrad<1, 0, 2, 2, 2, true>(N, Cout, Cin, V, T_out, stride, wsize);
   if (agcn_wgrad_chain_supported(Cout, Cin, V)) {
     const size_t t = agcn_wgrad_chain_workspace(0, N, Cout, Cin, V, T_out);
+    if (t > b) b = t;
+  }
+  if (stride == 1) {
+    const size_t t = agcn_wgrad_stream_workspace(N, Cout, Cin, T_out * V);
     if (t > b) b = t;
   }
   return b;
@@ -477,6 +482,12 @@
     }
     if (Cout % 128 == 0) return launch_wgrad<9, 0, 4, 1, 2, false, 7>(a, dw, workspace, workspace_bytes, s);
     return launch_wgrad<9, 0, 2, 2, 2, false, 7>(a, dw, workspace, workspace_bytes, s);
+  }
+  if (chain_wgrad_enabled() && agcn_wgrad_stream_supported(N, Cout, Cin, T * V, stride, dy_absmax, x_absmax)) {
+    int nslabs = 0;
+    const int rc = agcn_wgrad_stream(dy, x, workspace, workspace_bytes, &nslabs, N, Cout, Cin, T * V, s, dy_absmax, x_absmax);
+    if (rc) return rc;
+    return launch_reduce((const float*)workspace, dw, a.wsize, nslabs, a.M, a.C, a.so_m, a.so_t, a.so_c, s);
   }
   if (chain_wgrad_enabled() && agcn_wgrad_chain_supported(Cout, Cin, V))
     return chain_wgrad_and_reduce(0, a, dw, workspace, workspace_bytes, s, dy_absmax, x_absmax);
diff --git a/2s-agcn_amd/csrc/wgrad_chain.hip b/2s-agcn_amd/csrc/wgrad_chain.hip
--- a/2s-agcn_amd/csrc/wgrad_chain.hip
+++ b/2s-agcn_amd/csrc/wgrad_chain.hip
@@ -640,6 +640,7 @@
   auto kern = wgrad_chain_kernel<AGG, TM, NCB, VS, NW>;
   static unsigned char lds_ok[AGCN_MAX_DEVICES] = {};
   if (int e = agcn_allow_big_lds_rt(reinterpret_cast<const void*>(kern), lds_ok)) return e;
+  AGCN_NOTE_KERNEL("wgrad_chain_kernel<%d, %d, %d, %d, %d>", AGG, TM, NCB, VS, NW);
   hipLaunchKernelGGL(kern, dim3(g.grid_x, g.nsplit), dim3(NW * 64), g.smem_bytes, stream, a);
   *nslabs_out = g.nslabs;
   return agcn_check_launch();
diff --git a/2s-agcn_amd/csrc/wgrad_stream.hip b/2s-agcn_amd/csrc/wgrad_stream.hip
--- /dev/null
+++ b/2s-agcn_amd/csrc/wgrad_stream.hip
@@ -0,0 +1,263 @@
+#include "agcn_common.h"
+#include "split_f16.h"
+
+namespace {
+
+typedef f32x4 f32x4_u __attribute__((aligned(4)));
+typedef unsigned ws_u32x4 __attribute__((ext_vector_type(4)));
+
+__device__ __forceinline__ void ws_split_up(float a, float b, unsigned& p1, unsigned& p2) {
+  const sf_f32x2 v = {a, b};
+  const f16x2 h = __builtin_convertvector(v, f16x2);
+  const sf_f32x2 r = (v - __builtin_convertvector(h, sf_f32x2)) * 2048.f;
+  p1 = __builtin_bit_cast(unsigned, h);
+  p2 = __builtin_bit_cast(unsigned, __builtin_convertvector(r, f16x2));
+}
+
+struct WsArgs {
+  const float* dy;
+  const float* x;
+  float* part;
+  const float* dy_absmax;
+  const float* x_absmax;
+  int N, M, C, P;
+  int spr;
+  int total;
+  int spl;
+};
+
+constexpr int WS_WAVES = 8;
+
+template <int WM, int NMW, int NCW, int NKW, int KH>
+__global__ void __launch_bounds__(WS_WAVES * 64) wgrad_stream_kernel(const WsArgs a) {
+  static_assert(NMW * NCW * NKW == WS_WAVES, "8 waves");
+  constexpr int WC = 2, NT = WM * WC, NF = WM + WC, KS = 2 * KH, NK = KH / 8;
+  extern __shared__ float ws_red[];
+  const int lane = threadIdx.x & 63, wave = threadIdx.x >> 6;
+  const int r = lane & 31, h = lane >> 5;
+  const int mw = wave % NMW, cw = (wave / NMW) % NCW, kw = wave / (NMW * NCW);
+  const int m_base = mw * WM * 32, c_base = ((int)blockIdx.x * NCW + cw) * 64;
+  const int P = a.P;
+  const float* dy_end = a.dy + (long)a.N * a.M * P;
+  const float* x_end = a.x + (long)a.N * a.C * P;
+  float s_dy, i_dy, s_x, i_x;
+  f16_range_scale(a.dy_absmax, s_dy, i_dy);
+  f16_range_scale(a.x_absmax, s_x, i_x);
+
+  int loff[NF];
+#pragma unroll
+  for (int f = 0; f < NF; ++f) {
+    const int row = f < WM ? m_base + 32 * f + r : c_base + 32 * (f - WM) + r;
+    loff[f] = row * P + h * KH;
+  }
+
+  f32x16 acc[NT];
+#pragma unroll
+  for (int t = 0; t < NT; ++t)
+#pragma unroll
+    for (int j = 0; j < 16; ++j) acc[t][j] = 0.f;
+
+  const int q = (int)blockIdx.y * NKW + kw;
+  const long s_lo = (long)q * a.spl;
+  const int s0 = (int)(s_lo < a.total ? s_lo : a.total);
+  const int s1 = (int)(s_lo + a.spl < a.total ? s_lo + a.spl : a.total);
+
+  float raw[NF][KH];
+  auto load = [&](int s) __attribute__((always_inline)) {
+    const int n = s / a.spr, k0 = (s - n * a.spr) * KS;
+    const float* dyb = a.dy + (long)n * a.M * P + k0;
+    const float* xb = a.x + (long)n * a.C * P + k0;
+    if (k0 + KS <= P) {
+#pragma unroll
+      for (int f = 0; f < NF; ++f) {
+        const float* src = (f < WM ? dyb : xb) + loff[f];
+#pragma unroll
+        for (int e4 = 0; e4 < KH / 4; ++e4) {
+          const f32x4 v = *reinterpret_cast<const f32x4_u*>(src + 4 * e4);
+#pragma unroll
+          for (int e = 0; e < 4; ++e) raw[f][4 * e4 + e] = v[e];
+        }
+      }
+    } else {
+      const int rem = P - k0 - h * KH;
+#pragma unroll
+      for (int f = 0; f < NF; ++f) {
+        const float* src = (f < WM ? dyb : xb) + loff[f];
+        const float* end = f < WM ? dy_end : x_end;
+        if (src + KH <= end) {
+#pragma unroll
+          for (int e4 = 0; e4 < KH / 4; ++e4) {
+            const f32x4 v = *reinterpret_cast<const f32x4_u*>(src + 4 * e4);
+#pragma unroll
+            for (int e = 0; e < 4; ++e) raw[f][4 * e4 + e] = (4 * e4 + e < rem) ? v[e] : 0.f;
+          }
+        } else {
+#pragma unroll
+          for (int e = 0; e < KH; ++e) raw[f][e] = (e < rem) ? src[e] : 0.f;
+        }
+      }
+    }
+  };
+
+  if (s0 < s1) load(s0);
+  for (int s = s0; s < s1; ++s) {
+#pragma unroll
+    for (int kk = 0; kk < NK; ++kk) {
+      f16x8 hi[NF], lo[NF], hs[WC];
+#pragma unroll
+      for (int f = 0; f < NF; ++f) {
+        const float sc = f < WM ? s_dy : s_x;
+        ws_u32x4 p1, p2;
+#pragma unroll
+        for (int e2 = 0; e2 < 4; ++e2) {
+          unsigned q1, q2;
+          if (f < WM) ws_split_up(raw[f][8 * kk + 2 * e2] * sc, raw[f][8 * kk + 2 * e2 + 1] * sc, q1, q2);
+          else split_pair_f16_mix(raw[f][8 * kk + 2 * e2] * sc, raw[f][8 * kk + 2 * e2 + 1] * sc, q1, q2);
+          p1[e2] = q1; p2[e2] = q2;
+        }
+        hi[f] = __builtin_bit_cast(f16x8, p1);
+        lo[f] = __builtin_bit_cast(f16x8, p2);
+        if (f >= WM) hs[f - WM] = hi[f] * (_Float16)(1.f / 2048.f);
+      }
+      if (kk == NK - 1 && s + 1 < s1) load(s + 1);
+#pragma unroll
+      for (int i = 0; i < WM; ++i)
+#pragma unroll
+        for (int j = 0; j < WC; ++j) {
+          f32x16 d = acc[i * WC + j];
+          d = __builtin_amdgcn_mfma_f32_32x32x16_f16(lo[i], hs[j], d, 0, 0, 0);
+          d = __builtin_amdgcn_mfma_f32_32x32x16_f16(hi[i], lo[WM + j], d, 0, 0, 0);
+          d = __builtin_amdgcn_mfma_f32_32x32x16_f16(hi[i], hi[WM + j], d, 0, 0, 0);
+          acc[i * WC + j] = d;
+        }
+    }
+  }
+
+  if constexpr (NKW > 1) {
+    float* slot = ws_red + (size_t)(mw + NMW * cw) * NT * 16 * 64 + lane;
+    for (int k = 1; k < NKW; ++k) {
+      if (kw == k) {
+#pragma unroll
+        for (int t = 0; t < NT; ++t)
+#pragma unroll
+          for (int j = 0; j < 16; ++j) slot[(t * 16 + j) * 64] = acc[t][j];
+      }
+      __syncthreads();
+      if (kw == 0) {
+#pragma unroll
+        for (int t = 0; t < NT; ++t)
+#pragma unroll
+          for (int j = 0; j < 16; ++j) acc[t][j] += slot[(t * 16 + j) * 64];
+      }
+      __syncthreads();
+    }
+    if (kw != 0) return;
+  }
+  const float inv = i_dy * i_x;
+  float* dst = a.part + (long)blockIdx.y * a.M * a.C;
+#pragma unroll
+  for (int i = 0; i < WM; ++i)
+#pragma unroll
+    for (int j = 0; j < WC; ++j)
+#pragma unroll
+      for (int e = 0; e < 16; ++e) {
+        const int m = m_base + 32 * i + mfma_row(e, h), c = c_base + 32 * j + r;
+        dst[(long)m * a.C + c] = acc[i * WC + j][e] * inv;
+      }
+}
+
+struct WsPlan {
+  int wm, nmw, ncw, nkw, ncsplit;
+  bool ok;
+};
+
+#define WS_CASES(X)                                   \
+  X(3, 1, 1, 8)        \
+  X(3, 2, 1, 4)
+
+WsPlan ws_plan(int M, int C) {
+  WsPlan p = {0, 0, 0, 0, 1, false};
+  if (M <= 0 || C <= 0 || C % 64 != 0) return p;
+  if (M % 96 == 0) p.wm = 3;
+  else if (M % 64 == 0) p.wm = 2;
+  else return p;
+  p.nmw = M / (32 * p.wm);
+  p.ncw = C / 64;
+  if (p.nmw * p.ncw > WS_WAVES && p.ncw % 2 == 0) { p.ncsplit = 2; p.ncw /= 2; }
+  const int w = p.nmw * p.ncw;
+  if (w > WS_WAVES || WS_WAVES % w != 0) return p;
+  p.nkw = WS_WAVES / w;
+#define WS_LISTED(wm_, nmw_, ncw_, nkw_) if (p.wm == wm_ && p.nmw == nmw_ && p.ncw == ncw_ && p.nkw == nkw_) p.ok = true;
+  WS_CASES(WS_LISTED)
+#undef WS_LISTED
+  return p;
+}
+
+struct WsGeom {
+  int spr, total, spl, nsplit;
+  size_t smem;
+};
+
+WsGeom ws_geom(const WsPlan& p, int N, int P, int KH) {
+  WsGeom g;
+  g.spr = (P + 2 * KH - 1) / (2 * KH);
+  g.total = N * g.spr;
+  int want = 256 / p.ncsplit;
+  const int kmax = (g.total + p.nkw - 1) / p.nkw;
+  if (want > kmax) want = kmax;
+  if (want < 1) want = 1;
+  g.spl = (g.total + want * p.nkw - 1) / (want * p.nkw);
+  g.nsplit = (g.total + g.spl * p.nkw - 1) / (g.spl * p.nkw);
+  g.smem = p.nkw > 1 ? (size_t)p.nmw * p.ncw * (p.wm * 2) * 16 * 64 * 4 : 0;
+  return g;
+}
+
+constexpr int WS_KH = 16;
+
+template <int WM, int NMW, int NCW, int NKW>
+int ws_launch(WsArgs a, const WsPlan& p, const WsGeom& g, hipStream_t stream) {
+  auto kern = wgrad_stream_kernel<WM, NMW, NCW, NKW, WS_KH>;
+  static unsigned char lds_ok[AGCN_MAX_DEVICES] = {};
+  if (g.smem > 48 * 1024)
+    if (int e = agcn_allow_big_lds_rt(reinterpret_cast<const void*>(kern), lds_ok)) return e;
+  AGCN_NOTE_KERNEL("wgrad_stream_kernel<%d, %d, %d, %d, %d>", WM, NMW, NCW, NKW, WS_KH);
+  hipLaunchKernelGGL(kern, dim3(p.ncsplit, g.nsplit), dim3(WS_WAVES * 64), g.smem, stream, a);
+  return agcn_check_launch();
+}
+
+inline bool ws_enabled() {
+  static const int on = getenv("AGCN_WGRAD_STREAM") ? atoi(getenv("AGCN_WGRAD_STREAM")) : 1;
+  return on != 0;
+}
+
+}
+
+bool agcn_wgrad_stream_supported(int N, int M, int C, int P, int stride, const float* dy_absmax, const float* x_absmax) {
+  if (!ws_enabled() || !dy_absmax || !x_absmax || stride != 1 || agcn_gemm_precision() != 3) return false;
+  static const int f16x3 = getenv("AGCN_WGRAD_F16X3") ? atoi(getenv("AGCN_WGRAD_F16X3")) : 1;
+  if (!f16x3 || N <= 0 || P <= 0 || (long)(M > C ? M : C) * P >= (1L << 31) - 64) return false;
+  return ws_plan(M, C).ok;
+}
+
+size_t agcn_wgrad_stream_workspace(int N, int M, int C, int P) {
+  const WsPlan p = ws_plan(M, C);
+  if (!p.ok) return 0;
+  return (size_t)ws_geom(p, N, P, WS_KH).nsplit * M * C * 4;
+}
+
+int agcn_wgrad_stream(const float* dy, const float* x, void* ws, size_t ws_bytes, int* nslabs, int N, int M, int C, int P,
+                      hipStream_t s, const float* dy_absmax, const float* x_absmax) {
+  const WsPlan p = ws_plan(M, C);
+  if (!p.ok) return AGCN_ERR_UNSUPPORTED;
+  const WsGeom g = ws_geom(p, N, P, WS_KH);
+  if ((size_t)g.nsplit * M * C * 4 > ws_bytes) return AGCN_ERR_WORKSPACE;
+  WsArgs a = {};
+  a.dy = dy; a.x = x; a.part = (float*)ws; a.dy_absmax = dy_absmax; a.x_absmax = x_absmax;
+  a.N = N; a.M = M; a.C = C; a.P = P; a.spr = g.spr; a.total = g.total; a.spl = g.spl;
+  *nslabs = g.nsplit;
+#define WS_LAUNCH(wm_, nmw_, ncw_, nkw_) \
+  if (p.wm == wm_ && p.nmw == nmw_ && p.ncw == ncw_ && p.nkw == nkw_) return ws_launch<wm_, nmw_, ncw_, nkw_>(a, p, g, s);
+  WS_CASES(WS_LAUNCH)
+#undef WS_LAUNCH
+  return AGCN_ERR_UNSUPPORTED;
+}
diff --git a/2s-agcn_amd/lib.py b/2s-agcn_amd/lib.py
--- a/2s-agcn_amd/lib.py
+++ b/2s-agcn_amd/lib.py
@@ -46,7 +46,7 @@
     "agcn_tconv_bwd_weight_workspace": (_Z, [_I] * 8),
     "agcn_tconv_bwd_weight": (_I, [_P] * 4 + [_Z] + [_I] * 8 + [_P] * 3),
     "agcn_bn_act_fwd_ex": (_I, [_P, _P, _P, _P, _P, _P, _P, _P, _P, _I, _I, _I, _I, _I, _P]),
-    "agcn_bn_bwd_apply_ex": (_I, [_P, _I, _D, _F, _P, _P, _I] + [_P] * 16 + [_I, _I, _I, _P]),
+    "agcn_bn_bwd_apply_ex": (_I, [_P, _I, _D, _F, _P, _P, _I] + [_P] * 17 + [_I, _I, _I, _P]),
     "agcn_conv_fwd_ex": (_I, [_P, _P, _P, _P, _P, _P, _Z, _I, _I, _I, _I, _I, _I, _I, _P, _P]),
     "agcn_conv_bwd_data_ex": (_I, [_P, _P, _P, _I, _P, _P, _P, _P, _P, _Z, _I, _I, _I, _I, _I, _I, _I, _P, _P]),
     "agcn_gcn_first_supported": (_I, [_I, _I, _I]),
diff --git a/2s-agcn_amd/ops.py b/2s-agcn_amd/ops.py
--- a/2s-agcn_amd/ops.py
+++ b/2s-agcn_amd/ops.py
@@ -640,7 +640,7 @@
 
 
 def bn_bwd(dout, mask, y1, gamma1, st1, y2=None, gamma2=None, st2=None, sync=None, gcount=None, amax_out=None,
-           want_sums=True, bias_out=None):
+           want_sums=True, bias_out=None, amax2_out=None):
     if st1.eval:
         dy1, dg1, db1, dc1, dy2, dg2, db2, dc2 = bn_bwd_eval(dout, mask, y1, st1, y2, st2 if y2 is not None else None,
                                                              want_sums, amax_out)
@@ -670,7 +670,8 @@
             _lib.ptr(part), N, float(N) * float(T * V), 1.0, _lib.ptr(dout), mptr, mbits, _lib.ptr(y1),
             _lib.ptr(gamma1), _lib.ptr(st1.mean), _lib.ptr(st1.invstd), _lib.ptr(y2), _lib.ptr(gamma2),
             _lib.ptr(st2.mean) if st2 else None, _lib.ptr(st2.invstd) if st2 else None, _lib.ptr(coef), _lib.ptr(dy1),
-            _lib.ptr(dg1), _lib.ptr(db1), _lib.ptr(dy2), _lib.ptr(dg2), _lib.ptr(db2), _lib.ptr(amax_out), N, C, T * V,
+            _lib.ptr(dg1), _lib.ptr(db1), _lib.ptr(dy2), _lib.ptr(dg2), _lib.ptr(db2), _lib.ptr(amax_out),
+            _lib.ptr(amax2_out) if y2 is not None else None, N, C, T * V,
             _lib.stream()), "agcn_bn_bwd_apply")
     elif sync is None:
         _lib.check(_L().agcn_bn_bwd(
@@ -687,7 +688,8 @@
             _lib.ptr(sums), 1, total, 1.0 / sync.world, _lib.ptr(dout), mptr, mbits, _lib.ptr(y1),
             _lib.ptr(gamma1), _lib.ptr(st1.mean), _lib.ptr(st1.invstd), _lib.ptr(y2), _lib.ptr(gamma2),
             _lib.ptr(st2.mean) if st2 else None, _lib.ptr(st2.invstd) if st2 else None, _lib.ptr(coef), _lib.ptr(dy1),
-            _lib.ptr(dg1), _lib.ptr(db1), _lib.ptr(dy2), _lib.ptr(dg2), _lib.ptr(db2), _lib.ptr(amax_out), N, C, T * V,
+            _lib.ptr(dg1), _lib.ptr(db1), _lib.ptr(dy2), _lib.ptr(dg2), _lib.ptr(db2), _lib.ptr(amax_out),
+            _lib.ptr(amax2_out) if y2 is not None else None, N, C, T * V,
             _lib.stream()), "agcn_bn_bwd_apply")
     if S > 1:
         dg1, db1 = dg1.view(S, -1).sum(0), db1.view(S, -1).sum(0)
@@ -789,9 +791,11 @@
     Cout = wd.shape[0]
     dy_amax = _empty((1,), dout) if fused_amax_enabled() else None
     c.g_dbias = []
+    dd_amax = _empty((1,), dout) if dy_amax is not None and dpre is not None and not c.g_bn1.eval else None
     dypre, dg1, db1, ddpre, dg2, db2 = bn_bwd(dout, c.g_bits, ypre, gamma1, c.g_bn1, dpre, gamma2, c.g_bn2,
                                               sync=c.g_sync, gcount=c.g_count, amax_out=dy_amax,
-                                              want_sums=getattr(c, 'g_want_sums', True), bias_out=c.g_dbias)
+                                              want_sums=getattr(c, 'g_want_sums', True), bias_out=c.g_dbias,
+                                              amax2_out=dd_amax)
     x_amax = getattr(c, 'g_x_amax', None)
     dwd = _side_run(lambda: project_bwd_weight(dypre, x, adj, Cout, dy_amax, x_amax), (dypre, x, adj, dy_amax, x_amax))
     dPA = dwab = dbab = dalpha = dtp = dtp_amax = None
@@ -814,7 +818,7 @@
     c.g_dalpha = dalpha
     dwdown = None
     if dpre is not None:
-        dwdown = _side_run(lambda: conv_bwd_weight(ddpre, x, wdown.shape), (ddpre, x))
+        dwdown = _side_run(lambda: conv_bwd_weight(ddpre, x, wdown.shape, 1, dd_amax, x_amax), (ddpre, x, dd_amax, x_amax))
         conv_bwd_data(ddpre, wdown, x.shape, out=dx, accumulate=True)
     _side_join()
     return dx, dPA, dwab, dbab, dwd, dg1, db1, dwdown, dg2, db2
@@ -852,6 +856,7 @@
     c.t_g, c.t_zpre, c.t_rpre, c.t_out, c.t_bn1, c.t_bn2 = g, zpre, rpre, out, bn1, bn2
     c.t_g_amax = g_amax
     c.t_resx, c.t_res_identity = res_x, isinstance(res, str)
+    c.t_resx_amax = getattr(c, 'g_x_amax', None) if res_x is not None and getattr(c, 'g_x', None) is res_x else None
     c.t_params = (w, bn[0], res[0] if isinstance(res, tuple) else None, res[2] if isinstance(res, tuple) else None)
     c.t_stride, c.t_relu, c.t_pad = stride, relu, pad
     return out
@@ -862,9 +867,11 @@
     mask = c.t_bits if c.t_relu else None
     dz_amax = _empty((1,), dout) if fused_amax_enabled() else None
     c.t_dbias = []
+    dr_amax = _empty((1,), dout) if dz_amax is not None and c.t_rpre is not None and not c.t_bn1.eval else None
     dzpre, dg1, db1, drpre, dg2, db2 = bn_bwd(dout, mask, c.t_zpre, gamma1, c.t_bn1, c.t_rpre, gamma2, c.t_bn2,
                                               sync=c.t_sync, gcount=c.t_count, amax_out=dz_amax,
-                                              want_sums=getattr(c, 't_want_sums', True), bias_out=c.t_dbias)
+                                              want_sums=getattr(c, 't_want_sums', True), bias_out=c.t_dbias,
+                                              amax2_out=dr_amax)
     t_g, t_stride, t_pad = c.t_g, c.t_stride, getattr(c, 't_pad', None)
     t_g_amax = getattr(c, 't_g_amax', None)
     dw = _side_run(lambda: conv_bwd_weight(dzpre, t_g, w.shape, t_stride, dz_amax, t_g_amax, pad=t_pad),
@@ -873,7 +880,9 @@
     dwres = None
     if drpre is not None:
         t_resx = c.t_resx
-        dwres = _side_run(lambda: conv_bwd_weight(drpre, t_resx, wres.shape, t_stride), (drpre, t_resx))
+        resx_amax = getattr(c, 't_resx_amax', None)
+        dwres = _side_run(lambda: conv_bwd_weight(drpre, t_resx, wres.shape, t_stride, dr_amax, resx_amax),
+                          (drpre, t_resx, dr_amax, resx_amax))
     if join:
         _side_join()
     return dg, dw, dg1, db1, drpre, dwres, dg2, db2
diff --git a/include/agcn_hip.h b/include/agcn_hip.h
--- a/include/agcn_hip.h
+++ b/include/agcn_hip.h
@@ -49,7 +49,8 @@
                          const void* mask, int mask_bits, const float* y1, const float* gamma1, const float* mean1,
                          const float* invstd1, const float* y2, const float* gamma2, const float* mean2,
                          const float* invstd2, float* coef, float* dy1, float* dgamma1, float* dbeta1, float* dy2,
-                         float* dgamma2, float* dbeta2, float* absmax1_out, int N, int C, int P, void* stream);
+                         float* dgamma2, float* dbeta2, float* absmax1_out, float* absmax2_out, int N, int C, int P,
+                         void* stream);
 int agcn_gcn_aggregate_project_fwd_ex(const float* x, const float* adj, const float* wcat, const float* bias, float* y,
                                       float* stats_part, void* workspace, size_t workspace_bytes, int N, int C, int Cout,
                                       int T, int V, const float* x_absmax, void* stream);
```
